# markweberdev/maskbit

Hardware: AMD Instinct MI355X
Metric: images/sec (256x256, 64-step MaskBit-12bit, CFG) (higher is better)
Workload: dtype f16

## Files before the change

include/maskbit_hip_diag.h:

```cpp
#ifndef MASKBIT_HIP_DIAG_H
#define MASKBIT_HIP_DIAG_H

#include "maskbit_hip.h"

#ifdef __cplusplus
extern "C" {
#endif

int mb_gemm(int epi, const void* A, const void* W, const float* bias, const float* residual, float* out_f32,
            void* out_h16, int M, int N, int K, int period, int variant, mb_stream stream);
int mb_gemm_ex(int epi, const void* A, const void* W, const float* bias, const float* residual, float* out_f32, void* out_h16,
               int M, int N, int K, const float* ln_stats, const float* ln_g, const float* ln_b, int period, int variant, mb_stream stream);
int mb_layernorm(const float* y, const float* gamma, const float* beta, float eps, float* x_f32, void* x_h16, void* x_lo, float* stats,
                 int M, int d, mb_stream stream);
int mb_gemm_act_split(int epi, const void* A_hi, const void* A_lo, const void* W, const float* bias, const float* residual,
                      float* out_f32, void* out_h16, int M, int N, int kw, int variant, mb_stream stream);
int mb_gemm_mini(int epi, const void* A, const void* W, const float* bias, const float* residual, float* out_f32, void* out_h16, void* out4,
                 void* out4_scale, int rows, int pair, int N, int K, int nlo, const void* const* lo, mb_stream stream);
int mb_gemm_mini_seq(int epi, const void* A, const void* W, const float* bias, const float* residual, float* out_f32, void* out_h16, void* out4,
                     void* out4_scale, void* out4l, void* out4l_scale, int rows, int pair, int seq_rows, int N, int K, int nlo, const void* const* lo, mb_stream stream);
int mb_w4_from_f32(const float* W, int N, int K, void* dst4, void* scale_out, mb_stream stream);
int mb_w4lo_from_f32(const float* W, int N, int K, void* dst4, void* scale_out, mb_stream stream);
int mb_gemm_head(int epi, const void* A_hi, const void* A_lo, const void* W_hi, const void* W_lo, const float* scale, const float* bias, int bias_per_pos,
                 float* out_f32, int M, int N, int kw, int period, mb_stream stream);
int mb_cast_f32_to_h16(const float* src, void* dst, int64_t n, mb_stream stream);
int mb_split_f32_planes(const float* src, void* hi, void* lo, int N, int K, float* scale_out, unsigned* tmp, mb_stream stream);
int mb_gemm_mini_split(int epi, const void* A_hi, const void* A_lo, const void* W, const float* bias, void* out_h16, void* out4, void* out4_scale,
                       int rows, int N, int kw, const void* const* lo, mb_stream stream);
int mb_gemm_mini_ln(const void* A, const void* W, const float* bias, float* y, const float* ln_stats, const float* ln_g, const float* ln_b, int rows, int pair,
                    int seq_rows, int N, int K, int nlo, const void* const* lo, mb_stream stream);
int mb_layernorm_f4(const float* y, const float* gamma, const float* beta, float eps, float* x_f32, void* x_h16, void* x4, void* x4_scale, void* xl4,
                    void* xl4_scale, int M, int d, mb_stream stream);
int mb_layernorm_f4_seq(const float* y, const float* gamma, const float* beta, float eps, float* x_f32, void* x_h16, void* x4, void* x4_scale, void* xl4,
                        void* xl4_scale, int M, int d, int seq_rows, mb_stream stream);

int mb_layernorm_pair(const float* y, const float* gamma, const float* beta, float eps, void* x_h16, float* stats, void* x4, void* x4_scale, void* xl4,
                      void* xl4_scale, int P, int d, int seq_rows, mb_stream stream);
int mb_pairify(const float* x_f32, void* x_h16, void* x4, void* x4_scale, void* xl4, void* xl4_scale, int P, int d, int seq_rows, mb_stream stream);
int mb_embed_ln(const int64_t* tokens, const int64_t* labels, const uint8_t* drop, const float* w_in, const float* b_in, const float* class_emb,
                const float* pos, const float* gamma, const float* beta, const float* tables, float* x_f32, void* x_h16, void* x_lo, void* x4,
                void* x4_scale, void* xl4, void* xl4_scale, int nb, int seq, int m, int gbits, int d, int nclass, mb_stream stream);
int mb_embed_pair(const int64_t* tokens, const int64_t* labels, const float* w_in, const float* b_in, const float* class_emb, const float* pos,
                  const float* gamma, const float* beta, const float* tables, float* x_f32, void* x_h16, void* x4, void* x4_scale, void* xl4,
                  void* xl4_scale, int nb, int seq, int m, int gbits, int d, int nclass, mb_stream stream);
int mb_attention_pair(const void* qkv, void* out_h16, int pairs, int N, int d, int heads, mb_stream stream);
int mb_attention_pair_f4(const void* qkv, void* out_h16, void* out4, void* out4_scale, void* out4l, void* out4l_scale, int pairs, int N, int d, int heads, mb_stream stream);
int mb_attention(const void* qkv, void* out_h16, void* out4, void* out4_scale, int nb, int N, int d, int heads, mb_stream stream);
int mb_attention_probs(const void* qkv, float* out_f32, int nb, int N, int d, int heads, mb_stream stream);
int mb_gen_set_alo(mb_gen* g, int gemm_mask);
int mb_set_cu_count(int n);
int mb_gen_set_walk(mb_gen* g, int mode);
int mb_diag_set_walk(int reverse);
int mb_walk_tile(int vb, int ntiles, int reverse);
int mb_walk_seq(int slot, int n, int grp, int reverse);
int mb_walk_row(int slot, int rows, int seq_rows, int pair, int reverse);
int mb_walk_group(int seq_rows, int pair);
int mb_gemm_ht_supported(int epi, int M, int N, int K);

int mb_seeded_noise(const int64_t* seeds, int step, float randomize_temperature, float conf_weight, float* exp_u, float* exp_noise, float* conf_u,
                    float* conf_noise, int B, int P, int C, mb_stream stream);

int mb_vq_argmin(const float* z, const float* codebook, int N, int C, int K, int l2, int splits, int64_t* idx, float* dist, mb_stream stream);

int mb_vq_encode_rows(const void* z_h16, int stride16, const float* z_f32, const float* codebook, int B, int HW, int C, int K, int l2, int splits,
                      int64_t* idx, float* zq_nchw, float* zraw_nchw, float* dist, mb_stream stream);
int mb_vq_gather(const int64_t* codes, const float* codebook, int64_t npix, int C, int K, int l2, int cin_pad, void* out_h16, unsigned* sat,
                 mb_stream stream);
int mb_vq_pack_latent(const float* z_nchw, int B, int K, int HW, int cin_pad, void* out_h16, unsigned* sat, mb_stream stream);
int mb_lfq_pack(const void* z_h16, int B, int HW, int K, int Kp, int64_t* idx, float* zq_nchw, float* zraw_nchw, mb_stream stream);
int mb_lfq_latent(const int64_t* tokens, int64_t npix, int K, void* out_h16, mb_stream stream);
int mb_pack_image(const float* img_nchw, int B, int C, int H, int W, void* out_h16, mb_stream stream);

int mb_conv_layer(const void* in_h16, const float* w_oihw, const float* bias, const float* gn_gamma, const float* gn_beta, const void* residual_h16,
                  void* out_h16, float* img_nchw, uint8_t* img_nhwc_u8, const float* out_gamma, const float* out_beta, float* out_scale_shift,
                  float* out_gn_part, int* part_tiles, unsigned* saturated, int B, int H, int W, int Cin, int Cout, int ks, int up, int final_layer,
                  mb_stream stream);
int mb_conv_layer_ex(const void* in_h16, const float* w_oihw, const float* bias, const float* gn_gamma, const float* gn_beta, const void* residual_h16,
                     void* out_h16, float* img_nchw, uint8_t* img_nhwc_u8, const float* out_gamma, const float* out_beta, float* out_scale_shift,
                     float* out_gn_part, int* part_tiles, unsigned* saturated, int B, int H, int W, int Cin, int Cout, int ks, int up, int final_layer,
                     int flags, mb_stream stream);
int mb_autoenc_block(const void* x_h16, const float* n1_g, const float* n1_b, const float* c1_w, const float* c1_b, const float* n2_g, const float* n2_b,
                     const float* c2_w, const float* c2_b, const float* sc_w, const float* sc_b, int form, int bias, void* out_h16, void* h1_h16,
                     void* mid_h16, const float* out_gamma, const float* out_beta, float* out_scale_shift, unsigned* saturated, int B, int H, int W,
                     int cin, int cout, mb_stream stream);
int mb_groupnorm_stats(const void* x_h16, const float* gamma, const float* beta, float* scale_shift, int B, int HW, int C, mb_stream stream);
int mb_avgpool2(const void* x_h16, void* y_h16, int B, int H, int W, int C, mb_stream stream);
int mb_s2d(const void* x_h16, void* y_h16, int B, int H, int W, int C, mb_stream stream);

int mb_conv_relu_layer(const void* in_h16, const float* w_oihw, const float* bias, void* out_h16, unsigned* saturated, int B, int H, int W, int Cin,
                       int Cout, int ks, mb_stream stream);
int mb_maxpool2(const void* x_h16, void* y_h16, int B, int H, int W, int C, mb_stream stream);
int mb_lpips_input(const float* real, const float* fake, const float* shift_scale, void* out_h16, int B, int H, int W, int clamp01, mb_stream stream);
int mb_lpips_distance(const void* feat_a, const void* feat_b, const float* w, int B, int HW, int C, double* per_image, mb_stream stream);
int mb_lpips_features(mb_lpips* h, const float* real, const float* fake, int B, int H, int W, int clamp01, void* tap0, void* tap1, void* tap2, void* tap3,
                      void* tap4, mb_stream stream);

int mb_convbn_layer(const void* in_h16, const float* w_oihw, const float* scale, const float* shift, void* out_h16, unsigned* saturated, int B, int H,
                    int W, int Cin, int Cout, int kh, int kw, int stride, int ph, int pw, int in_off, int in_cs, int out_off, int out_cs, int variant,
                    mb_stream stream);
int mb_pool3(const void* x_h16, void* y_h16, int B, int H, int W, int C, int mode, int in_off, int in_cs, int out_off, int out_cs, mb_stream stream);
int mb_inception_input(const uint8_t* u8, void* out_h16, int B, int H, int W, mb_stream stream);
int mb_inception_taps(mb_inception* h, const uint8_t* u8, int B, int H, int W, void* map0, void* map1, void* map2, void* map3, float* tap64,
                      float* tap192, float* tap768, float* pool, float* logits_unbiased, float* logits, mb_stream stream);

int mb_spatial_attention(const void* q, const void* k, const void* v, void* out_h16, unsigned* sat, int B, int N, int ld, int ldo, mb_stream stream);
int mb_taming_set_tap(mb_taming* h, int block, void* out_h16);
int mb_taming_attn_block(mb_taming* h, int block, const void* x_h16, void* qkv_out, void* attn_out, void* out_h16, const float* out_gamma,
                         const float* out_beta, float* out_scale_shift, int B, int H, int W, mb_stream stream);
int mb_taming_final(mb_taming* h, const void* x_h16, float* img_nchw, uint8_t* img_nhwc_u8, int B, int H, int W, mb_stream stream);
int mb_taming_pack_image(const float* img_nchw, void* out_h16, int B, int H, int W, mb_stream stream);

int mb_gemm_f32(int epi, const float* A, const float* W, const float* bias, const float* residual, float* out, int M, int N, int K, int period,
                int bias_per_pos, mb_stream stream);
int mb_attention_f32(const float* qkv, float* out, int nb, int N, int d, int heads, mb_stream stream);

typedef struct {
  int64_t* label; int64_t* seed;
  int32_t* num_regen; int32_t* slot; int32_t* local_step; int32_t* N;
  mb_request_step* pool;
  int max_active, max_steps;
} mb_session_rows;
int mb_session_row_table(const mb_session_rows* rows, mb_request_step* row_out, int A, mb_stream stream);
int mb_session_admit_rows(const mb_session_rows* rows, int64_t* tokens, int A, int K, const int64_t* labels, const int64_t* seeds, const int* num_steps,
                          const mb_request_step* schedule, const int64_t* init_tokens, int n, int m, int C, mb_stream stream);
int mb_session_retire(const mb_session_rows* rows, int64_t* tokens, const int64_t* pred, int64_t* codes_all, int64_t* codes_out, int32_t* plan,
                      int A, int n, int m, int C, mb_stream stream);

int mb_image_coeffs(int in_size, int out_size, int filter, int first, int count, int ksize, int32_t* xmin, int32_t* n, int32_t* taps, mb_stream stream);

#ifdef __cplusplus
}
#endif
#endif
```

maskbit_amd/_lib.py:

```python
from __future__ import annotations

import ctypes as C
import os
from typing import Optional

_HERE = os.path.dirname(os.path.abspath(__file__))
LIB_PATH = os.path.join(_HERE, "libmaskbit_hip.so")
ABI_VERSION = 8


class GenCfg(C.Structure):
    _fields_ = [(n, C.c_int) for n in ("bits", "splits", "hidden", "heads", "depth", "mlp", "seq", "nclass", "prenorm", "embed_tables", "precision")]


class DecCfg(C.Structure):
    _fields_ = [("token_size", C.c_int), ("hidden_channels", C.c_int), ("num_resolutions", C.c_int),
                ("num_res_blocks", C.c_int), ("num_channels", C.c_int), ("channel_mult", C.c_int * 8),
                ("latent_size", C.c_int), ("build_encoder", C.c_int), ("sample_with_conv", C.c_int),
                ("enc_res_blocks", C.c_int)]


class SamplePlan(C.Structure):
    _fields_ = [("num_steps", C.c_int), ("use_guidance", C.c_int), ("scale", C.POINTER(C.c_float)),
                ("temperature", C.POINTER(C.c_float)), ("mask_len", C.POINTER(C.c_int)), ("step_begin", C.c_int), ("step_end", C.c_int)]
# ... 25 lines not shown
SIGNATURES = {
    "mb_gen_saturation_count": (C.c_int, [C.c_void_p, C.POINTER(C.c_uint), C.c_int, C.c_void_p]),
    "mb_abi_version": (C.c_int, []),
    "mb_last_error": (C.c_char_p, []),
    "mb_gen_create": (C.c_int, [C.POINTER(GenCfg), C.c_int, C.POINTER(C.c_void_p)]),
    "mb_gen_destroy": (None, [C.c_void_p]),
    "mb_gen_load": (C.c_int, [C.c_void_p, C.c_char_p, C.c_void_p, C.POINTER(C.c_int64), C.c_int, C.c_void_p]),
    "mb_gen_set_alo": (C.c_int, [C.c_void_p, C.c_int]),
    "mb_gen_forward": (C.c_int, [C.c_void_p, C.c_void_p, C.c_void_p, C.c_void_p, C.c_void_p, C.c_int, C.c_void_p]),
    "mb_gen_forward_cfg": (C.c_int, [C.c_void_p, C.c_void_p, C.c_void_p, C.c_void_p, C.c_int, C.c_void_p]),
    "mb_gen_forward_attn": (C.c_int, [C.c_void_p, C.c_void_p, C.c_void_p, C.c_void_p, C.c_void_p, C.c_void_p, C.c_int, C.c_void_p]),
    "mb_sample_step": (C.c_int, [C.c_void_p, C.c_void_p, C.c_float, C.c_float, C.c_void_p, C.c_void_p, C.c_int,
                                 C.c_void_p, C.c_void_p, C.c_void_p, C.c_int, C.c_int, C.c_int, C.c_int, C.c_void_p]),
    "mb_dec_create": (C.c_int, [C.POINTER(DecCfg), C.c_int, C.POINTER(C.c_void_p)]),
    "mb_dec_destroy": (None, [C.c_void_p]),
    "mb_dec_load": (C.c_int, [C.c_void_p, C.c_char_p, C.c_void_p, C.POINTER(C.c_int64), C.c_int, C.c_void_p]),
    "mb_dec_decode": (C.c_int, [C.c_void_p, C.c_void_p, C.c_void_p, C.c_void_p, C.c_int, C.c_void_p]),
    "mb_dec_saturation_count": (C.c_int, [C.c_void_p, C.POINTER(C.c_uint), C.c_int, C.c_void_p]),
    "mb_enc_encode": (C.c_int, [C.c_void_p, C.c_void_p, C.c_void_p, C.c_void_p, C.c_void_p, C.c_int, C.c_void_p]),
    "mb_dec_create_vq": (C.c_int, [C.POINTER(DecCfg), C.c_int, C.c_int, C.c_int, C.POINTER(C.c_void_p)]),
    "mb_dec_decode_latent": (C.c_int, [C.c_void_p, C.c_void_p, C.c_void_p, C.c_void_p, C.c_int, C.c_void_p]),
    "mb_enc_encode_vq": (C.c_int, [C.c_void_p, C.c_void_p, C.c_void_p, C.c_void_p, C.c_void_p, C.c_void_p, C.c_int, C.c_void_p]),
    "mb_vq_argmin": (C.c_int, [C.c_void_p, C.c_void_p, C.c_int, C.c_int, C.c_int, C.c_int, C.c_int, C.c_void_p, C.c_void_p, C.c_void_p]),
    "mb_vq_encode_rows": (C.c_int, [C.c_void_p, C.c_int, C.c_void_p, C.c_void_p] + [C.c_int] * 6 + [C.c_void_p] * 5),
    "mb_vq_gather": (C.c_int, [C.c_void_p, C.c_void_p, C.c_int64, C.c_int, C.c_int, C.c_int, C.c_int, C.c_void_p, C.c_void_p, C.c_void_p]),
    "mb_vq_pack_latent": (C.c_int, [C.c_void_p, C.c_int, C.c_int, C.c_int, C.c_int, C.c_void_p, C.c_void_p, C.c_void_p]),
    "mb_lfq_pack": (C.c_int, [C.c_void_p, C.c_int, C.c_int, C.c_int, C.c_int, C.c_void_p, C.c_void_p, C.c_void_p, C.c_void_p]),
    "mb_lfq_latent": (C.c_int, [C.c_void_p, C.c_int64, C.c_int, C.c_void_p, C.c_void_p]),
    "mb_pack_image": (C.c_int, [C.c_void_p, C.c_int, C.c_int, C.c_int, C.c_int, C.c_void_p, C.c_void_p]),
    "mb_sample": (C.c_int, [C.c_void_p, C.c_void_p, C.POINTER(SamplePlan), C.c_void_p, C.c_int, C.c_void_p, C.c_void_p,
                            C.c_void_p, C.c_void_p, C.c_void_p, C.c_void_p, C.c_void_p]),
    "mb_sample_step_edit": (C.c_int, [C.c_void_p, C.c_void_p, C.c_float, C.c_float, C.c_void_p, C.c_void_p, C.c_float, C.c_void_p,
                                      C.c_void_p, C.c_void_p, C.c_void_p, C.c_int, C.c_int, C.c_int, C.c_int, C.c_void_p]),
    "mb_sample_edit": (C.c_int, [C.c_void_p, C.c_void_p, C.POINTER(EditPlan), C.c_void_p, C.c_int, C.c_void_p, C.c_void_p, C.c_void_p,
                                 C.c_void_p, C.c_void_p, C.c_void_p, C.c_void_p, C.c_void_p]),
    "mb_sample_step_seeded": (C.c_int, [C.c_void_p, C.c_void_p, C.c_float, C.c_float, C.c_void_p, C.c_int, C.c_float, C.c_float, C.c_float, C.c_void_p,
                                        C.c_void_p, C.c_void_p, C.c_void_p, C.c_int, C.c_int, C.c_int, C.c_int, C.c_void_p]),
    "mb_sample_seeded": (C.c_int, [C.c_void_p, C.c_void_p, C.POINTER(EditPlan), C.c_void_p, C.c_int, C.c_void_p, C.c_void_p, C.c_float,
                                   C.POINTER(C.c_float), C.c_void_p, C.c_void_p, C.c_void_p, C.c_void_p, C.c_void_p]),
    "mb_sample_step_requests": (C.c_int, [C.c_void_p, C.c_void_p, C.c_void_p, C.c_void_p, C.c_void_p, C.c_void_p, C.c_void_p, C.c_void_p,
                                          C.c_int, C.c_int, C.c_int, C.c_int, C.c_void_p]),
    "mb_sample_requests": (C.c_int, [C.c_void_p, C.c_void_p, C.POINTER(RequestPlan), C.c_void_p, C.c_int, C.c_void_p, C.c_void_p,
                                     C.c_void_p, C.c_void_p, C.c_void_p, C.c_void_p, C.c_void_p]),
    "mb_session_create": (C.c_int, [C.c_int, C.c_int, C.c_int, C.c_int, C.c_int, C.c_int, C.POINTER(C.c_void_p)]),
    "mb_session_destroy": (None, [C.c_void_p]),
    "mb_session_admit": (C.c_int, [C.c_void_p, C.c_int, C.c_void_p, C.c_void_p, C.POINTER(C.c_int), C.c_void_p, C.c_void_p, C.POINTER(C.c_uint64), C.c_void_p]),
    "mb_session_due": (C.c_int, [C.c_void_p]),
    "mb_session_active": (C.c_int, [C.c_void_p]),
    "mb_session_tick": (C.c_int, [C.c_void_p, C.c_void_p, C.c_void_p, C.c_void_p, C.c_void_p, C.c_void_p, C.c_void_p, C.POINTER(C.c_uint64),
                                  C.POINTER(C.c_uint64), C.POINTER(C.c_int), C.c_void_p]),
    "mb_session_row_table": (C.c_int, [C.POINTER(SessionRows), C.c_void_p, C.c_int, C.c_void_p]),
    "mb_session_admit_rows": (C.c_int, [C.POINTER(SessionRows), C.c_void_p, C.c_int, C.c_int, C.c_void_p, C.c_void_p, C.POINTER(C.c_int), C.c_void_p,
                                        C.c_void_p, C.c_int, C.c_int, C.c_int, C.c_void_p]),
    "mb_session_retire": (C.c_int, [C.POINTER(SessionRows), C.c_void_p, C.c_void_p, C.c_void_p, C.c_void_p, C.c_void_p, C.c_int, C.c_int, C.c_int,
                                    C.c_int, C.c_void_p]),
    "mb_seeded_noise": (C.c_int, [C.c_void_p, C.c_int, C.c_float, C.c_float, C.c_void_p, C.c_void_p, C.c_void_p, C.c_void_p, C.c_int, C.c_int, C.c_int,
                                  C.c_void_p]),
    "mb_edit_init": (C.c_int, [C.c_void_p, C.c_void_p, C.c_void_p, C.c_void_p, C.c_int, C.c_int, C.c_int, C.c_int, C.c_void_p]),
    "mb_edit_token_mask": (C.c_int, [C.c_void_p, C.c_void_p, C.c_int, C.c_int, C.c_int, C.c_int, C.c_void_p]),
    "mb_edit_composite": (C.c_int, [C.c_void_p, C.c_void_p, C.c_void_p, C.c_void_p, C.c_void_p, C.c_int, C.c_int, C.c_int, C.c_int, C.c_void_p]),
    "mb_gemm_ex": (C.c_int, [C.c_int, C.c_void_p, C.c_void_p, C.c_void_p, C.c_void_p, C.c_void_p, C.c_void_p, C.c_int, C.c_int, C.c_int,
                             C.c_void_p, C.c_void_p, C.c_void_p, C.c_int, C.c_int, C.c_void_p]),
    "mb_layernorm": (C.c_int, [C.c_void_p, C.c_void_p, C.c_void_p, C.c_float, C.c_void_p, C.c_void_p, C.c_void_p, C.c_void_p, C.c_int, C.c_int, C.c_void_p]),
    "mb_w4_from_f32": (C.c_int, [C.c_void_p, C.c_int, C.c_int, C.c_void_p, C.c_void_p, C.c_void_p]),
    "mb_w4lo_from_f32": (C.c_int, [C.c_void_p, C.c_int, C.c_int, C.c_void_p, C.c_void_p, C.c_void_p]),
    "mb_gemm_head": (C.c_int, [C.c_int, C.c_void_p, C.c_void_p, C.c_void_p, C.c_void_p, C.c_void_p, C.c_void_p, C.c_int, C.c_void_p, C.c_int, C.c_int,
                               C.c_int, C.c_int, C.c_void_p]),
    "mb_cast_f32_to_h16": (C.c_int, [C.c_void_p, C.c_void_p, C.c_int64, C.c_void_p]),
    "mb_split_f32_planes": (C.c_int, [C.c_void_p, C.c_void_p, C.c_void_p, C.c_int, C.c_int, C.c_void_p, C.c_void_p, C.c_void_p]),
    "mb_layernorm_f4": (C.c_int, [C.c_void_p, C.c_void_p, C.c_void_p, C.c_float, C.c_void_p, C.c_void_p, C.c_void_p, C.c_void_p, C.c_void_p, C.c_void_p,
                                  C.c_int, C.c_int, C.c_void_p]),
    "mb_layernorm_f4_seq": (C.c_int, [C.c_void_p, C.c_void_p, C.c_void_p, C.c_float] + [C.c_void_p] * 6 + [C.c_int] * 3 + [C.c_void_p]),
    "mb_layernorm_pair": (C.c_int, [C.c_void_p, C.c_void_p, C.c_void_p, C.c_float] + [C.c_void_p] * 6 + [C.c_int] * 3 + [C.c_void_p]),
    "mb_pairify": (C.c_int, [C.c_void_p] * 6 + [C.c_int] * 3 + [C.c_void_p]),
    "mb_embed_ln": (C.c_int, [C.c_void_p] * 17 + [C.c_int] * 6 + [C.c_void_p]),
    "mb_embed_pair": (C.c_int, [C.c_void_p] * 15 + [C.c_int] * 6 + [C.c_void_p]),
    "mb_attention": (C.c_int, [C.c_void_p, C.c_void_p, C.c_void_p, C.c_void_p, C.c_int, C.c_int, C.c_int, C.c_int, C.c_void_p]),
    "mb_attention_probs": (C.c_int, [C.c_void_p, C.c_void_p, C.c_int, C.c_int, C.c_int, C.c_int, C.c_void_p]),
    "mb_attention_pair": (C.c_int, [C.c_void_p, C.c_void_p, C.c_int, C.c_int, C.c_int, C.c_int, C.c_void_p]),
    "mb_attention_pair_f4": (C.c_int, [C.c_void_p, C.c_void_p, C.c_void_p, C.c_void_p, C.c_void_p, C.c_void_p, C.c_int, C.c_int, C.c_int, C.c_int, C.c_void_p]),
    "mb_gemm_mini": (C.c_int, [C.c_int, C.c_void_p, C.c_void_p, C.c_void_p, C.c_void_p, C.c_void_p, C.c_void_p, C.c_void_p, C.c_void_p, C.c_int, C.c_int,
                               C.c_int, C.c_int, C.c_int, C.POINTER(C.c_void_p), C.c_void_p]),
    "mb_gemm_mini_seq": (C.c_int, [C.c_int, C.c_void_p, C.c_void_p, C.c_void_p, C.c_void_p, C.c_void_p, C.c_void_p, C.c_void_p, C.c_void_p, C.c_void_p, C.c_void_p, C.c_int, C.c_int,
                                   C.c_int, C.c_int, C.c_int, C.c_int, C.POINTER(C.c_void_p), C.c_void_p]),
    "mb_gemm_mini_split": (C.c_int, [C.c_int, C.c_void_p, C.c_void_p, C.c_void_p, C.c_void_p, C.c_void_p, C.c_void_p, C.c_void_p, C.c_int, C.c_int, C.c_int,
                                     C.POINTER(C.c_void_p), C.c_void_p]),
    "mb_gemm_mini_ln": (C.c_int, [C.c_void_p] * 7 + [C.c_int] * 6 + [C.POINTER(C.c_void_p), C.c_void_p]),
    "mb_gemm_act_split": (C.c_int, [C.c_int, C.c_void_p, C.c_void_p, C.c_void_p, C.c_void_p, C.c_void_p, C.c_void_p, C.c_void_p, C.c_int, C.c_int, C.c_int,
                                    C.c_int, C.c_void_p]),
    "mb_gemm": (C.c_int, [C.c_int, C.c_void_p, C.c_void_p, C.c_void_p, C.c_void_p, C.c_void_p, C.c_void_p, C.c_int, C.c_int, C.c_int,
                          C.c_int, C.c_int, C.c_void_p]),
    "mb_conv_layer": (C.c_int, [C.c_void_p] * 13 + [C.POINTER(C.c_int), C.POINTER(C.c_uint)] + [C.c_int] * 8 + [C.c_void_p]),
    "mb_conv_layer_ex": (C.c_int, [C.c_void_p] * 13 + [C.POINTER(C.c_int), C.POINTER(C.c_uint)] + [C.c_int] * 9 + [C.c_void_p]),
    "mb_autoenc_block": (C.c_int, [C.c_void_p] * 11 + [C.c_int, C.c_int] + [C.c_void_p] * 6 + [C.POINTER(C.c_uint)] + [C.c_int] * 5 + [C.c_void_p]),
    "mb_groupnorm_stats": (C.c_int, [C.c_void_p, C.c_void_p, C.c_void_p, C.c_void_p, C.c_int, C.c_int, C.c_int, C.c_void_p]),
    "mb_avgpool2": (C.c_int, [C.c_void_p, C.c_void_p, C.c_int, C.c_int, C.c_int, C.c_int, C.c_void_p]),
    "mb_s2d": (C.c_int, [C.c_void_p, C.c_void_p, C.c_int, C.c_int, C.c_int, C.c_int, C.c_void_p]),
    "mb_eval_workspace_bytes": (C.c_size_t, [C.c_int, C.c_int, C.c_int, C.c_int]),
    "mb_eval_images": (C.c_int, [C.c_void_p, C.c_void_p, C.c_int, C.c_int, C.c_int, C.c_int, C.c_uint, C.c_int, C.c_void_p, C.c_void_p, C.c_void_p, C.c_void_p]),
    "mb_eval_codebook": (C.c_int, [C.c_void_p, C.c_int64, C.c_int, C.c_void_p, C.c_void_p, C.c_void_p]),
    "mb_mlm_workspace_bytes": (C.c_size_t, [C.c_int, C.c_int, C.c_int, C.c_int]),
    "mb_mlm_state_bytes": (C.c_size_t, []),
    "mb_mlm_mask": (C.c_int, [C.c_void_p, C.c_void_p, C.c_void_p, C.c_int64, C.c_void_p, C.c_void_p, C.c_int, C.c_int, C.c_int, C.c_void_p]),
    "mb_mlm_loss": (C.c_int, [C.c_void_p, C.c_void_p, C.c_void_p, C.c_float, C.c_int, C.c_int, C.c_int, C.c_int, C.c_void_p, C.c_void_p, C.c_void_p,
                              C.c_void_p, C.c_void_p]),
    "mb_lpips_create": (C.c_int, [C.c_int, C.c_int, C.c_int, C.POINTER(C.c_void_p)]),
    "mb_lpips_destroy": (None, [C.c_void_p]),
    "mb_lpips_load": (C.c_int, [C.c_void_p, C.c_char_p, C.c_void_p, C.POINTER(C.c_int64), C.c_int, C.c_void_p]),
    "mb_lpips_forward": (C.c_int, [C.c_void_p, C.c_void_p, C.c_void_p, C.c_int, C.c_int, C.c_int, C.c_int, C.c_void_p, C.c_void_p, C.c_void_p]),
    "mb_lpips_saturation_count": (C.c_int, [C.c_void_p, C.POINTER(C.c_uint), C.c_int, C.c_void_p]),
    "mb_conv_relu_layer": (C.c_int, [C.c_void_p] * 4 + [C.POINTER(C.c_uint)] + [C.c_int] * 6 + [C.c_void_p]),
    "mb_maxpool2": (C.c_int, [C.c_void_p, C.c_void_p, C.c_int, C.c_int, C.c_int, C.c_int, C.c_void_p]),
    "mb_lpips_input": (C.c_int, [C.c_void_p, C.c_void_p, C.c_void_p, C.c_void_p, C.c_int, C.c_int, C.c_int, C.c_int, C.c_void_p]),
    "mb_lpips_distance": (C.c_int, [C.c_void_p, C.c_void_p, C.c_void_p, C.c_int, C.c_int, C.c_int, C.c_void_p, C.c_void_p]),
    "mb_lpips_features": (C.c_int, [C.c_void_p, C.c_void_p, C.c_void_p, C.c_int, C.c_int, C.c_int, C.c_int] + [C.c_void_p] * 6),
    "mb_fid_accumulate": (C.c_int, [C.c_void_p, C.c_int, C.c_int, C.c_int, C.c_int64, C.c_void_p, C.c_void_p, C.c_void_p]),
    "mb_is_workspace_bytes": (C.c_size_t, [C.c_int, C.c_int]),
    "mb_is_accumulate": (C.c_int, [C.c_void_p, C.c_int, C.c_int, C.c_int, C.c_int64, C.c_void_p, C.c_void_p, C.c_void_p, C.c_void_p]),
    "mb_manifold_workspace_bytes": (C.c_size_t, [C.c_int, C.c_int]),
    "mb_knn_radii": (C.c_int, [C.c_void_p, C.c_int, C.c_int, C.c_int, C.c_int64, C.c_int, C.c_void_p, C.c_void_p, C.c_void_p]),
    "mb_manifold_cover": (C.c_int, [C.c_void_p, C.c_int, C.c_int, C.c_int64, C.c_void_p, C.c_int, C.c_int, C.c_int64, C.c_int, C.c_void_p, C.c_void_p,
                                    C.c_void_p, C.c_void_p]),
    "mb_image_workspace_bytes": (C.c_size_t, [C.POINTER(ImageJob), C.c_int, C.c_int]),
    "mb_image_resample": (C.c_int, [C.POINTER(ImageJob), C.c_void_p, C.c_int, C.c_int, C.c_void_p, C.c_size_t, C.c_void_p, C.c_void_p, C.c_int64,
                                    C.c_void_p, C.c_size_t, C.c_void_p]),
    "mb_image_coeffs": (C.c_int, [C.c_int] * 6 + [C.c_void_p] * 4),
    "mb_inception_create": (C.c_int, [C.c_int, C.POINTER(C.c_void_p)]),
    "mb_inception_destroy": (None, [C.c_void_p]),
    "mb_inception_load": (C.c_int, [C.c_void_p, C.c_char_p, C.c_void_p, C.POINTER(C.c_int64), C.c_int, C.c_void_p]),
    "mb_inception_forward": (C.c_int, [C.c_void_p, C.c_void_p, C.c_int, C.c_int, C.c_int, C.c_void_p, C.c_void_p, C.c_void_p, C.c_void_p]),
    "mb_inception_forward_spatial": (C.c_int, [C.c_void_p, C.c_void_p, C.c_int, C.c_int, C.c_int, C.c_void_p, C.c_void_p, C.c_void_p, C.c_void_p, C.c_void_p]),
    "mb_inception_saturation_count": (C.c_int, [C.c_void_p, C.POINTER(C.c_uint), C.c_int, C.c_void_p]),
    "mb_convbn_layer": (C.c_int, [C.c_void_p] * 5 + [C.POINTER(C.c_uint)] + [C.c_int] * 15 + [C.c_void_p]),
    "mb_pool3": (C.c_int, [C.c_void_p, C.c_void_p] + [C.c_int] * 9 + [C.c_void_p]),
    "mb_inception_input": (C.c_int, [C.c_void_p, C.c_void_p, C.c_int, C.c_int, C.c_int, C.c_void_p]),
    "mb_inception_taps": (C.c_int, [C.c_void_p, C.c_void_p, C.c_int, C.c_int, C.c_int] + [C.c_void_p] * 11),
    "mb_taming_create": (C.c_int, [C.c_int, C.c_int, C.POINTER(C.c_void_p)]),
    "mb_taming_destroy": (None, [C.c_void_p]),
    "mb_taming_load": (C.c_int, [C.c_void_p, C.c_char_p, C.c_void_p, C.POINTER(C.c_int64), C.c_int, C.c_void_p]),
    "mb_taming_encode": (C.c_int, [C.c_void_p, C.c_void_p, C.c_void_p, C.c_void_p, C.c_void_p, C.c_void_p, C.c_int, C.c_void_p]),
    "mb_taming_decode": (C.c_int, [C.c_void_p, C.c_void_p, C.c_void_p, C.c_void_p, C.c_int, C.c_void_p]),
    "mb_taming_decode_latent": (C.c_int, [C.c_void_p, C.c_void_p, C.c_void_p, C.c_void_p, C.c_int, C.c_void_p]),
    "mb_taming_saturation_count": (C.c_int, [C.c_void_p, C.POINTER(C.c_uint), C.c_int, C.c_void_p]),
    "mb_taming_set_tap": (C.c_int, [C.c_void_p, C.c_int, C.c_void_p]),
    "mb_taming_attn_block": (C.c_int, [C.c_void_p, C.c_int] + [C.c_void_p] * 7 + [C.c_int] * 3 + [C.c_void_p]),
    "mb_taming_final": (C.c_int, [C.c_void_p] * 4 + [C.c_int] * 3 + [C.c_void_p]),
    "mb_taming_pack_image": (C.c_int, [C.c_void_p, C.c_void_p, C.c_int, C.c_int, C.c_int, C.c_void_p]),
    "mb_spatial_attention": (C.c_int, [C.c_void_p] * 5 + [C.c_int] * 4 + [C.c_void_p]),
    "mb_gemm_f32": (C.c_int, [C.c_int] + [C.c_void_p] * 5 + [C.c_int] * 5 + [C.c_void_p]),
    "mb_attention_f32": (C.c_int, [C.c_void_p, C.c_void_p] + [C.c_int] * 4 + [C.c_void_p]),
    "mb_set_cu_count":(C.c_int, [C.c_int]),
    "mb_gen_set_walk": (C.c_int, [C.c_void_p, C.c_int]),
    "mb_diag_set_walk": (C.c_int, [C.c_int]),
    "mb_walk_tile": (C.c_int, [C.c_int] * 3),
    "mb_walk_seq": (C.c_int, [C.c_int] * 4),
    "mb_walk_row": (C.c_int, [C.c_int] * 5),
    "mb_walk_group": (C.c_int, [C.c_int] * 2),
    "mb_gemm_ht_supported": (C.c_int, [C.c_int, C.c_int, C.c_int, C.c_int]),
    "mb_prof_enable": (C.c_int, [C.c_int]),
    "mb_prof_read": (C.c_int, [C.c_char_p, C.c_int]),
}

_lib: Optional[C.CDLL] = None


def load() -> C.CDLL:
    global _lib
    if _lib is not None:
        return _lib
    import torch
    if not os.path.exists(LIB_PATH):
        raise RuntimeError(
            f"{LIB_PATH} is missing: the MaskBit HIP kernels are not built. Run `python -c 'import __graft_entry__ as g; "
            f"g.build()'` (needs hipcc, gfx950). There is no CPU fallback in maskbit_amd.")
    lib = C.CDLL(LIB_PATH)
    for name, (res, args) in SIGNATURES.items():
        fn = getattr(lib, name)
        fn.restype = res
        fn.argtypes = args
    v = lib.mb_abi_version()
    if v != ABI_VERSION:
        raise RuntimeError(f"libmaskbit_hip.so ABI {v} != binding ABI {ABI_VERSION}; rebuild")
    _lib = lib
    return lib


def check(rc: int, what: str = "") -> None:
    if rc != 0:
        msg = load().mb_last_error()
        raise RuntimeError(f"{what or 'libmaskbit_hip'} failed (code {rc}): {msg.decode() if msg else '?'}")


def prof_enable(on, every: int = 1) -> None:
    load().mb_prof_enable(max(1, int(every)) if on else 0)


def prof_read() -> dict:
    buf = C.create_string_buffer(1 << 16)
    n = load().mb_prof_read(buf, len(buf))
    if n < 0:
        check(n, "mb_prof_read")
    out = {}
    for line in buf.value.decode().splitlines():
        name, calls, ms = line.split()
        out[name] = (int(calls), float(ms))
    return out
```

maskbit_amd/csrc/diag.hip:

```cpp
#include <hip/hip_runtime.h>

#include <vector>

#include "../../include/maskbit_hip_diag.h"
#include "mb_abi.h"
#include "mb_autoenc.h"
#include "mb_conv.h"
#include "mb_image.h"
#include "mb_kernels.h"
#include "mb_spattn.h"
#include "mb_vq.h"

using mb::fail;
using mb::launched;
using mb::ProfScope;

namespace {

int g_walk_reverse = 0;

int run_gemm(mb_stream stream, int epi, const mb::GemmArgs& args, int variant, const char* mini = nullptr) {
  mb::GemmArgs a = args;
  a.reverse = g_walk_reverse;
  ProfScope p("gemm_diag", (hipStream_t)stream);
  if (mb::gemm_tn((hipStream_t)stream, (mb::GemmEpi)epi, a, variant))
    return mini ? fail(-3, "%s: shape refused", mini) : fail(-3, "GEMM shape M=%d N=%d K=%d is outside the kernels' shapes", a.M, a.N, a.K);
  return launched();
}

int w4_entry(const char* what, decltype(mb::w4_from_f32)* pack, const float* W, int N, int K, void* dst4, void* scale_out, mb_stream stream) {
  if (!W || !dst4 || !scale_out || N <= 0 || K <= 0 || N % 64 || K % 128) return fail(-1, "%s: bad arguments", what);
  pack((hipStream_t)stream, W, (uint8_t*)dst4, N, K, (uint8_t*)scale_out);
  return launched();
}

int pool_entry(const char* what, decltype(mb::launch_s2d)* launch, const void* x, void* y, int B, int H, int W, int C, mb_stream stream) {
  if (!x || !y) return fail(-1, "%s: null argument", what);
  if (B <= 0 || H <= 0 || W <= 0 || H % 2 || W % 2 || C <= 0 || C % 8) return fail(-1, "%s: H and W must be even, C a multiple of 8", what);
  launch((hipStream_t)stream, (const h16*)x, (h16*)y, B, H, W, C);
  return launched();
}

bool vq_shape_ok(int C, int K) { return C >= 2 && C <= 65536 && K >= 1 && K <= 256; }
mb::VqCodebook vq_shape(int C, int K, int l2) {
  mb::VqCodebook q;
  q.C = C; q.K = K; q.Kp = mb::vq_kp(K); q.Cpad = mb::vq_cpad(C); q.l2 = l2 ? 1 : 0;
  return q;
}
struct StreamTemps {
  explicit StreamTemps(hipStream_t stream) : s(stream) {}
  StreamTemps(const StreamTemps&) = delete;
  StreamTemps& operator=(const StreamTemps&) = delete;
  ~StreamTemps() { for (void* p : owned) (void)hipFreeAsync(p, s); }
  template <class T>
  void get(T** out, size_t n) {
    void* p = nullptr;
    *out = nullptr;
    if (ok && hipMallocAsync(&p, n * sizeof(T), s) == hipSuccess) { owned.push_back(p); *out = (T*)p; }
    else ok = false;
  }
  hipStream_t s;
  std::vector<void*> owned;
  bool ok = true;
};

int f4_rows(const char* who, mb::Fp4Rows& f4, void* x4, void* x4_scale, void* xl4, void* xl4_scale, int rows, int d, int seq_rows) {
  f4 = mb::Fp4Rows{};
  if ((x4 != nullptr) != (x4_scale != nullptr) || (xl4 != nullptr) != (xl4_scale != nullptr)) return fail(-1, "%s: an e2m1 copy and its scale array go together", who);
  if (!x4 && !xl4) return 0;
  if (d != 768 && d != 1024) return fail(-1, "%s: e2m1 copies are written at d = 768 / 1024 only, not %d", who, d);
  if (seq_rows < 65 || (seq_rows - 1) % 64 || rows % seq_rows)
    return fail(-1, "%s: e2m1 copies: sequences of 64 k tokens + the class token, whole sequences (%d rows of %d)", who, rows, seq_rows);
  f4 = mb::Fp4Rows{(uint8_t*)x4, (uint8_t*)x4_scale, (uint8_t*)xl4, (uint8_t*)xl4_scale, rows / seq_rows, seq_rows};
  return 0;
}

int embed_args(const char* who, mb::EmbedArgs& e, const int64_t* tokens, const int64_t* labels, const float* w_in, const float* b_in, const float* class_emb,
               const float* pos, const float* gamma, const float* beta, const float* tables, float* x_f32, void* x_h16, void* x4, void* x4_scale, void* xl4,
               void* xl4_scale, int nb, int seq, int m, int gbits, int d, int nclass) {
  if (!tokens || !labels || !class_emb || !pos || !gamma || !beta || !x_f32 || !x_h16 || (!tables && (!w_in || !b_in))) return fail(-1, "%s: null argument", who);
  if (nb <= 0 || seq <= 0 || m <= 0 || gbits <= 0 || d <= 0 || nclass < 0) return fail(-1, "%s: bad sizes", who);
  if (d > 2048) return fail(-1, "%s: d = %d is beyond the row kernels (2048)", who, d);
  if ((int64_t)m * gbits > 24) return fail(-1, "%s: %d groups of %d bits are beyond the embed kernels (24 bits)", who, m, gbits);
  if (tables && m > 8) return fail(-1, "%s: %d embedding tables are beyond the embed kernel (8)", who, m);
  mb::Fp4Rows f4;
  if (int rc = f4_rows(who, f4, x4, x4_scale, xl4, xl4_scale, nb * (seq + 1), d, seq + 1)) return rc;
  e = mb::EmbedArgs{tokens, labels, nullptr, nullptr, b_in, class_emb, pos, gamma, beta, x_f32, (h16*)x_h16, nb, seq, m, gbits, d, nclass, tables};
  e.f4 = f4;
  return 0;
}
int embed_weight(const char* who, mb::DevArena& arena, mb::EmbedArgs& e, const float* w_in, hipStream_t s) {
  if (e.tables) return 0;
  const int K = e.m * e.gbits;
  float* wt = nullptr;
  arena.get(&wt, (size_t)K * e.d);
  if (int rc = arena.failed(who)) return rc;
  mb::transpose_f32(s, w_in, wt, e.d, K);
  e.w_in = wt;
  return 0;
}

}

extern "C" {

int mb_set_cu_count(int n) { mb::set_cu_count(n); return 0; }
int mb_diag_set_walk(int reverse) {
  if (reverse != 0 && reverse != 1) return fail(-1, "mb_diag_set_walk: direction 0 or 1");
  g_walk_reverse = reverse;
  return 0;
}
int mb_walk_tile(int vb, int ntiles, int reverse) { return vb < 0 || vb >= ntiles ? -1 : mb::walk_tile(vb, ntiles, reverse ? 1 : 0); }
int mb_walk_seq(int slot, int n, int grp, int reverse) { return slot < 0 || slot >= n || grp < 1 ? -1 : mb::walk_seq(slot, n, grp, reverse ? 1 : 0); }
int mb_walk_row(int slot, int rows, int seq_rows, int pair, int reverse) {
  return slot < 0 || slot >= rows ? -1 : mb::walk_row(slot, rows, mb::walk_rows(rows, seq_rows, pair != 0, reverse));
}
int mb_walk_group(int seq_rows, int pair) { return seq_rows < 2 ? -1 : mb::walk_group(seq_rows, pair != 0); }
int mb_gemm_ht_supported(int epi, int M, int N, int K) {
  mb::GemmArgs a{nullptr, nullptr, nullptr, nullptr, nullptr, nullptr, M, N, K, 0};
  return mb::gemm_ht_supported((mb::GemmEpi)epi, a) ? 1 : 0;
}

int mb_gemm(int epi, const void* A, const void* W, const float* bias, const float* residual, float* out_f32, void* out_h16,
            int M, int N, int K, int period, int variant, mb_stream stream) {
  if (!A || !W || !bias || epi < 0 || epi > 4) return fail(-1, "mb_gemm: bad arguments");
  if (K % 64) return fail(-1, "mb_gemm: K must be a multiple of 64");
  mb::GemmArgs a{(const h16*)A, (const h16*)W, bias, residual, out_f32, (h16*)out_h16, M, N, K, period};
  return run_gemm(stream, epi, a, variant);
}
int mb_gemm_ex(int epi, const void* A, const void* W, const float* bias, const float* residual, float* out_f32, void* out_h16,
               int M, int N, int K, const float* ln_stats, const float* ln_g, const float* ln_b, int period, int variant, mb_stream stream) {
  if (!A || !W || !bias || epi < 0 || epi > 4) return fail(-1, "mb_gemm_ex: bad arguments");
  if (K % 64) return fail(-1, "mb_gemm_ex: K must be a multiple of 64");
  if (ln_stats && (!ln_g || !ln_b || epi != mb::EPI_RES_F32)) return fail(-1, "mb_gemm_ex: LayerNorm residual needs gamma, beta and the fp32+residual epilogue");
  mb::GemmArgs a{(const h16*)A, (const h16*)W, bias, residual, out_f32, (h16*)out_h16, M, N, K, period, nullptr, ln_stats, ln_g, ln_b};
  return run_gemm(stream, epi, a, variant);
}
int mb_gemm_act_split(int epi, const void* A_hi, const void* A_lo, const void* W, const float* bias, const float* residual, float* out_f32,
                      void* out_h16, int M, int N, int kw, int variant, mb_stream stream) {
  if (!A_hi || !A_lo || !W || !bias || epi < 0 || epi > 3 || kw <= 0 || kw % 64) return fail(-1, "mb_gemm_act_split: bad arguments");
  mb::GemmArgs a{(const h16*)A_hi, (const h16*)W, bias, residual, out_f32, (h16*)out_h16, M, N, 2 * kw, 0};
  a.A2 = (const h16*)A_lo; a.kw = kw;
  return run_gemm(stream, epi, a, variant);
}
int mb_gemm_mini(int epi, const void* A, const void* W, const float* bias, const float* residual, float* out_f32, void* out_h16, void* out4,
                 void* out4_scale, int rows, int pair, int N, int K, int nlo, const void* const* lo , mb_stream stream) {
  return mb_gemm_mini_seq(epi, A, W, bias, residual, out_f32, out_h16, out4, out4_scale, nullptr, nullptr, rows, pair, 0, N, K, nlo, lo, stream);
}
int mb_gemm_mini_seq(int epi, const void* A, const void* W, const float* bias, const float* residual, float* out_f32, void* out_h16, void* out4,
                     void* out4_scale, void* out4l, void* out4l_scale, int rows, int pair, int seq_rows, int N, int K, int nlo, const void* const* lo, mb_stream stream) {
  if ((out4l || out4l_scale) && (!out4l || !out4l_scale || !out4 || !out4_scale)) return fail(-1, "mb_gemm_mini_seq: the lo copy (out4l / out4l_scale) rides with the value copy (out4 / out4_scale)");
  if (!A || !W || !bias || epi < 0 || epi > 2 || rows <= 0 || K <= 0 || K % 64 || nlo < 0 || nlo > 2 || (nlo && !lo)) return fail(-1, "mb_gemm_mini: bad arguments");
  mb::GemmArgs a{(const h16*)A, (const h16*)W, bias, residual, out_f32, (h16*)out_h16, pair ? 2 * rows : rows, N, K, 0};
  if (pair) a.pair_rows = rows;
  a.seq_rows = seq_rows;
  a.nlo = nlo;
  for (int i = 0; i < nlo; ++i) a.lo[i] = {(const uint8_t*)lo[4 * i], (const uint8_t*)lo[4 * i + 1], (const uint8_t*)lo[4 * i + 2], (const uint8_t*)lo[4 * i + 3]};
  a.out4 = (uint8_t*)out4; a.out4_scale = (uint8_t*)out4_scale;
  a.out4l = (uint8_t*)out4l; a.out4l_scale = (uint8_t*)out4l_scale;
  if ((!seq_rows && a.M % 257) || !mb::gemm_ht_supported((mb::GemmEpi)epi, a)) return fail(-3, "mb_gemm_mini: shape not supported by the sequence-aligned tiles");
  return run_gemm(stream, epi, a, 257, "mb_gemm_mini");
}
int mb_gemm_mini_ln(const void* A, const void* W, const float* bias, float* y, const float* ln_stats, const float* ln_g, const float* ln_b, int rows, int pair,
                    int seq_rows, int N, int K, int nlo, const void* const* lo, mb_stream stream) {
  if (!A || !W || !bias || !y || !ln_stats || !ln_g || !ln_b || rows <= 0 || K <= 0 || K % 64 || nlo < 0 || nlo > 2 || (nlo && !lo))
    return fail(-1, "mb_gemm_mini_ln: bad arguments");
  mb::GemmArgs a{(const h16*)A, (const h16*)W, bias, y, y, nullptr, pair ? 2 * rows : rows, N, K, 0, nullptr, ln_stats, ln_g, ln_b};
  if (pair) a.pair_rows = rows;
  a.seq_rows = seq_rows;
  a.nlo = nlo;
  for (int i = 0; i < nlo; ++i) a.lo[i] = {(const uint8_t*)lo[4 * i], (const uint8_t*)lo[4 * i + 1], (const uint8_t*)lo[4 * i + 2], (const uint8_t*)lo[4 * i + 3]};
  if ((!seq_rows && a.M % 257) || !mb::gemm_ht_supported(mb::EPI_RES_F32, a)) return fail(-3, "mb_gemm_mini_ln: shape not supported by the sequence-aligned tiles");
  return run_gemm(stream, mb::EPI_RES_F32, a, 257, "mb_gemm_mini_ln");
}
int mb_gemm_mini_split(int epi, const void* A_hi, const void* A_lo, const void* W, const float* bias, void* out_h16, void* out4, void* out4_scale,
                       int rows, int N, int kw, const void* const* lo , mb_stream stream) {
  if (!A_hi || !A_lo || !W || !bias || !out_h16 || !lo || epi < 0 || epi > 1 || rows <= 0 || rows % 257 || kw <= 0 || kw % 128)
    return fail(-1, "mb_gemm_mini_split: bad arguments");
  mb::GemmArgs a{(const h16*)A_hi, (const h16*)W, bias, nullptr, nullptr, (h16*)out_h16, rows, N, 2 * kw, 0};
  a.A2 = (const h16*)A_lo; a.kw = kw;
  a.nlo = 1;
  a.lo[0] = {(const uint8_t*)lo[0], (const uint8_t*)lo[1], (const uint8_t*)lo[2], (const uint8_t*)lo[3]};
  a.out4 = (uint8_t*)out4; a.out4_scale = (uint8_t*)out4_scale;
  if (!mb::gemm_ht_supported((mb::GemmEpi)epi, a)) return fail(-3, "mb_gemm_mini_split: shape not supported by the sequence-aligned tiles");
  return run_gemm(stream, epi, a, 257, "mb_gemm_mini_split");
}

int mb_gemm_head(int epi, const void* A_hi, const void* A_lo, const void* W_hi, const void* W_lo, const float* scale, const float* bias, int bias_per_pos,
                 float* out_f32, int M, int N, int kw, int period, mb_stream stream) {
  if (!A_hi || !A_lo || !W_hi || !bias || !out_f32) return fail(-1, "mb_gemm_head: null argument");
  if ((W_lo != nullptr) != (scale != nullptr)) return fail(-1, "mb_gemm_head: the weights' lo plane and the scale go together");
  if (epi != mb::EPI_GELU_F32 && epi != mb::EPI_LOGITS_F32) return fail(-1, "mb_gemm_head: epilogue 3 or 4");
  if (M <= 0 || N <= 0 || N % 4 || kw <= 0 || kw % 64) return fail(-1, "mb_gemm_head: M > 0, N a multiple of 4, kw a multiple of 64");
  if (epi == mb::EPI_LOGITS_F32 && (period < 2 || M % period)) return fail(-1, "mb_gemm_head: epilogue 4: whole sequences of period >= 2 rows");
  if (bias_per_pos && epi != mb::EPI_LOGITS_F32) return fail(-1, "mb_gemm_head: a per-position bias goes with epilogue 4");
  mb::GemmArgs a{(const h16*)A_hi, (const h16*)W_hi, bias, nullptr, out_f32, nullptr, M, N, (W_lo ? 3 : 2) * kw, period, scale};
  a.A2 = (const h16*)A_lo; a.kw = kw; a.W2 = (const h16*)W_lo;
  a.bias_per_pos = bias_per_pos;
  return run_gemm(stream, epi, a, 0, "mb_gemm_head");
}
int mb_cast_f32_to_h16(const float* src, void* dst, int64_t n, mb_stream stream) {
  if (!src || !dst || n < 0) return fail(-1, "mb_cast_f32_to_h16: bad arguments");
  mb::cast_f32_to_h16((hipStream_t)stream, src, (h16*)dst, (size_t)n);
  return launched();
}
int mb_split_f32_planes(const float* src, void* hi, void* lo, int N, int K, float* scale_out, unsigned* tmp, mb_stream stream) {
  if (!src || !hi || !lo || !scale_out || !tmp || N <= 0 || K <= 0) return fail(-1, "mb_split_f32_planes: bad arguments");
  mb::split_f32_to_h16_planes((hipStream_t)stream, src, (h16*)hi, (h16*)lo, N, K, scale_out, tmp);
  return launched();
}

int mb_w4_from_f32(const float* W, int N, int K, void* dst4, void* scale_out, mb_stream stream) {
  return w4_entry("mb_w4_from_f32", mb::w4_from_f32, W, N, K, dst4, scale_out, stream);
}
int mb_w4lo_from_f32(const float* W, int N, int K, void* dst4, void* scale_out, mb_stream stream) {
  return w4_entry("mb_w4lo_from_f32", mb::w4lo_from_f32, W, N, K, dst4, scale_out, stream);
}

int mb_layernorm(const float* y, const float* gamma, const float* beta, float eps, float* x_f32, void* x_h16, void* x_lo, float* stats, int M,
                 int d, mb_stream stream) {
  if (!y || !gamma || !beta || M <= 0 || d <= 0 || d > 2048) return fail(-1, "mb_layernorm: bad arguments");
  mb::layernorm_rows((hipStream_t)stream, y, gamma, beta, eps, x_f32, (h16*)x_h16, stats, M, d, (h16*)x_lo, mb::Fp4Rows{}, g_walk_reverse, 0);
  return launched();
}
int mb_layernorm_f4_seq(const float* y, const float* gamma, const float* beta, float eps, float* x_f32, void* x_h16, void* x4, void* x4_scale, void* xl4,
                        void* xl4_scale, int M, int d, int seq_rows, mb_stream stream) {
  if (!y || !gamma || !beta || (!x4 && !xl4) || M <= 0) return fail(-1, "mb_layernorm_f4: bad arguments (an e2m1 output is required)");
  mb::Fp4Rows f4;
  if (int rc = f4_rows("mb_layernorm_f4", f4, x4, x4_scale, xl4, xl4_scale, M, d, seq_rows)) return rc;
  mb::layernorm_rows((hipStream_t)stream, y, gamma, beta, eps, x_f32, (h16*)x_h16, nullptr, M, d, nullptr, f4, g_walk_reverse, seq_rows);
  return launched();
}
int mb_layernorm_f4(const float* y, const float* gamma, const float* beta, float eps, float* x_f32, void* x_h16, void* x4, void* x4_scale, void* xl4,
                    void* xl4_scale, int M, int d, mb_stream stream) {
  return mb_layernorm_f4_seq(y, gamma, beta, eps, x_f32, x_h16, x4, x4_scale, xl4, xl4_scale, M, d, 257, stream);
}

int mb_layernorm_pair(const float* y, const float* gamma, const float* beta, float eps, void* x_h16, float* stats, void* x4, void* x4_scale, void* xl4,
                      void* xl4_scale, int P, int d, int seq_rows, mb_stream stream) {
  if (!y || !gamma || !beta || !x_h16 || P <= 0 || d <= 0 || d > 2048) return fail(-1, "mb_layernorm_pair: bad arguments");
  mb::Fp4Rows f4;
  if (int rc = f4_rows("mb_layernorm_pair", f4, x4, x4_scale, xl4, xl4_scale, P, d, seq_rows)) return rc;
  if (mb::layernorm_pair((hipStream_t)stream, y, gamma, beta, eps, (h16*)x_h16, stats, P, d, f4, g_walk_reverse, seq_rows))
    return fail(-3, "mb_layernorm_pair: width %d is outside the pair kernels (768 or 1024)", d);
  return launched();
}
int mb_pairify(const float* x_f32, void* x_h16, void* x4, void* x4_scale, void* xl4, void* xl4_scale, int P, int d, int seq_rows, mb_stream stream) {
  if (!x_f32 || !x_h16 || P <= 0 || d <= 0 || d > 2048) return fail(-1, "mb_pairify: bad arguments");
  mb::Fp4Rows f4;
  if (int rc = f4_rows("mb_pairify", f4, x4, x4_scale, xl4, xl4_scale, P, d, seq_rows)) return rc;
  if (mb::pairify_rows((hipStream_t)stream, x_f32, (h16*)x_h16, P, d, f4, g_walk_reverse, seq_rows))
    return fail(-3, "mb_pairify: width %d is outside the pair kernels (768 or 1024)", d);
  return launched();
}
int mb_embed_ln(const int64_t* tokens, const int64_t* labels, const uint8_t* drop, const float* w_in, const float* b_in, const float* class_emb,
                const float* pos, const float* gamma, const float* beta, const float* tables, float* x_f32, void* x_h16, void* x_lo, void* x4,
                void* x4_scale, void* xl4, void* xl4_scale, int nb, int seq, int m, int gbits, int d, int nclass, mb_stream stream) {
  mb::EmbedArgs e;
  if (int rc = embed_args("mb_embed_ln", e, tokens, labels, w_in, b_in, class_emb, pos, gamma, beta, tables, x_f32, x_h16, x4, x4_scale, xl4, xl4_scale,
                          nb, seq, m, gbits, d, nclass)) return rc;
  e.drop = drop; e.x_lo = (h16*)x_lo;
  mb::DevArena arena;
  if (int rc = embed_weight("mb_embed_ln", arena, e, w_in, (hipStream_t)stream)) return rc;
  mb::embed_ln((hipStream_t)stream, e);
  if (hipStreamSynchronize((hipStream_t)stream) != hipSuccess) return fail(-10, "mb_embed_ln: the launch failed");
  return launched();
}
int mb_embed_pair(const int64_t* tokens, const int64_t* labels, const float* w_in, const float* b_in, const float* class_emb, const float* pos,
                  const float* gamma, const float* beta, const float* tables, float* x_f32, void* x_h16, void* x4, void* x4_scale, void* xl4,
                  void* xl4_scale, int nb, int seq, int m, int gbits, int d, int nclass, mb_stream stream) {
  const bool f4 = x4 || x4_scale || xl4 || xl4_scale;
  if (tables || (m > 0 && gbits > 0 && (int64_t)m * gbits > 24) || (!f4 && d > 0 && d <= 2048 && d != 768 && d != 1024))
    return fail(-3, "mb_embed_pair: not served by the fused kernel (embedding tables, more than 24 bits, widths other than 768 / 1024): embed_ln + pairify");
  mb::EmbedArgs e;
  if (int rc = embed_args("mb_embed_pair", e, tokens, labels, w_in, b_in, class_emb, pos, gamma, beta, tables, x_f32, x_h16, x4, x4_scale, xl4, xl4_scale,
                          nb, seq, m, gbits, d, nclass)) return rc;
  mb::DevArena arena;
  if (int rc = embed_weight("mb_embed_pair", arena, e, w_in, (hipStream_t)stream)) return rc;
  const int refused = mb::embed_pair((hipStream_t)stream, e);
  if (hipStreamSynchronize((hipStream_t)stream) != hipSuccess) return fail(-10, "mb_embed_pair: the launch failed");
  if (refused) return fail(-3, "mb_embed_pair: not served by the fused kernel");
  return launched();
}

int mb_attention(const void* qkv, void* out_h16, void* out4, void* out4_scale, int nb, int N, int d, int heads, mb_stream stream) {
  if (!qkv || !out_h16 || (!out4) != (!out4_scale) || nb <= 0 || N <= 0 || d <= 0 || heads <= 0 || d % heads) return fail(-1, "mb_attention: bad arguments");
  if (d / heads != 32 && d / heads != 64) return fail(-3, "mb_attention: head width %d is outside the attention kernels (32 or 64)", d / heads);
  ProfScope p("attention", (hipStream_t)stream);
  mb::attention((hipStream_t)stream, (const h16*)qkv, (h16*)out_h16, nb, N, d, heads, (uint8_t*)out4, (uint8_t*)out4_scale, g_walk_reverse);
  return launched();
}
int mb_attention_probs(const void* qkv, float* out_f32, int nb, int N, int d, int heads, mb_stream stream) {
  if (!qkv || !out_f32 || nb <= 0 || N <= 0 || d <= 0 || heads <= 0 || d % heads) return fail(-1, "mb_attention_probs: bad arguments");
  if (mb::attention_probs((hipStream_t)stream, (const h16*)qkv, out_f32, nb, N, d, heads))
    return fail(-3, "mb_attention_probs: head width %d / N = %d tokens is outside the probabilities kernel (32 or 64; N <= 5120)", d / heads, N);
  return launched();
}
int mb_attention_pair(const void* qkv, void* out_h16, int pairs, int N, int d, int heads, mb_stream stream) {
  if (!qkv || !out_h16 || pairs <= 0 || N <= 0 || heads <= 0 || d % heads) return fail(-1, "mb_attention_pair: bad arguments");
  ProfScope p("attention", (hipStream_t)stream);
  if (mb::attention_pair((hipStream_t)stream, (const h16*)qkv, (h16*)out_h16, pairs, N, d, heads, nullptr, nullptr, nullptr, nullptr, g_walk_reverse))
    return fail(-3, "mb_attention_pair: head width %d (N = %d tokens) is outside the attention kernels", d / heads, N);
  return launched();
}
int mb_attention_pair_f4(const void* qkv, void* out_h16, void* out4, void* out4_scale, void* out4l, void* out4l_scale, int pairs, int N, int d, int heads, mb_stream stream) {
  if (!qkv || !out_h16 || !out4 || !out4_scale || (!out4l) != (!out4l_scale) || pairs <= 0 || N <= 0 || heads <= 0 || d % heads) return fail(-1, "mb_attention_pair_f4: bad arguments");
  ProfScope p("attention", (hipStream_t)stream);
  if (mb::attention_pair((hipStream_t)stream, (const h16*)qkv, (h16*)out_h16, pairs, N, d, heads, (uint8_t*)out4, (uint8_t*)out4_scale, (uint8_t*)out4l, (uint8_t*)out4l_scale, g_walk_reverse))
    return fail(-3, "mb_attention_pair_f4: head width %d / N = %d tokens: no e2m1 copy for this shape", d / heads, N);
  return launched();
}

int mb_seeded_noise(const int64_t* seeds, int step, float randomize_temperature, float conf_weight, float* exp_u, float* exp_noise, float* conf_u,
                    float* conf_noise, int B, int P, int C, mb_stream stream) {
  if (!seeds || !exp_noise || !conf_noise) return fail(-1, "mb_seeded_noise: null argument");
  if (B <= 0 || P <= 0 || C <= 0 || step < 0) return fail(-1, "mb_seeded_noise: bad sizes");
  if (exp_u == exp_noise || conf_u == conf_noise) return fail(-1, "mb_seeded_noise: the uniforms and the noise must not alias");
  if (mb::seeded_noise_dump((hipStream_t)stream, seeds, step, randomize_temperature, conf_weight, exp_u, exp_noise, conf_u, conf_noise, B, P, C))
    return fail(-1, "mb_seeded_noise: C=%d or P=%d too large", C, P);
  return launched();
}

int mb_vq_argmin(const float* z, const float* codebook, int N, int C, int K, int l2, int splits, int64_t* idx, float* dist, mb_stream stream) {
  if (!z || !codebook || !idx) return fail(-1, "mb_vq_argmin: null argument");
  if (int rc = mb::vq_argmin(z, codebook, N, C, K, l2, splits, idx, dist, (hipStream_t)stream)) return rc;
  return launched();
}

int mb_vq_encode_rows(const void* z_h16, int stride16, const float* z_f32, const float* codebook, int B, int HW, int C, int K, int l2, int splits,
                      int64_t* idx, float* zq_nchw, float* zraw_nchw, float* dist, mb_stream stream) {
  using namespace mb;
  hipStream_t s = (hipStream_t)stream;
  if (!codebook || (z_h16 != nullptr) == (z_f32 != nullptr)) return fail(-1, "mb_vq_encode_rows: a codebook and exactly one of z_h16 / z_f32 required");
  if (!vq_shape_ok(C, K)) return fail(-1, "mb_vq_encode_rows: C in [2, 65536], K in [1, 256] required");
  if (B < 1 || HW < 1 || (int64_t)B * HW > (1 << 24)) return fail(-1, "mb_vq_encode_rows: B >= 1, HW >= 1, B * HW <= 2^24 required");
  if (z_h16 && stride16 < K) return fail(-1, "mb_vq_encode_rows: stride16 = %d is below K = %d", stride16, K);
  const int N = B * HW, Npad = vq_npad(N);
  VqCodebook q = vq_shape(C, K, l2);
  splits = vq_splits(q, N, splits);
  StreamTemps t(s);
  float *zT = nullptr, *ps = nullptr;
  int* pi = nullptr;
  t.get(&q.cb, (size_t)C * K); t.get(&q.cbT, (size_t)q.Kp * q.Cpad); t.get(&q.cbn, (size_t)q.Cpad);
  t.get(&zT, (size_t)q.Kp * Npad); t.get(&ps, (size_t)splits * Npad); t.get(&pi, (size_t)splits * Npad);
  if (!t.ok) return fail(-10, "mb_vq_encode_rows: device allocation failed");
  vq_prep_codebook(q, codebook, s);
  vq_prep_rows(q, (const h16*)z_h16, stride16, z_f32, N, HW, zT, zraw_nchw, s);
  vq_search(q, zT, N, HW, splits, ps, pi, idx, zq_nchw, dist, s);
  return launched();
}
int mb_vq_gather(const int64_t* codes, const float* codebook, int64_t npix, int C, int K, int l2, int cin_pad, void* out_h16, unsigned* sat,
                 mb_stream stream) {
  using namespace mb;
  hipStream_t s = (hipStream_t)stream;
  if (!codes || !codebook || !out_h16 || !sat) return fail(-1, "mb_vq_gather: null argument");
  if (!vq_shape_ok(C, K)) return fail(-1, "mb_vq_gather: C in [2, 65536], K in [1, 256] required");
  if (npix < 1 || npix > (1 << 24)) return fail(-1, "mb_vq_gather: npix in [1, 2^24] required");
  if (cin_pad < K || cin_pad % CK) return fail(-1, "mb_vq_gather: cin_pad = %d must be a multiple of 64 and at least K = %d", cin_pad, K);
  VqCodebook q = vq_shape(C, K, l2);
  StreamTemps t(s);
  t.get(&q.cb, (size_t)C * K); t.get(&q.cbT, (size_t)q.Kp * q.Cpad); t.get(&q.cbn, (size_t)q.Cpad);
  if (!t.ok) return fail(-10, "mb_vq_gather: device allocation failed");
  vq_prep_codebook(q, codebook, s);
  vq_gather(q, codes, (size_t)npix, (h16*)out_h16, cin_pad, sat, s);
  return launched();
}
int mb_vq_pack_latent(const float* z_nchw, int B, int K, int HW, int cin_pad, void* out_h16, unsigned* sat, mb_stream stream) {
  if (!z_nchw || !out_h16 || !sat) return fail(-1, "mb_vq_pack_latent: null argument");
  if (B < 1 || HW < 1 || (int64_t)B * HW > (1 << 24) || K < 1 || K > 256) return fail(-1, "mb_vq_pack_latent: B >= 1, HW >= 1, B * HW <= 2^24, K in [1, 256] required");
  if (cin_pad < K || cin_pad % mb::CK) return fail(-1, "mb_vq_pack_latent: cin_pad = %d must be a multiple of 64 and at least K = %d", cin_pad, K);
  mb::vq_pack_latent(z_nchw, B, K, HW, (h16*)out_h16, cin_pad, sat, (hipStream_t)stream);
  return launched();
}
int mb_lfq_pack(const void* z_h16, int B, int HW, int K, int Kp, int64_t* idx, float* zq_nchw, float* zraw_nchw, mb_stream stream) {
  if (!z_h16 || !idx) return fail(-1, "mb_lfq_pack: null argument");
  if (B < 1 || HW < 1 || (int64_t)B * HW > (1 << 24)) return fail(-1, "mb_lfq_pack: B >= 1, HW >= 1, B * HW <= 2^24 required");
  if (K < 1 || K > mb::CK || Kp < K) return fail(-1, "mb_lfq_pack: K in [1, 64] and Kp >= K required");
  mb::launch_lfq((hipStream_t)stream, (const h16*)z_h16, idx, zq_nchw, zraw_nchw, B, HW, K, Kp);
  return launched();
}
int mb_lfq_latent(const int64_t* tokens, int64_t npix, int K, void* out_h16, mb_stream stream) {
  if (!tokens || !out_h16) return fail(-1, "mb_lfq_latent: null argument");
  if (npix < 1 || npix > (1 << 24) || K < 1 || K > mb::CK) return fail(-1, "mb_lfq_latent: npix in [1, 2^24] and K in [1, 64] required");
  mb::launch_latent((hipStream_t)stream, tokens, (h16*)out_h16, (size_t)npix, K);
  return launched();
}
int mb_pack_image(const float* img_nchw, int B, int C, int H, int W, void* out_h16, mb_stream stream) {
  if (!img_nchw || !out_h16) return fail(-1, "mb_pack_image: null argument");
  if (B < 1 || H < 1 || W < 1 || (int64_t)B * H * W > (1 << 24) || C < 1 || C > 4) return fail(-1, "mb_pack_image: B, H, W >= 1, B * H * W <= 2^24, C in [1, 4] required");
  mb::launch_pack_image((hipStream_t)stream, img_nchw, (h16*)out_h16, B, C, H, W);
  return launched();
}

int mb_conv_layer(const void* in_h16, const float* w_oihw, const float* bias, const float* gn_gamma, const float* gn_beta, const void* residual_h16,
                  void* out_h16, float* img_nchw, uint8_t* img_nhwc_u8, const float* out_gamma, const float* out_beta, float* out_scale_shift,
                  float* out_gn_part, int* part_tiles, unsigned* saturated, int B, int H, int W, int Cin, int Cout, int ks, int up_, int final_layer,
// ... 249 lines not shown
```

maskbit_amd/csrc/engine.hip:

```cpp
#include <hip/hip_runtime.h>

#include <algorithm>
#include <cstdio>
#include <cstring>
#include <string>
#include <vector>

#include "../../include/maskbit_hip_diag.h"
#include "mb_abi.h"
#include "mb_kernels.h"

using mb::fail;
using mb::g_prof;
using mb::launched;
using mb::ProfScope;

struct F4Buf { uint8_t *v = nullptr, *s = nullptr; };

struct mb_gen {
  mb_gen_cfg c{};
  int max_seqs = 0, chunk_seqs = 0, N = 0, C = 0, gbits = 0, device = 0;
  struct Layer {
    h16 *wqkv = nullptr, *wo = nullptr, *w1 = nullptr, *w2 = nullptr;
    float *bqkv = nullptr, *bo = nullptr, *b1 = nullptr, *b2 = nullptr;
    float *ln1g = nullptr, *ln1b = nullptr, *ln2g = nullptr, *ln2b = nullptr;
  };
  std::vector<Layer> layers;
  float *w_in = nullptr, *b_in = nullptr, *class_emb = nullptr, *pos = nullptr, *ln0g = nullptr, *ln0b = nullptr;
  h16 *wl = nullptr, *wp = nullptr;
  float *bl = nullptr, *lnhg = nullptr, *lnhb = nullptr, *bp = nullptr;
  float *lnag = nullptr, *lnab = nullptr;
  float *tables = nullptr, *bias_pos = nullptr;
  unsigned* split_tmp = nullptr;
  float *y_f32 = nullptr, *ln_stats = nullptr;
  h16 *x_h16 = nullptr, *x_lo = nullptr, *qkv = nullptr, *att = nullptr, *h = nullptr;
  bool pair_ok = false, mini_ok = false;
  F4Buf x4, xl4;
  std::vector<uint8_t*> w4, w4s;
  float* logits_tmp = nullptr;
  h16 *wl_lo = nullptr, *wp_lo = nullptr;
  float* head_scale = nullptr;
  unsigned* sat = nullptr;
  std::vector<uint8_t*> w4lo, w4los;
  F4Buf att4, h4;
  F4Buf attl4, hl4;
  struct Run {
    struct Id {
      int B = 0, steps = 0, guided = 0, kind = 0;
      bool operator==(const Id& o) const { return B == o.B && steps == o.steps && guided == o.guided && kind == o.kind; }
    } id;
    int next = -1;
    const int64_t* cfg_labels = nullptr;
    int cfg_B = 0;
  } run;
  int* num_regen = nullptr;
  int alo_mask = 0, alo_mask_built = 0;
  int walk = 1;
  bool f32 = false;
  struct Layer32 { float *wqkv = nullptr, *wo = nullptr, *w1 = nullptr, *w2 = nullptr; };
  std::vector<Layer32> layers32;
  float *wl32 = nullptr, *wp32 = nullptr;
  float *x_f32 = nullptr, *qkv32 = nullptr, *att32 = nullptr, *h32 = nullptr;
  int64_t *tok_a = nullptr, *tok_b = nullptr, *tok_cfg = nullptr, *lab_cfg = nullptr, *pred = nullptr, *codes = nullptr;
  uint8_t* drop_cfg = nullptr;
  float* logits = nullptr;
  mb::DevArena mem;
  int loaded = 0;
};

namespace {

void alloc_f4(mb::DevArena& m, F4Buf* b, size_t rows, size_t width, size_t ntok) {
  m.zeroed(&b->v, rows * 2 * width);
  m.zeroed(&b->s, (width / 64) * ntok + 256);
}

int head_gemms(mb_gen* g, float* logits, int M, hipStream_t s) {
  using namespace mb;
  const mb_gen_cfg& c = g->c;
  const int d = c.hidden;
  int rc = 0;
  { ProfScope p("gemm_head", s, true);
    GemmArgs ga{g->x_h16, g->wl, g->bl, nullptr, g->y_f32, nullptr, M, d, 3 * d, 0, g->head_scale};
    ga.A2 = g->x_lo; ga.kw = d; ga.W2 = g->wl_lo;
    rc |= gemm_tn(s, EPI_GELU_F32, ga); }
  { ProfScope p("layernorm", s, true);
    layernorm_rows(s, g->y_f32, g->lnhg, g->lnhb, 1e-12f, nullptr, g->x_h16, nullptr, M, d, g->x_lo); }
  { ProfScope p("gemm_head", s, true);
    GemmArgs ga{g->x_h16, g->wp, c.embed_tables ? g->bias_pos : g->bp, nullptr, logits, nullptr, M, c.splits * g->C, (g->wp_lo ? 3 : 2) * d, g->N,
                g->wp_lo ? g->head_scale + 1 : nullptr};
    ga.A2 = g->x_lo; ga.kw = d; ga.W2 = g->wp_lo;
    ga.bias_per_pos = c.embed_tables;
    rc |= gemm_tn(s, EPI_LOGITS_F32, ga); }
  return rc;
}

int gen_forward_impl(mb_gen* g, const int64_t* tokens, const int64_t* labels, const uint8_t* drop, float* logits,
                     int nb, hipStream_t s, float* attn = nullptr) {
  using namespace mb;
  const mb_gen_cfg& c = g->c;
  const int d = c.hidden, f = c.mlp, N = g->N, M = nb * N;
  auto attn_maps = [&](int l) {
    return attn ? attention_probs(s, g->qkv, attn + (size_t)l * nb * N * N, nb, N, d, c.heads) : 0;
  };
  int attn_rc = 0, gemm_rc = 0;
  int wdir = 0;
  auto walk_next = [&] { wdir ^= g->walk; return wdir; };
  const bool xlo = c.precision >= 1;
  const bool wm = g->mini_ok && c.precision >= 2;
  const bool xlo_all = xlo && !wm;
  auto xlo_layer = [&](int l) { return xlo && (xlo_all || 2 * l + 1 >= c.depth); };
  h16* const xlo_ffn = xlo ? g->x_lo : nullptr;
  h16* const xlo_qkv = xlo_all ? g->x_lo : nullptr;
  Fp4Rows f4x;
  if (wm) { f4x.x4 = g->x4.v; f4x.x4s = g->x4.s; f4x.nseq = nb; f4x.seq_rows = N; }
  auto lo_set = [&](GemmArgs& ga, const uint8_t* a4, const uint8_t* a4s, int widx) {
    if (!wm) return;
    ga.nlo = 1; ga.lo[0] = {a4, a4s, g->w4lo[widx], g->w4los[widx]};
  };
  auto xgemm = [&](GemmEpi epi, const h16* W, const float* bias, h16* out, int Nout, int widx) {
    GemmArgs ga{g->x_h16, W, bias, nullptr, nullptr, out, M, Nout, d, 0};
    if (wm) ga.seq_rows = N;
    lo_set(ga, g->x4.v, g->x4.s, widx);
    if (wm && epi == EPI_GELU_H16) { ga.out4 = g->h4.v; ga.out4_scale = g->h4.s; }
    if (((widx & 3) == 2 || xlo_all) && xlo_layer(widx >> 2)) { ga.K = 2 * d; ga.A2 = g->x_lo; ga.kw = d; }
    ga.sat = g->sat;
    ga.reverse = walk_next();
    gemm_rc |= gemm_tn(s, epi, ga, wm ? 257 : 0);
  };
  auto rgemm = [&](const h16* A, const h16* W, const float* bias, int K, int widx, const uint8_t* a4, const uint8_t* a4s, const float* ln_g, const float* ln_b) {
    GemmArgs ga{A, W, bias, g->y_f32, g->y_f32, nullptr, M, d, K, 0};
    if (ln_g) { ga.ln_stats = g->ln_stats; ga.ln_g = ln_g; ga.ln_b = ln_b; }
    if (wm) ga.seq_rows = N;
    lo_set(ga, a4, a4s, widx);
    ga.reverse = walk_next();
    gemm_rc |= gemm_tn(s, EPI_RES_F32, ga, wm ? 257 : 0);
  };
  {
    ProfScope p("embed_ln", s, true);
    EmbedArgs e{tokens, labels, drop, g->w_in, g->b_in, g->class_emb, g->pos, g->ln0g, g->ln0b,
                g->y_f32, g->x_h16, nb, c.seq, c.splits, g->gbits, d, c.nclass, g->tables};
    e.x_lo = c.depth ? (c.prenorm ? nullptr : xlo_qkv) : g->x_lo;
    e.f4 = f4x;
    embed_ln(s, e);
  }
  for (int l = 0; l < c.depth; ++l) {
    const mb_gen::Layer& L = g->layers[l];
    if (c.prenorm) { ProfScope p("layernorm", s, true); layernorm_rows(s, g->y_f32, L.ln1g, L.ln1b, 1e-12f, nullptr, g->x_h16, nullptr, M, d, xlo_qkv, f4x, walk_next(), N); }
    { ProfScope p("gemm_qkv", s, true); xgemm(EPI_H16, L.wqkv, L.bqkv, g->qkv, 3 * d, 4 * l); }
    { ProfScope p("attention", s, true); attention(s, g->qkv, g->att, nb, N, d, c.heads, wm ? g->att4.v : nullptr, wm ? g->att4.s : nullptr, walk_next()); }
    attn_rc |= attn_maps(l);
    { ProfScope p("gemm_attn_out", s, true);
      const bool re = !c.prenorm && l > 0;
      rgemm(g->att, L.wo, L.bo, d, 4 * l + 1, g->att4.v, g->att4.s, re ? g->layers[l - 1].ln2g : nullptr, re ? g->layers[l - 1].ln2b : nullptr); }
    { ProfScope p("layernorm", s, true);
      layernorm_rows(s, g->y_f32, c.prenorm ? L.ln2g : L.ln1g, c.prenorm ? L.ln2b : L.ln1b, 1e-12f, nullptr, g->x_h16, c.prenorm ? nullptr : g->ln_stats, M, d, xlo_layer(l) ? xlo_ffn : nullptr, f4x, walk_next(), N); }
    { ProfScope p("gemm_ffn_up", s, true); xgemm(EPI_GELU_H16, L.w1, L.b1, g->h, f, 4 * l + 2); }
    { ProfScope p("gemm_ffn_down", s, true);
      rgemm(g->h, L.w2, L.b2, f, 4 * l + 3, g->h4.v, g->h4.s, c.prenorm ? nullptr : L.ln1g, c.prenorm ? nullptr : L.ln1b); }
    if (!c.prenorm) { ProfScope p("layernorm", s, true);
      const bool last = l + 1 == c.depth;
      layernorm_rows(s, g->y_f32, L.ln2g, L.ln2b, 1e-12f, nullptr, g->x_h16, g->ln_stats, M, d, last ? g->x_lo : xlo_qkv, last ? Fp4Rows{} : f4x, walk_next(), N); }
  }
  if (c.prenorm) { ProfScope p("layernorm", s, true); layernorm_rows(s, g->y_f32, g->lnag, g->lnab, 1e-12f, nullptr, g->x_h16, nullptr, M, d, g->x_lo, Fp4Rows{}, walk_next(), N); }
  gemm_rc |= head_gemms(g, logits, M, s);
  if (int rc = launched()) return rc;
  if (attn_rc) return fail(-3, "attention maps: head dim %d / %d tokens not supported", d / c.heads, N);
  if (gemm_rc) return fail(-3, "a trunk GEMM of this forward (%d sequences x %d tokens, hidden %d, mlp %d; precision %d%s) is outside the half-tile "
                               "kernel's shapes: its correction mini-tiles cannot run", nb, N, d, f, c.precision, wm ? ", weight-correction mini-tiles" : "");
  return 0;
}

int gen_forward_pair_impl(mb_gen* g, const int64_t* tokens, const int64_t* labels, const uint8_t* drop, float* logits, int B, bool wmode, hipStream_t s) {
  using namespace mb;
  const mb_gen_cfg& c = g->c;
  const int d = c.hidden, f = c.mlp, N = g->N, nb = 2 * B, M = nb * N, P = B * N;
  int rc = 0;
  int wdir = 0;
  auto walk_next = [&] { wdir ^= g->walk; return wdir; };
  auto alo_on = [&](int gemm) { return wmode && c.precision >= 3 && ((g->alo_mask >> gemm) & 1); };
  auto f4_for = [&](bool feeds_ffn = false) {
    Fp4Rows f;
    if (wmode) {
      f.x4 = g->x4.v; f.x4s = g->x4.s; f.nseq = B; f.seq_rows = N;
      if (alo_on(feeds_ffn ? 2 : 0)) { f.xl4 = g->xl4.v; f.xl4s = g->xl4.s; }
    }
    return f;
  };
  auto pgemm = [&](GemmEpi epi, const h16* A, const h16* W, const float* bias, h16* out16, float* res, int Nout, int K, int widx, int lo,
                   const uint8_t* a4 = nullptr, const uint8_t* a4s = nullptr, const uint8_t* al4 = nullptr, const uint8_t* al4s = nullptr) {
    GemmArgs ga{A, W, bias, res, res, out16, M, Nout, K, 0};
    ga.pair_rows = P;
    ga.seq_rows = N;
    if (epi != EPI_RES_F32) ga.sat = g->sat;
    if (lo) {
      ga.nlo = lo; ga.lo[0] = {a4, a4s, g->w4lo[widx], g->w4los[widx]};
      if (lo == 2) ga.lo[1] = {al4, al4s, g->w4[widx], g->w4s[widx]};
    }
    ga.reverse = walk_next();
    return ga;
  };
  {
    ProfScope p("embed_ln", s, true);
    EmbedArgs e{tokens, labels, nullptr, g->w_in, g->b_in, g->class_emb, g->pos, g->ln0g, g->ln0b,
                g->y_f32, g->x_h16, B, c.seq, c.splits, g->gbits, d, c.nclass, g->tables};
    e.f4 = f4_for();
    if (embed_pair(s, e)) {
      e.drop = drop; e.nb = nb; e.f4 = Fp4Rows{};
      embed_ln(s, e);
      rc |= pairify_rows(s, g->y_f32, g->x_h16, P, d, f4_for(), walk_next(), N);
    }
  }
  if (c.prenorm && c.depth > 0) {
    ProfScope p("layernorm", s, true);
    rc |= layernorm_pair(s, g->y_f32, g->layers[0].ln1g, g->layers[0].ln1b, 1e-12f, g->x_h16, nullptr, P, d, f4_for(), walk_next(), N);
  }
  for (int l = 0; l < c.depth; ++l) {
    const mb_gen::Layer& L = g->layers[l];
    const int xlo_mode = wmode ? (alo_on(2) ? 2 : 1) : 0;
    { ProfScope p("gemm_qkv", s, true);
      GemmArgs ga = pgemm(EPI_H16, g->x_h16, L.wqkv, L.bqkv, g->qkv, nullptr, 3 * d, d, 4 * l, wmode ? (alo_on(0) ? 2 : 1) : 0, g->x4.v, g->x4.s, g->xl4.v, g->xl4.s);
      rc |= gemm_tn(s, EPI_H16, ga, 257); }
    const bool lo_o = alo_on(1), lo_h = alo_on(3);
    { ProfScope p("attention", s, true); rc |= attention_pair(s, g->qkv, g->att, B, N, d, c.heads, wmode ? g->att4.v : nullptr, wmode ? g->att4.s : nullptr,
                                                              lo_o ? g->attl4.v : nullptr, lo_o ? g->attl4.s : nullptr, walk_next()); }
    { ProfScope p("gemm_attn_out", s, true);
      GemmArgs ga = pgemm(EPI_RES_F32, g->att, L.wo, L.bo, nullptr, g->y_f32, d, d, 4 * l + 1, wmode ? (alo_on(1) ? 2 : 1) : 0, g->att4.v, g->att4.s, g->attl4.v, g->attl4.s);
      if (l > 0 && !c.prenorm) { ga.ln_stats = g->ln_stats; ga.ln_g = g->layers[l - 1].ln2g; ga.ln_b = g->layers[l - 1].ln2b; }
      rc |= gemm_tn(s, EPI_RES_F32, ga, 257); }
    { ProfScope p("layernorm", s, true);
      rc |= layernorm_pair(s, g->y_f32, c.prenorm ? L.ln2g : L.ln1g, c.prenorm ? L.ln2b : L.ln1b, 1e-12f, g->x_h16, c.prenorm ? nullptr : g->ln_stats, P, d, f4_for(true), walk_next(), N); }
    { ProfScope p("gemm_ffn_up", s, true);
      GemmArgs ga = pgemm(EPI_GELU_H16, g->x_h16, L.w1, L.b1, g->h, nullptr, f, d, 4 * l + 2, xlo_mode, g->x4.v, g->x4.s, g->xl4.v, g->xl4.s);
      if (wmode) { ga.out4 = g->h4.v; ga.out4_scale = g->h4.s; }
      if (lo_h) { ga.out4l = g->hl4.v; ga.out4l_scale = g->hl4.s; }
      rc |= gemm_tn(s, EPI_GELU_H16, ga, 257); }
    { ProfScope p("gemm_ffn_down", s, true);
      GemmArgs ga = pgemm(EPI_RES_F32, g->h, L.w2, L.b2, nullptr, g->y_f32, d, f, 4 * l + 3, wmode ? (alo_on(3) ? 2 : 1) : 0, g->h4.v, g->h4.s, g->hl4.v, g->hl4.s);
      if (!c.prenorm) { ga.ln_stats = g->ln_stats; ga.ln_g = L.ln1g; ga.ln_b = L.ln1b; }
      rc |= gemm_tn(s, EPI_RES_F32, ga, 257); }
    { ProfScope p("layernorm", s, true);
      if (c.prenorm) {
        if (l + 1 == c.depth) layernorm_rows(s, g->y_f32, g->lnag, g->lnab, 1e-12f, nullptr, g->x_h16, nullptr, M, d, g->x_lo, Fp4Rows{}, walk_next(), N);
        else rc |= layernorm_pair(s, g->y_f32, g->layers[l + 1].ln1g, g->layers[l + 1].ln1b, 1e-12f, g->x_h16, nullptr, P, d, f4_for(), walk_next(), N);
      }
      else if (l + 1 == c.depth) layernorm_rows(s, g->y_f32, L.ln2g, L.ln2b, 1e-12f, nullptr, g->x_h16, g->ln_stats, M, d, g->x_lo, Fp4Rows{}, walk_next(), N);
      else rc |= layernorm_pair(s, g->y_f32, L.ln2g, L.ln2b, 1e-12f, g->x_h16, g->ln_stats, P, d, f4_for(), walk_next(), N); }
  }
  rc |= head_gemms(g, logits, M, s);
  if (int lrc = launched()) return lrc;
  if (rc) return fail(-3, "differential CFG forward: a kernel refused the shape (%d pairs x %d tokens, hidden %d, mlp %d)", B, N, d, f);
  return 0;
}

int gen_forward_f32_impl(mb_gen* g, const int64_t* tokens, const int64_t* labels, const uint8_t* drop, float* logits, int nb, hipStream_t s) {
  using namespace mb;
  const mb_gen_cfg& c = g->c;
  const int d = c.hidden, f = c.mlp, N = g->N, M = nb * N;
  int rc = 0;
  auto gemm = [&](int epi, const float* A, const float* W, const float* bias, const float* res, float* out, int Nout, int K) {
    GemmF32Args ga{epi, A, W, bias, res, out, M, Nout, K};
    rc |= gemm_f32(s, ga);
  };
  auto ln = [&](const float* gamma, const float* beta) {
    ProfScope p("layernorm", s, true);
    layernorm_rows(s, g->y_f32, gamma, beta, 1e-12f, g->x_f32, nullptr, nullptr, M, d);
  };
  float* const stream = c.prenorm ? g->y_f32 : g->x_f32;
  {
    ProfScope p("embed_ln", s, true);
    EmbedArgs e{tokens, labels, drop, g->w_in, g->b_in, g->class_emb, g->pos, g->ln0g, g->ln0b,
                stream, nullptr, nb, c.seq, c.splits, g->gbits, d, c.nclass, g->tables};
    embed_ln(s, e);
  }
  for (int l = 0; l < c.depth; ++l) {
    const mb_gen::Layer& L = g->layers[l];
    const mb_gen::Layer32& W = g->layers32[l];
    if (c.prenorm) ln(L.ln1g, L.ln1b);
    { ProfScope p("gemm_qkv", s, true); gemm(F32_EPI_PLAIN, g->x_f32, W.wqkv, L.bqkv, nullptr, g->qkv32, 3 * d, d); }
    { ProfScope p("attention", s, true); rc |= attention_f32(s, g->qkv32, g->att32, nb, N, d, c.heads); }
    { ProfScope p("gemm_attn_out", s, true); gemm(F32_EPI_RES, g->att32, W.wo, L.bo, stream, g->y_f32, d, d); }
    ln(c.prenorm ? L.ln2g : L.ln1g, c.prenorm ? L.ln2b : L.ln1b);
    { ProfScope p("gemm_ffn_up", s, true); gemm(F32_EPI_GELU, g->x_f32, W.w1, L.b1, nullptr, g->h32, f, d); }
    { ProfScope p("gemm_ffn_down", s, true); gemm(F32_EPI_RES, g->h32, W.w2, L.b2, stream, g->y_f32, d, f); }
    if (!c.prenorm) ln(L.ln2g, L.ln2b);
  }
  if (c.prenorm) ln(g->lnag, g->lnab);
  { ProfScope p("gemm_head", s, true); gemm(F32_EPI_GELU, g->x_f32, g->wl32, g->bl, nullptr, g->y_f32, d, d); }
  ln(g->lnhg, g->lnhb);
  { ProfScope p("gemm_head", s, true);
    GemmF32Args ga{F32_EPI_LOGITS, g->x_f32, g->wp32, c.embed_tables ? g->bias_pos : g->bp, nullptr, logits, M, c.splits * g->C, d, N, c.embed_tables};
    rc |= gemm_f32(s, ga); }
  if (int lrc = launched()) return lrc;
  if (rc) return fail(-3, "fp32 reference forward: a kernel refused the shape (%d sequences x %d tokens, hidden %d, heads %d, mlp %d)", nb, N, d, c.heads, f);
  return 0;
}

int gen_forward_pass(mb_gen* g, const int64_t* tokens, const int64_t* labels, const uint8_t* drop, float* logits, int nb, hipStream_t s, float* attn = nullptr) {
  if (g->f32) return gen_forward_f32_impl(g, tokens, labels, drop, logits, nb, s);
  return gen_forward_impl(g, tokens, labels, drop, logits, nb, s, attn);
}

int gen_forward(mb_gen* g, const int64_t* tokens, const int64_t* labels, const uint8_t* drop, float* logits, int nb, hipStream_t s,
                float* attn = nullptr) {
  const int chunk = g->chunk_seqs;
  g_prof.begin_forward(true);
  if (nb <= chunk) return gen_forward_pass(g, tokens, labels, drop, logits, nb, s, attn);
  if (attn) return fail(-3, "attention maps are limited to %d sequences per call", chunk);
  const size_t P = (size_t)g->c.seq * g->c.splits;
  for (int b0 = 0; b0 < nb; b0 += chunk) {
    const int nc = nb - b0 < chunk ? nb - b0 : chunk;
    int rc = gen_forward_pass(g, tokens + (size_t)b0 * P, labels + b0, drop ? drop + b0 : nullptr, logits + (size_t)b0 * P * g->C, nc, s);
    if (rc) return rc;
  }
  return 0;
}

int gen_forward_cfg(mb_gen* g, const int64_t* tokens, const int64_t* labels, float* logits, int B, hipStream_t s) {
  const size_t P = (size_t)g->c.seq * g->c.splits;
  const bool pair = !g->f32 && g->pair_ok && g->c.precision >= 1;
  const bool wmode = pair && g->c.precision >= 2;
  const int chunk = g->chunk_seqs / 2;
  if (chunk < 1) return fail(-1, "engine holds %d sequences: too few for a guided forward", g->chunk_seqs);
  for (int b0 = 0; b0 < B; b0 += chunk) {
    const int nc = B - b0 < chunk ? B - b0 : chunk;
    HIP_TRY(hipMemcpyAsync(g->tok_cfg, tokens + (size_t)b0 * P, nc * P * sizeof(int64_t), hipMemcpyDeviceToDevice, s));
    if (!(pair && !g->c.embed_tables && g->c.bits <= 24))
      HIP_TRY(hipMemcpyAsync(g->tok_cfg + nc * P, tokens + (size_t)b0 * P, nc * P * sizeof(int64_t), hipMemcpyDeviceToDevice, s));
    if (!(nc == B && g->run.cfg_labels == labels && g->run.cfg_B == B)) {
      g->run.cfg_labels = nullptr;
      HIP_TRY(hipMemcpyAsync(g->lab_cfg, labels + b0, nc * sizeof(int64_t), hipMemcpyDeviceToDevice, s));
      HIP_TRY(hipMemcpyAsync(g->lab_cfg + nc, labels + b0, nc * sizeof(int64_t), hipMemcpyDeviceToDevice, s));
      HIP_TRY(hipMemsetAsync(g->drop_cfg, 0, nc, s));
      HIP_TRY(hipMemsetAsync(g->drop_cfg + nc, 1, nc, s));
    }
    float* out = (nc == B) ? logits : g->logits_tmp;
    if (b0 == 0) g_prof.begin_forward(false);
    int rc = pair ? gen_forward_pair_impl(g, g->tok_cfg, g->lab_cfg, g->drop_cfg, out, nc, wmode, s)
                  : gen_forward_pass(g, g->tok_cfg, g->lab_cfg, g->drop_cfg, out, 2 * nc, s);
    if (rc) return rc;
    if (nc != B) {
      HIP_TRY(hipMemcpyAsync(logits + (size_t)b0 * P * g->C, out, nc * P * g->C * sizeof(float), hipMemcpyDeviceToDevice, s));
      HIP_TRY(hipMemcpyAsync(logits + (size_t)(B + b0) * P * g->C, out + (size_t)nc * P * g->C, nc * P * g->C * sizeof(float), hipMemcpyDeviceToDevice, s));
    }
  }
  return 0;
}

}

extern "C" {

int mb_abi_version(void) { return MB_ABI_VERSION; }
const char* mb_last_error(void) { return mb::g_err.c_str(); }

int mb_prof_enable(int on) {
  if (!on) g_prof.drain();
  g_prof.on = on != 0;
  if (on) { g_prof.acc.clear(); g_prof.stride = on; g_prof.tick[0] = g_prof.tick[1] = 0; }
  return 0;
}
int mb_prof_read(char* buf, int buflen) {
  g_prof.drain();
  std::string out;
  char line[256];
  for (auto& kv : g_prof.acc) {
    snprintf(line, sizeof line, "%s %ld %.6f\n", g_prof.names[kv.first].c_str(), kv.second.first, kv.second.second);
    out += line;
  }
  if ((int)out.size() + 1 > buflen) return fail(-3, "mb_prof_read: buffer too small (%zu needed)", out.size() + 1);
  memcpy(buf, out.c_str(), out.size() + 1);
  return (int)out.size();
}

int mb_gen_create(const mb_gen_cfg* cfg, int max_seqs, mb_gen** out) {
  if (!cfg || !out || max_seqs <= 0) return fail(-1, "mb_gen_create: bad arguments");
  const mb_gen_cfg& c = *cfg;
  if (c.splits <= 0 || c.bits % c.splits) return fail(-1, "bits (%d) must be divisible by splits (%d)", c.bits, c.splits);
  if (c.bits > 24) return fail(-1, "bits > 24 is not supported");
  if (c.hidden % 64 || c.mlp % 64) return fail(-1, "hidden (%d) and mlp (%d) must be multiples of 64", c.hidden, c.mlp);
  if (c.hidden > 2048) return fail(-1, "hidden > 2048 is not supported");
  const int dh = c.heads > 0 ? c.hidden / c.heads : 0;
  if (c.heads <= 0 || c.hidden % c.heads || (dh != 32 && dh != 64)) return fail(-1, "hidden/heads must be 32 or 64 (got %d)", dh);
  if (c.seq < 1 || c.seq > 4096) return fail(-1, "seq = %d outside [1, 4096]", c.seq);
  if ((size_t)c.seq * c.splits > 8192) return fail(-1, "seq * splits = %zu exceeds the step kernel's 8192 positions", (size_t)c.seq * c.splits);
  const int C = 1 << (c.bits / c.splits);
  if (C > 4096 || (c.splits * C) % 4) return fail(-1, "unsupported group codebook size %d (the fused step kernel holds up to 4096 codes per group)", C);
  if ((c.prenorm != 0 && c.prenorm != 1) || (c.embed_tables != 0 && c.embed_tables != 1)) return fail(-1, "prenorm / embed_tables must be 0 or 1");
  if (c.embed_tables && c.splits > 8) return fail(-1, "embed_tables supports up to 8 token groups");
  if (c.precision < 0 || c.precision > MB_PREC_F32) return fail(-1, "precision must be 0 .. 5 (MB_PREC_FP16 / _DIFF / _WCORR / _ALO / _ALO_ALL / _F32)");
  const bool f32 = c.precision == MB_PREC_F32;
  mb_gen* g = new mb_gen();
  g->f32 = f32;
  g->c = c; g->max_seqs = max_seqs; g->N = c.seq + 1; g->gbits = c.bits / c.splits; g->C = C;
  (void)hipGetDevice(&g->device);
  const size_t widest = (size_t)(c.mlp > 3 * c.hidden ? c.mlp : 3 * c.hidden);
  const size_t max_rows = ((1ull << 32) - 1) / (4 * widest);
  g->chunk_seqs = (int)std::min<size_t>((size_t)max_seqs, std::max<size_t>(1, max_rows / g->N));
  const size_t d = c.hidden, f = c.mlp, M = (size_t)g->chunk_seqs * g->N;
  mb::DevArena& m = g->mem;
  g->layers.resize(c.depth);
  if (f32) g->layers32.resize(c.depth);
  else m.get(&g->split_tmp, 1);
  m.zeroed(&g->sat, 1);
  for (int l = 0; l < c.depth; ++l) {
    mb_gen::Layer& L = g->layers[l];
    if (f32) { mb_gen::Layer32& W = g->layers32[l]; m.get(&W.wqkv, 3 * d * d); m.get(&W.wo, d * d); m.get(&W.w1, f * d); m.get(&W.w2, d * f); }
    else { m.get(&L.wqkv, 3 * d * d); m.get(&L.wo, d * d); m.get(&L.w1, f * d); m.get(&L.w2, d * f); }
    m.get(&L.bqkv, 3 * d); m.get(&L.bo, d); m.get(&L.b1, f); m.get(&L.b2, d);
    m.get(&L.ln1g, d); m.get(&L.ln1b, d); m.get(&L.ln2g, d); m.get(&L.ln2b, d);
  }
  m.get(&g->w_in, d * c.bits); m.get(&g->b_in, d);
  if (c.prenorm) { m.get(&g->lnag, d); m.get(&g->lnab, d); }
  if (c.embed_tables) { m.get(&g->tables, (size_t)c.splits * (C + 1) * d); m.get(&g->bias_pos, (size_t)c.seq * c.splits * C); }
  m.get(&g->class_emb, (size_t)(c.nclass + 1) * d); m.get(&g->pos, (size_t)g->N * d);
  m.get(&g->ln0g, d); m.get(&g->ln0b, d);
  m.get(&g->bl, d); m.get(&g->lnhg, d); m.get(&g->lnhb, d); m.get(&g->bp, (size_t)c.splits * C);
  m.get(&g->y_f32, M * d);
  if (f32) {
    m.get(&g->wl32, d * d); m.get(&g->wp32, (size_t)c.splits * C * d);
    m.get(&g->x_f32, M * d); m.get(&g->qkv32, M * 3 * d); m.get(&g->att32, M * d); m.get(&g->h32, M * f);
  } else {
    m.get(&g->wl, d * d); m.get(&g->wl_lo, d * d);
    m.get(&g->wp, (size_t)c.splits * C * d); m.get(&g->head_scale, 2);
    if (!c.embed_tables) m.get(&g->wp_lo, (size_t)c.splits * C * d);
    m.get(&g->ln_stats, M * 2); m.get(&g->x_h16, M * d);
    m.get(&g->x_lo, M * d);
    m.get(&g->qkv, M * 3 * d); m.get(&g->att, M * d); m.get(&g->h, M * f);
  }
  g->mini_ok = !f32 && c.precision >= 2 && (c.seq == 256 || c.seq == 1024) && (c.hidden == 768 || c.hidden == 1024) && c.mlp % 256 == 0 && c.hidden / c.heads == 64;
  if (c.precision == 3) g->alo_mask = g->alo_mask_built = 6;
  if (c.precision == 4) g->alo_mask = g->alo_mask_built = 14;
  g->pair_ok = !f32 && c.precision >= 1 && (c.seq == 256 || c.seq == 1024) && (c.hidden == 768 || c.hidden == 1024) && c.mlp % 256 == 0 && g->chunk_seqs >= 2 &&
               (c.precision == 1 || g->mini_ok);
  if (g->mini_ok) {
    const size_t ntok = (size_t)g->chunk_seqs * c.seq;
    alloc_f4(m, &g->x4, M, d, ntok);
    alloc_f4(m, &g->att4, M, d, ntok);
    alloc_f4(m, &g->h4, M, f, ntok);
    if (g->alo_mask_built & 5) alloc_f4(m, &g->xl4, M, d, ntok);
    if (g->alo_mask_built & 2) alloc_f4(m, &g->attl4, M, d, ntok);
    if (g->alo_mask_built & 8) alloc_f4(m, &g->hl4, M, f, ntok);
    g->w4lo.assign((size_t)4 * c.depth, nullptr); g->w4los.assign((size_t)4 * c.depth, nullptr);
    g->w4.assign((size_t)4 * c.depth, nullptr); g->w4s.assign((size_t)4 * c.depth, nullptr);
    const size_t wn[4] = {3 * d * d, d * d, f * d, d * f};
    for (int i = 0; i < 4 * c.depth; ++i) {
      const size_t n = wn[i & 3];
      m.get(&g->w4lo[i], n / 2); m.get(&g->w4los[i], n / 128);
      if ((g->alo_mask_built >> (i & 3)) & 1) { m.get(&g->w4[i], n / 2); m.get(&g->w4s[i], n / 128); }
    }
  }
  const size_t P = (size_t)c.seq * c.splits, B = max_seqs;
  m.get(&g->tok_a, B * P); m.get(&g->tok_b, B * P); m.get(&g->tok_cfg, B * P);
  m.get(&g->pred, B * P); m.get(&g->codes, B * c.seq);
  m.get(&g->lab_cfg, B); m.get(&g->drop_cfg, B); m.get(&g->logits, B * P * C);
  m.get(&g->num_regen, B);
  if (g->chunk_seqs < max_seqs) m.get(&g->logits_tmp, (size_t)g->chunk_seqs * P * C);
  if (int rc = m.failed("mb_gen_create")) { delete g; return rc; }
  *out = g;
  return 0;
}

void mb_gen_destroy(mb_gen* g) { delete g; }

int mb_gen_load(mb_gen* g, const char* name, const float* data, const int64_t* shape, int ndim, mb_stream stream) {
  if (!g || !name || !data) return fail(-1, "mb_gen_load: bad arguments");
  hipStream_t s = (hipStream_t)stream;
  const mb_gen_cfg& c = g->c;
  const size_t d = c.hidden, f = c.mlp;
  size_t numel = 1;
  for (int i = 0; i < ndim; ++i) numel *= (size_t)shape[i];
  float* dst_f = nullptr; h16* dst_h = nullptr; size_t want = 0;
  int wrows = 0, wcols = 0, sidx = -1;
  int l = -1, sub = -1; char rest[96] = {0};
  std::string n(name);
  if (c.embed_tables && (n.rfind("prediction_layer.", 0) == 0 || n.rfind("input_proj.", 0) == 0))
    return fail(-2, "mb_gen_load: unknown checkpoint entry '%s' (embed_tables engine: tok_emb_list.* / bias.* instead)", name);
  if (sscanf(name, "transformer.layers.%d.%d.%95s", &l, &sub, rest) == 3) {
    if (l < 0 || l >= c.depth) return fail(-2, "layer index out of range in '%s'", name);
    mb_gen::Layer& L = g->layers[l];
    std::string r(rest);
    if (sub == 0) {
      if (r == "mha.in_proj_weight") { dst_h = L.wqkv; want = 3 * d * d; wrows = 3 * d; wcols = d; sidx = 4 * l; }
      else if (r == "mha.in_proj_bias") { dst_f = L.bqkv; want = 3 * d; }
      else if (r == "mha.out_proj.weight") { dst_h = L.wo; want = d * d; wrows = d; wcols = d; sidx = 4 * l + 1; }
      else if (r == "mha.out_proj.bias") { dst_f = L.bo; want = d; }
      else if (r == "norm.weight") { dst_f = L.ln1g; want = d; }
      else if (r == "norm.bias") { dst_f = L.ln1b; want = d; }
    } else if (sub == 1) {
      if (r == "net.0.weight") { dst_h = L.w1; want = f * d; wrows = f; wcols = d; sidx = 4 * l + 2; }
      else if (r == "net.0.bias") { dst_f = L.b1; want = f; }
      else if (r == "net.2.weight") { dst_h = L.w2; want = d * f; wrows = d; wcols = f; sidx = 4 * l + 3; }
      else if (r == "net.2.bias") { dst_f = L.b2; want = d; }
      else if (r == "norm.weight") { dst_f = L.ln2g; want = d; }
      else if (r == "norm.bias") { dst_f = L.ln2b; want = d; }
    }
  } else if (n == "pos_emb") { dst_f = g->pos; want = (size_t)g->N * d; }
  else if (n == "class_emb.weight") { dst_f = g->class_emb; want = (size_t)(c.nclass + 1) * d; }
  else if (n == "input_proj.weight") { dst_f = g->w_in; want = d * c.bits; }
  else if (n == "input_proj.bias") { dst_f = g->b_in; want = d; }
  else if (n == "first_layer.0.weight") { dst_f = g->ln0g; want = d; }
  else if (n == "first_layer.0.bias") { dst_f = g->ln0b; want = d; }
  else if (n == "last_layer.0.weight") { dst_h = g->wl; want = d * d; wrows = d; wcols = d; sidx = 4 * c.depth; }
  else if (n == "last_layer.0.bias") { dst_f = g->bl; want = d; }
  else if (n == "last_layer.2.weight") { dst_f = g->lnhg; want = d; }
  else if (n == "last_layer.2.bias") { dst_f = g->lnhb; want = d; }
  else if (n == "prediction_layer.weight") { dst_h = g->wp; want = (size_t)c.splits * g->C * d; wrows = c.splits * g->C; wcols = d; sidx = 4 * c.depth + 1; }
  else if (n == "prediction_layer.bias") { dst_f = g->bp; want = (size_t)c.splits * g->C; }
  else if (n == "bits_to_indices") return 0;
  else if (c.prenorm && n == "norm_after_transformer.weight") { dst_f = g->lnag; want = d; }
  else if (c.prenorm && n == "norm_after_transformer.bias") { dst_f = g->lnab; want = d; }
  else if (c.embed_tables) {
    int q = -1;
    if (sscanf(name, "tok_emb_list.%d.weight", &q) == 1 && n == "tok_emb_list." + std::to_string(q) + ".weight") {
      if (q < 0 || q >= c.splits) return fail(-2, "group index out of range in '%s'", name);
      const size_t rows = (size_t)g->C + 1;
      if (numel != rows * d) return fail(-4, "mb_gen_load: '%s' has %zu elements, expected %zu", name, numel, rows * d);
      HIP_TRY(hipMemcpyAsync(g->tables + (size_t)q * rows * d, data, numel * sizeof(float), hipMemcpyDeviceToDevice, s));
      if (g->f32) HIP_TRY(hipMemcpyAsync(g->wp32 + (size_t)q * g->C * d, data, (size_t)g->C * d * sizeof(float), hipMemcpyDeviceToDevice, s));
      else mb::cast_f32_to_h16(s, data, g->wp + (size_t)q * g->C * d, (size_t)g->C * d);
      g->loaded++;
      return 0;
    }
    if (sscanf(name, "bias.%d", &q) == 1 && n == "bias." + std::to_string(q)) {
      if (q < 0 || q >= c.splits) return fail(-2, "group index out of range in '%s'", name);
      if (numel != (size_t)c.seq * g->C) return fail(-4, "mb_gen_load: '%s' has %zu elements, expected %zu", name, numel, (size_t)c.seq * g->C);
      HIP_TRY(hipMemcpy2DAsync(g->bias_pos + (size_t)q * g->C, (size_t)c.splits * g->C * sizeof(float), data, (size_t)g->C * sizeof(float),
                               (size_t)g->C * sizeof(float), (size_t)c.seq, hipMemcpyDeviceToDevice, s));
      g->loaded++;
      return 0;
    }
  }
  if (g->f32 && sidx >= 0) {
    if (sidx < 4 * c.depth) { mb_gen::Layer32& W = g->layers32[sidx >> 2]; float* const w4[4] = {W.wqkv, W.wo, W.w1, W.w2}; dst_f = w4[sidx & 3]; }
    else dst_f = sidx == 4 * c.depth ? g->wl32 : g->wp32;
    dst_h = nullptr;
  }
  if (!dst_f && !dst_h) return fail(-2, "mb_gen_load: unknown checkpoint entry '%s'", name);
  if (numel != want) return fail(-4, "mb_gen_load: '%s' has %zu elements, expected %zu", name, numel, want);
  if (dst_f == g->w_in) mb::transpose_f32(s, data, g->w_in, (int)d, c.bits);
  else if (dst_h && dst_h == g->wl) mb::split_f32_to_h16_planes(s, data, g->wl, g->wl_lo, wrows, wcols, g->head_scale, g->split_tmp);
  else if (dst_h && dst_h == g->wp) mb::split_f32_to_h16_planes(s, data, g->wp, g->wp_lo, wrows, wcols, g->head_scale + 1, g->split_tmp);
  else if (dst_h) {
    mb::cast_f32_to_h16(s, data, dst_h, numel);
    if (g->mini_ok && sidx >= 0 && sidx < 4 * c.depth) {
      mb::w4lo_from_f32(s, data, g->w4lo[sidx], wrows, wcols, g->w4los[sidx]);
      if (g->w4[sidx]) mb::w4_from_f32(s, data, g->w4[sidx], wrows, wcols, g->w4s[sidx]);
    }
  }
  else HIP_TRY(hipMemcpyAsync(dst_f, data, numel * sizeof(float), hipMemcpyDeviceToDevice, s));
  g->loaded++;
  return 0;
}

int mb_gen_set_alo(mb_gen* g, int gemm_mask) {
  if (!g || gemm_mask < 0 || gemm_mask > 15) return fail(-1, "mb_gen_set_alo: mask outside [0, 15]");
  if (gemm_mask & ~g->alo_mask_built)
    return fail(-1, "mb_gen_set_alo: the handle was created (precision %d) with the activation-lo operands of GEMM mask %d only", g->c.precision, g->alo_mask_built);
  g->alo_mask = gemm_mask;
  return 0;
}

int mb_gen_set_walk(mb_gen* g, int mode) {
  if (!g || (mode != 0 && mode != 1)) return fail(-1, "mb_gen_set_walk: mode 0 (every launch front to back) or 1 (alternating)");
  g->walk = mode;
  return 0;
}

int mb_gen_saturation_count(mb_gen* g, unsigned* count, int reset, mb_stream stream) {
  if (!g || !count) return fail(-1, "mb_gen_saturation_count: null argument");
  return mb::read_counter("mb_gen_saturation_count", g->sat, count, reset, (hipStream_t)stream);
}

int mb_gen_forward(mb_gen* g, const int64_t* tokens, const int64_t* labels, const uint8_t* drop, float* logits,
                   int nb, mb_stream stream) {
  if (!g || !tokens || !labels || !logits) return fail(-1, "mb_gen_forward: null argument");
  if (nb <= 0 || nb > g->max_seqs) return fail(-1, "mb_gen_forward: nb=%d outside [1, %d]", nb, g->max_seqs);
  return gen_forward(g, tokens, labels, drop, logits, nb, (hipStream_t)stream);
}

int mb_gen_forward_cfg(mb_gen* g, const int64_t* tokens, const int64_t* labels, float* logits, int B, mb_stream stream) {
  if (!g || !tokens || !labels || !logits) return fail(-1, "mb_gen_forward_cfg: null argument");
  if (B <= 0 || 2 * B > g->max_seqs) return fail(-1, "mb_gen_forward_cfg: B=%d needs %d sequences, engine holds %d", B, 2 * B, g->max_seqs);
  return gen_forward_cfg(g, tokens, labels, logits, B, (hipStream_t)stream);
}

int mb_gen_forward_attn(mb_gen* g, const int64_t* tokens, const int64_t* labels, const uint8_t* drop, float* logits, float* attn,
                        int nb, mb_stream stream) {
  if (!g || !tokens || !labels || !logits || !attn) return fail(-1, "mb_gen_forward_attn: null argument");
  if (nb <= 0 || nb > g->max_seqs) return fail(-1, "mb_gen_forward_attn: nb=%d outside [1, %d]", nb, g->max_seqs);
  if (g->f32) return fail(-3, "mb_gen_forward_attn: attention maps are not available in the fp32 reference mode (precision %d)", (int)MB_PREC_F32);
  return gen_forward(g, tokens, labels, drop, logits, nb, (hipStream_t)stream, attn);
}

static int sample_step_checked(const char* who, const mb::StepArgs& a, const int64_t* tokens_in, const int32_t* num_regen, float mask_ratio, hipStream_t s) {
  if (!a.logits_c || (!a.seeds && (!a.exp_noise || !a.conf_noise)) || !tokens_in || !a.tokens) return fail(-1, "%s: null argument", who);
  if (tokens_in == a.tokens) return fail(-1, "%s: tokens_in and tokens_out must not alias", who);
  if (a.B <= 0 || a.P <= 0 || a.C <= 0) return fail(-1, "%s: bad sizes", who);
  ProfScope p(a.req ? "sample_step_requests" : a.seeds ? "sample_step_seeded" : num_regen ? "sample_step_edit" : "sample_step", s);
  if (mb::sample_step(s, a, tokens_in, num_regen, mask_ratio)) return fail(-1, "%s: C=%d or n*m=%d too large", who, a.C, a.P);
  return launched();
}

static int step_slots(int n, int m) { return n > 0 && m > 0 ? n * m : 0; }

int mb_sample_step(const float* logits_c, const float* logits_u, float scale, float temperature,
                   const float* exp_noise, const float* conf_noise, int k_mask_len, const int64_t* tokens_in,
                   int64_t* tokens_out, int64_t* pred_out, int B, int n, int m, int C, mb_stream stream) {
  mb::StepArgs a{};
  a.logits_c = logits_c; a.logits_u = logits_u; a.scale = scale; a.temperature = temperature;
  a.exp_noise = exp_noise; a.conf_noise = conf_noise; a.k_mask_len = k_mask_len;
  a.tokens = tokens_out; a.pred = pred_out; a.B = B; a.P = step_slots(n, m); a.C = C;
  return sample_step_checked("mb_sample_step", a, tokens_in, nullptr, 0.f, (hipStream_t)stream);
}

int mb_sample_step_edit(const float* logits_c, const float* logits_u, float scale, float temperature, const float* exp_noise, const float* conf_noise,
                        float mask_ratio, const int32_t* num_regen, const int64_t* tokens_in, int64_t* tokens_out, int64_t* pred_out, int B, int n, int m,
                        int C, mb_stream stream) {
  if (!num_regen) return fail(-1, "mb_sample_step_edit: null argument");
  mb::StepArgs a{};
  a.logits_c = logits_c; a.logits_u = logits_u; a.scale = scale; a.temperature = temperature;
  a.exp_noise = exp_noise; a.conf_noise = conf_noise;
  a.tokens = tokens_out; a.pred = pred_out; a.B = B; a.P = step_slots(n, m); a.C = C;
  return sample_step_checked("mb_sample_step_edit", a, tokens_in, num_regen, mask_ratio, (hipStream_t)stream);
}

int mb_sample_step_seeded(const float* logits_c, const float* logits_u, float scale, float temperature, const int64_t* seeds, int step,
                          float randomize_temperature, float conf_weight, float mask_ratio, const int32_t* num_regen, const int64_t* tokens_in,
                          int64_t* tokens_out, int64_t* pred_out, int B, int n, int m, int C, mb_stream stream) {
  if (!seeds || !num_regen) return fail(-1, "mb_sample_step_seeded: null argument");
  if (step < 0) return fail(-1, "mb_sample_step_seeded: step = %d is negative", step);
  if (pred_out && (pred_out == tokens_out || pred_out == tokens_in)) return fail(-1, "mb_sample_step_seeded: pred_out must not alias tokens_in or tokens_out");
  mb::StepArgs a{};
  a.logits_c = logits_c; a.logits_u = logits_u; a.scale = scale; a.temperature = temperature;
  a.seeds = seeds; a.step = step; a.rand_temp = randomize_temperature; a.conf_w = conf_weight;
  a.tokens = tokens_out; a.pred = pred_out; a.B = B; a.P = step_slots(n, m); a.C = C;
  return sample_step_checked("mb_sample_step_seeded", a, tokens_in, num_regen, mask_ratio, (hipStream_t)stream);
}

static_assert(sizeof(mb::RequestStep) == sizeof(mb_request_step) && sizeof(mb_request_step) == 24, "mb_request_step is the kernels' RequestStep");

int mb_sample_step_requests(const float* logits_c, const float* logits_u, const mb_request_step* table_row, const int64_t* seeds, const int32_t* num_regen,
                            const int64_t* tokens_in, int64_t* tokens_out, int64_t* pred_out, int B, int n, int m, int C, mb_stream stream) {
  if (!table_row || !seeds || !num_regen) return fail(-1, "mb_sample_step_requests: null argument");
  if (pred_out && (pred_out == tokens_out || pred_out == tokens_in)) return fail(-1, "mb_sample_step_requests: pred_out must not alias tokens_in or tokens_out");
  mb::StepArgs a{};
  a.logits_c = logits_c; a.logits_u = logits_u;
  a.seeds = seeds; a.req = (const mb::RequestStep*)table_row;
  a.tokens = tokens_out; a.pred = pred_out; a.B = B; a.P = step_slots(n, m); a.C = C;
  return sample_step_checked("mb_sample_step_requests", a, tokens_in, num_regen, 0.f, (hipStream_t)stream);
}

}

namespace {

struct RunNoise {
  const float* exp_noise = nullptr; const float* conf_noise = nullptr;
  const int64_t* seeds = nullptr; float rand_temp = 0.f; const float* conf_weight = nullptr;
};
struct RunSpec {
  const char* who = nullptr;
  int num_steps = 0, use_guidance = 0, step_begin = 0, step_end = 0;
  const float* scale = nullptr; const float* temperature = nullptr;
  const int* mask_len = nullptr; const float* mask_ratio = nullptr;
  const int64_t* init_tokens = nullptr;
  RunNoise noise;
};
struct RunOut { int64_t* step_tokens; int64_t* codes; float* img_nchw; uint8_t* img_nhwc_u8; };

const char* const kRunKind[3] = {"plain", "edit", "seeded"};
const char* const kStepEntry[3] = {"mb_sample_step", "mb_sample_step_edit", "mb_sample_step_seeded"};

template <class Plan>
RunSpec run_spec(const char* who, const Plan& p) {
  RunSpec r;
  r.who = who; r.num_steps = p.num_steps; r.use_guidance = p.use_guidance; r.step_begin = p.step_begin; r.step_end = p.step_end;
  r.scale = p.scale; r.temperature = p.temperature;
  return r;
}

int sample_run(mb_gen* g, mb_dec* d, const RunSpec& r, const int64_t* labels, int B, const RunOut& out, hipStream_t s) {
  const char* who = r.who;
  const RunNoise& nz = r.noise;
  const bool edit = r.mask_ratio != nullptr, seeded = nz.seeds != nullptr;
  const int num_steps = r.num_steps;
  if (!r.scale || !r.temperature || !(edit ? (const void*)r.mask_ratio : (const void*)r.mask_len) || num_steps <= 0) return fail(-1, "%s: incomplete plan", who);
  const mb_gen::Run::Id id{B, num_steps, r.use_guidance != 0, seeded ? 2 : edit ? 1 : 0};
  const int nbf = id.guided ? 2 * B : B;
  if (B <= 0 || nbf > g->max_seqs) return fail(-1, "%s: B=%d needs %d sequences, engine holds %d", who, B, nbf, g->max_seqs);
  if (!d && (out.img_nchw || out.img_nhwc_u8)) return fail(-1, "%s: image requested without a decoder", who);
  const mb_gen_cfg& c = g->c;
  const int n = c.seq, m = c.splits, C = g->C;
  const size_t P = (size_t)n * m;
  const int s0 = r.step_end > 0 ? r.step_begin : 0, s1 = r.step_end > 0 ? r.step_end : num_steps;
  if (s0 < 0 || s1 > num_steps || s0 >= s1) return fail(-1, "%s: step chunk [%d, %d) outside [0, %d)", who, s0, s1, num_steps);
  mb_gen::Run& run = g->run;
  if (s0 == 0) {
    if (r.init_tokens) mb::edit_load_tokens(s, r.init_tokens, g->tok_a, g->num_regen, B, (int)P, C);
    else {
      mb::fill_i64(s, g->tok_a, (int64_t)C, (size_t)B * P);
      if (seeded) mb::edit_load_tokens(s, g->tok_a, nullptr, g->num_regen, B, (int)P, C);
    }
    run.id = id;
  }
  else if (!(run.id == id && run.next == s0))
    return fail(-1, "%s: step chunk [%d, %d) of a %d-step %s run with B = %d does not continue the run in progress (next step %d of %d, B = %d, %s %s run)",
                who, s0, s1, num_steps, kRunKind[id.kind], B, run.next, run.id.steps, run.id.B, run.id.kind == 1 ? "an" : "a", kRunKind[run.id.kind]);
  run.next = -1;
  int64_t* cur = (s0 & 1) ? g->tok_b : g->tok_a;
  int64_t* nxt = (s0 & 1) ? g->tok_a : g->tok_b;
  int64_t* last_pred = g->pred;
  struct CfgReady { mb_gen::Run& run; ~CfgReady() { run.cfg_labels = nullptr; } } cfg_ready{run};
  run.cfg_labels = nullptr;
  mb::StepArgs a{};
  a.logits_c = g->logits; a.B = B; a.P = (int)P; a.C = C;
  a.seeds = nz.seeds; a.rand_temp = nz.rand_temp;
  for (int i = s0; i < s1; ++i) {
    int rc;
    if (id.guided && (r.scale[i] != 0.0f || (!g->f32 && g->pair_ok && c.precision >= 4))) {
      rc = gen_forward_cfg(g, cur, labels, g->logits, B, s);
      a.logits_u = g->logits + (size_t)B * P * C;
      if (B <= g->chunk_seqs / 2) { run.cfg_labels = labels; run.cfg_B = B; }
    } else {
      rc = gen_forward(g, cur, labels, nullptr, g->logits, B, s);
      a.logits_u = nullptr;
    }
    if (rc) return rc;
    const size_t k = (size_t)(i - s0);
    a.scale = r.scale[i]; a.temperature = r.temperature[i];
    a.tokens = nxt; a.pred = out.step_tokens ? out.step_tokens + k * B * P : g->pred;
    if (seeded) { a.step = i; a.conf_w = nz.conf_weight[i]; }
    else { a.exp_noise = nz.exp_noise + k * B * P * C; a.conf_noise = nz.conf_noise + k * B * P; }
    if (!edit) a.k_mask_len = r.mask_len[i];
    rc = sample_step_checked(kStepEntry[id.kind], a, cur, edit ? g->num_regen : nullptr, edit ? r.mask_ratio[i] : 0.f, s);
    if (rc) return rc;
    last_pred = a.pred;
    int64_t* t = cur; cur = nxt; nxt = t;
  }
  if (s1 < num_steps) {
    if (int rc = launched()) return rc;
    run.next = s1;
    return 0;
  }
  int64_t* codes = out.codes ? out.codes : g->codes;
  mb::combine_groups(s, last_pred, codes, (size_t)B * n, m, g->gbits);
  if (d) {
    int rc = mb_dec_decode(d, codes, out.img_nchw, out.img_nhwc_u8, B, (mb_stream)s);
    if (rc) return rc;
  }
  return launched();
}

int sample_requests_run(mb_gen* g, mb_dec* d, const mb_request_plan& plan, const int64_t* labels, int B, const int64_t* init_tokens, const int64_t* seeds,
                        const RunOut& out, hipStream_t s) {
  const char* who = "mb_sample_requests";
  const int S = plan.num_steps;
  if (!plan.active || !plan.table || !labels || !seeds) return fail(-1, "%s: null argument", who);
  if (S <= 0 || B <= 0) return fail(-1, "%s: bad sizes (num_steps = %d, B = %d)", who, S, B);
  for (int t = 0; t < S; ++t) {
    if (plan.active[t] < 1 || plan.active[t] > B) return fail(-1, "%s: active[%d] = %d outside [1, %d]", who, t, plan.active[t], B);
    if (t && plan.active[t] < plan.active[t - 1])
      return fail(-1, "%s: active[] is not non-decreasing (active[%d] = %d after %d): order the requests by num_steps descending", who, t, plan.active[t], plan.active[t - 1]);
  }
  if (plan.active[S - 1] != B) return fail(-1, "%s: active[%d] = %d, but all %d requests run the last step", who, S - 1, plan.active[S - 1], B);
  if (!d && (out.img_nchw || out.img_nhwc_u8)) return fail(-1, "%s: image requested without a decoder", who);
  if (!g) return fail(-1, "%s: null argument (no generator handle)", who);
  const bool guided = plan.use_guidance != 0;
  const int nbf = guided ? 2 * B : B;
  if (nbf > g->max_seqs) return fail(-1, "%s: B=%d needs %d sequences, engine holds %d", who, B, nbf, g->max_seqs);
  const mb_gen_cfg& c = g->c;
  const int n = c.seq, m = c.splits, C = g->C;
  const size_t P = (size_t)n * m;
  mb_gen::Run& run = g->run;
  run.next = -1;
  if (init_tokens) mb::edit_load_tokens(s, init_tokens, g->tok_a, g->num_regen, B, (int)P, C);
  else {
    mb::fill_i64(s, g->tok_a, (int64_t)C, (size_t)B * P);
    mb::edit_load_tokens(s, g->tok_a, nullptr, g->num_regen, B, (int)P, C);
  }
  HIP_TRY(hipMemcpyAsync(g->tok_b, g->tok_a, (size_t)B * P * sizeof(int64_t), hipMemcpyDeviceToDevice, s));
  int64_t* cur = g->tok_a;
  int64_t* nxt = g->tok_b;
  int64_t* last_pred = g->pred;
  struct CfgReady { mb_gen::Run& run; ~CfgReady() { run.cfg_labels = nullptr; } } cfg_ready{run};
  run.cfg_labels = nullptr;
  mb::StepArgs a{};
  a.logits_c = g->logits; a.P = (int)P; a.C = C;
  a.seeds = seeds;
  for (int t = 0; t < S; ++t) {
    const int Bt = plan.active[t];
    int rc;
    if (guided) {
      rc = gen_forward_cfg(g, cur, labels, g->logits, Bt, s);
      a.logits_u = g->logits + (size_t)Bt * P * C;
      if (Bt <= g->chunk_seqs / 2) { run.cfg_labels = labels; run.cfg_B = Bt; }
      else run.cfg_labels = nullptr;
    } else {
      rc = gen_forward(g, cur, labels, nullptr, g->logits, Bt, s);
      a.logits_u = nullptr;
    }
    if (rc) return rc;
    a.B = Bt;
    a.req = (const mb::RequestStep*)plan.table + (size_t)t * B;
    a.tokens = nxt; a.pred = out.step_tokens ? out.step_tokens + (size_t)t * B * P : g->pred;
    rc = sample_step_checked(who, a, cur, g->num_regen, 0.f, s);
    if (rc) return rc;
    last_pred = a.pred;
    int64_t* tmp = cur; cur = nxt; nxt = tmp;
  }
  int64_t* codes = out.codes ? out.codes : g->codes;
  mb::combine_groups(s, last_pred, codes, (size_t)B * n, m, g->gbits);
  if (d) {
    int rc = mb_dec_decode(d, codes, out.img_nchw, out.img_nhwc_u8, B, (mb_stream)s);
    if (rc) return rc;
  }
  return launched();
}

}

extern "C" {

int mb_sample_requests(mb_gen* g, mb_dec* d, const mb_request_plan* plan, const int64_t* labels, int B, const int64_t* init_tokens, const int64_t* seeds,
                       int64_t* step_tokens, int64_t* tokens_out, float* img_nchw, uint8_t* img_nhwc_u8, mb_stream stream) {
  if (!plan) return fail(-1, "mb_sample_requests: null argument");
  return sample_requests_run(g, d, *plan, labels, B, init_tokens, seeds, RunOut{step_tokens, tokens_out, img_nchw, img_nhwc_u8}, (hipStream_t)stream);
}

int mb_sample(mb_gen* g, mb_dec* d, const mb_sample_plan* plan, const int64_t* labels, int B, const float* exp_noise,
              const float* conf_noise, int64_t* step_tokens, int64_t* tokens_out, float* img_nchw,
              uint8_t* img_nhwc_u8, mb_stream stream) {
  if (!plan || !g || !labels || !exp_noise || !conf_noise) return fail(-1, "mb_sample: null argument");
  RunSpec r = run_spec("mb_sample", *plan);
  r.mask_len = plan->mask_len;
  r.noise.exp_noise = exp_noise; r.noise.conf_noise = conf_noise;
  return sample_run(g, d, r, labels, B, RunOut{step_tokens, tokens_out, img_nchw, img_nhwc_u8}, (hipStream_t)stream);
}

int mb_sample_edit(mb_gen* g, mb_dec* d, const mb_edit_plan* plan, const int64_t* labels, int B, const int64_t* init_tokens, const float* exp_noise,
                   const float* conf_noise, int64_t* step_tokens, int64_t* tokens_out, float* img_nchw, uint8_t* img_nhwc_u8, mb_stream stream) {
  if (!plan || !plan->mask_ratio) return fail(-1, "mb_sample_edit: %s", plan ? "incomplete plan" : "null argument");
  if (!g || !labels || !exp_noise || !conf_noise || !init_tokens) return fail(-1, "mb_sample_edit: null argument");
  RunSpec r = run_spec("mb_sample_edit", *plan);
  r.mask_ratio = plan->mask_ratio;
  r.init_tokens = init_tokens;
  r.noise.exp_noise = exp_noise; r.noise.conf_noise = conf_noise;
  return sample_run(g, d, r, labels, B, RunOut{step_tokens, tokens_out, img_nchw, img_nhwc_u8}, (hipStream_t)stream);
}

int mb_sample_seeded(mb_gen* g, mb_dec* d, const mb_edit_plan* plan, const int64_t* labels, int B, const int64_t* init_tokens, const int64_t* seeds,
                     float randomize_temperature, const float* conf_weight, int64_t* step_tokens, int64_t* tokens_out, float* img_nchw,
                     uint8_t* img_nhwc_u8, mb_stream stream) {
  if (!plan || !plan->mask_ratio) return fail(-1, "mb_sample_seeded: %s", plan ? "incomplete plan" : "null argument");
  if (!seeds || !conf_weight || !g || !labels) return fail(-1, "mb_sample_seeded: null argument");
  RunSpec r = run_spec("mb_sample_seeded", *plan);
  r.mask_ratio = plan->mask_ratio;
  r.init_tokens = init_tokens;
  r.noise.seeds = seeds; r.noise.rand_temp = randomize_temperature; r.noise.conf_weight = conf_weight;
  return sample_run(g, d, r, labels, B, RunOut{step_tokens, tokens_out, img_nchw, img_nhwc_u8}, (hipStream_t)stream);
}

}

struct mb_session {
  int n = 0, m = 0, C = 0, gbits = 0, cap = 0, max_steps = 0;
  bool guided = false, allocated = false;
  size_t P = 0;
  struct Row { uint64_t ticket; int local_step, N; };
  std::vector<Row> rows;
  uint64_t next_ticket = 0;
  int64_t* tok[2] = {nullptr, nullptr};
  int cur = 0;
  int64_t *pred = nullptr, *codes_all = nullptr, *codes = nullptr;
  mb::SessionRows st{};
  mb::RequestStep* row = nullptr;
  int* plan = nullptr;
  bool cfg_dirty = true;
  mb::DevArena mem;
};

namespace {

int session_allocate(mb_session* s) {
  if (s->allocated) return 0;
  mb::DevArena& m = s->mem;
  const size_t cap = (size_t)s->cap;
  m.get(&s->tok[0], cap * s->P); m.get(&s->tok[1], cap * s->P); m.get(&s->pred, cap * s->P);
  m.get(&s->codes_all, cap * s->n); m.get(&s->codes, cap * s->n);
  m.get(&s->st.label, cap); m.get(&s->st.seed, cap);
  m.get(&s->st.num_regen, cap); m.get(&s->st.slot, cap); m.zeroed(&s->st.local_step, cap); m.zeroed(&s->st.N, cap);
  m.get(&s->st.pool, cap * s->max_steps);
  m.get(&s->row, cap); m.get(&s->plan, mb::session_plan_ints(s->cap));
  if (int rc = m.failed("mb_session_admit")) return rc;
  std::vector<int> iota(cap);
  for (size_t r = 0; r < cap; ++r) iota[r] = (int)r;
  HIP_TRY(hipMemcpy(s->st.slot, iota.data(), cap * sizeof(int), hipMemcpyHostToDevice));
  s->st.cap = s->cap; s->st.max_steps = s->max_steps;
  s->allocated = true;
  return 0;
}

}

extern "C" {

int mb_session_create(int seq, int splits, int bits, int max_active, int max_steps, int use_guidance, mb_session** out) {
  if (!out) return fail(-1, "mb_session_create: null argument");
  if (max_active < 1 || max_steps < 1) return fail(-1, "mb_session_create: bad sizes (max_active = %d, max_steps = %d: both at least 1)", max_active, max_steps);
  if (seq < 1 || splits < 1 || bits < 1 || bits > 24 || bits % splits || (size_t)seq * splits > 8192 || (1 << (bits / splits)) > 4096)
    return fail(-1, "mb_session_create: seq = %d, splits = %d, bits = %d is no generator configuration (mb_gen_create)", seq, splits, bits);
  if ((size_t)max_active * max_steps > ((size_t)1 << 27)) return fail(-1, "mb_session_create: max_active * max_steps = %zu schedule records exceed 2^27", (size_t)max_active * max_steps);
  mb_session* s = new mb_session();
  s->n = seq; s->m = splits; s->gbits = bits / splits; s->C = 1 << s->gbits; s->P = (size_t)seq * splits;
  s->cap = max_active; s->max_steps = max_steps; s->guided = use_guidance != 0;
  s->rows.reserve(max_active);
  *out = s;
  return 0;
}

void mb_session_destroy(mb_session* s) { delete s; }

int mb_session_active(const mb_session* s) { return s ? (int)s->rows.size() : -1; }

int mb_session_due(const mb_session* s) {
  if (!s) return -1;
  int due = 0;
  for (const mb_session::Row& r : s->rows) due += r.local_step + 1 == r.N;
  return due;
}

int mb_session_admit(mb_session* s, int K, const int64_t* labels, const int64_t* seeds, const int* num_steps, const mb_request_step* schedule,
                     const int64_t* init_tokens, uint64_t* tickets, mb_stream stream) {
  const char* who = "mb_session_admit";
  if (K < 1) return fail(-1, "%s: bad sizes (K = %d)", who, K);
  if (!s || !labels || !seeds || !num_steps || !schedule || !tickets) return fail(-1, "%s: null argument", who);
  for (int k = 0; k < K; ++k)
    if (num_steps[k] < 1 || num_steps[k] > s->max_steps) return fail(-1, "%s: num_steps[%d] = %d outside [1, %d]", who, k, num_steps[k], s->max_steps);
  const int A = (int)s->rows.size();
  if (K > s->cap - A) return fail(-1, "%s: %d active + %d new requests exceed max_active = %d", who, A, K, s->cap);
  if (int rc = session_allocate(s)) return rc;
  hipStream_t st = (hipStream_t)stream;
  mb::session_admit(st, s->st, s->tok[s->cur], init_tokens, num_steps, labels, seeds, (const mb::RequestStep*)schedule, A, K, (int)s->P, s->C);
  for (int k = 0; k < K; ++k) {
    tickets[k] = s->next_ticket;
    s->rows.push_back({s->next_ticket++, 0, num_steps[k]});
  }
  s->cfg_dirty = true;
  return launched();
}

int mb_session_tick(mb_session* s, mb_gen* g, mb_dec* d, int64_t* pred_out, int64_t* codes_out, float* img_nchw, uint8_t* img_nhwc_u8, uint64_t* finished,
                    uint64_t* ran, int* num_finished, mb_stream stream) {
  const char* who = "mb_session_tick";
  if (!s || !num_finished) return fail(-1, "%s: null argument", who);
// ... 68 lines not shown
```

maskbit_amd/csrc/mb_kernels.h:

```cpp
#pragma once
#include "mb_common.h"

namespace mb {

enum GemmEpi {
  EPI_H16 = 0,
  EPI_GELU_H16 = 1,
  EPI_RES_F32 = 2,
  EPI_GELU_F32 = 3,
  EPI_LOGITS_F32 = 4,
};
struct GemmArgs {
  const h16* A;
  const h16* W;
  const float* bias;
  const float* residual;
  float* out_f32;
  h16* out_h16;
  int M, N, K;
  int period;
  const float* scale = nullptr;
  const float* ln_stats = nullptr;
  const float* ln_g = nullptr;
  const float* ln_b = nullptr;
  int bias_per_pos = 0;
  const h16* A2 = nullptr;
  int kw = 0;
  const h16* W2 = nullptr;
  int pair_rows = 0;
  int seq_rows = 0;
  uint8_t* out4 = nullptr;
  uint8_t* out4_scale = nullptr;
  uint8_t* out4l = nullptr;
  uint8_t* out4l_scale = nullptr;
  struct LoSet { const uint8_t* A4; const uint8_t* a_scale; const uint8_t* W4; const uint8_t* w_scale; };
  LoSet lo[2] = {};
  int nlo = 0;
  unsigned* sat = nullptr;
  int reverse = 0;
};
__host__ __device__ inline size_t w4_packed_offset(int n, int k, int K) {
  const int r = n & 15, c = (k & 127) >> 5;
  return ((size_t)(n >> 4) * (K >> 7) + (k >> 7)) * 1024 + r * 64 + ((c ^ ((r >> 1) & 3)) << 4) + ((k & 31) >> 1);
}
__host__ __device__ inline size_t w4_scale_index(int n, int j, int K) {
  return (((size_t)(n >> 6) * (K >> 7) + j) * 16 + (n & 15)) * 4 + ((n >> 4) & 3);
}
__host__ __device__ inline size_t fp4_scale_index(int blk, int nseq, int seq, int r, int groups = 4) {
  return (((size_t)blk * nseq + seq) * groups + (r >> 6)) * 64 + (r & 15) * 4 + ((r >> 4) & 3);
}
__host__ __device__ inline int walk_tile(int vb, int ntiles, int reverse) { return xcd_remap(reverse ? ntiles - 1 - vb : vb, ntiles); }
__host__ __device__ inline int xcd_chunk_start(int x, int n) { return xcd_remap(x, n); }
__host__ __device__ inline int walk_seq(int slot, int n, int grp, int reverse) {
  if (reverse) slot = n - 1 - slot;
  const int q = n >> 3, r = n & 7;
  for (int lo = 0, before = 0;; lo += grp) {
    const int a = q + 1 - lo < grp ? (q + 1 - lo > 0 ? q + 1 - lo : 0) : grp;
    const int b = q - lo < grp ? (q - lo > 0 ? q - lo : 0) : grp;
    const int step = r * a + (8 - r) * b;
    if (slot < before + step) {
      int s = slot - before, x;
      if (s < r * a) { x = s / a; s -= x * a; }
      else { s -= r * a; x = s / b; s -= x * b; x += r; }
      return xcd_chunk_start(x, n) + lo + s;
    }
    before += step;
  }
}
inline int walk_group(int seq_rows, bool pair) { const int tps = (seq_rows - 1) / (pair ? 128 : 256); return tps >= 8 ? 1 : tps >= 1 ? 8 / tps : 8; }
struct WalkRows { int seq_rows, grp, reverse; };
__host__ __device__ inline int walk_row(int slot, int rows, const WalkRows& w) {
  if (w.reverse) slot = rows - 1 - slot;
  const int ss = slot / w.seq_rows;
  return walk_seq(ss, rows / w.seq_rows, w.grp, 0) * w.seq_rows + (slot - ss * w.seq_rows);
}
inline WalkRows walk_rows(int rows, int seq_rows, bool pair, int reverse) {
  if (seq_rows <= 0 || rows % seq_rows) return WalkRows{rows, 8, reverse ? 1 : 0};
  return WalkRows{seq_rows, walk_group(seq_rows, pair), reverse ? 1 : 0};
}

int gemm_tn(hipStream_t s, GemmEpi epi, const GemmArgs& a, int variant = 0);
bool gemm_ht_supported(GemmEpi epi, const GemmArgs& a);
void gemm_ht(hipStream_t s, GemmEpi epi, const GemmArgs& a, int mt);
void set_cu_count(int n);

enum GemmF32Epi {
  F32_EPI_PLAIN = 0,
  F32_EPI_GELU = 1,
  F32_EPI_RES = 2,
  F32_EPI_LOGITS = 3,
};
struct GemmF32Args {
  int epi;
  const float* A; const float* W; const float* bias; const float* residual; float* out;
  int M, N, K;
  int period = 0, bias_per_pos = 0;
};
int gemm_f32(hipStream_t s, const GemmF32Args& a);
int attention_f32(hipStream_t s, const float* qkv, float* out, int nb, int N, int d, int heads);

void w4_from_f32(hipStream_t s, const float* src, uint8_t* dst4, int N, int K, uint8_t* scale_out);
void w4lo_from_f32(hipStream_t s, const float* src, uint8_t* dst4, int N, int K, uint8_t* scale_out);

struct Fp4Rows { uint8_t* x4 = nullptr; uint8_t* x4s = nullptr; uint8_t* xl4 = nullptr; uint8_t* xl4s = nullptr; int nseq = 0; int seq_rows = 257; };

void layernorm_rows(hipStream_t s, const float* y, const float* gamma, const float* beta, float eps,
                    float* x_f32, h16* x_h16, float* stats, int M, int d, h16* x_lo = nullptr,
                    const Fp4Rows& f4 = Fp4Rows{}, int reverse = 0, int seq_rows = 0);

int layernorm_pair(hipStream_t s, const float* y, const float* gamma, const float* beta, float eps, h16* x_h16, float* stats, int P, int d,
                   const Fp4Rows& f4 = Fp4Rows{}, int reverse = 0, int seq_rows = 0);
int pairify_rows(hipStream_t s, const float* x32, h16* x_h16, int P, int d, const Fp4Rows& f4 = Fp4Rows{}, int reverse = 0, int seq_rows = 0);

struct EmbedArgs {
  const int64_t* tokens;
  const int64_t* labels;
  const uint8_t* drop;
  const float* w_in;
  const float* b_in;
  const float* class_emb;
  const float* pos;
  const float* gamma; const float* beta;
  float* x_f32; h16* x_h16;
  int nb, seq, m, gbits, d, nclass;
  const float* tables = nullptr;
  h16* x_lo = nullptr;
  Fp4Rows f4;
};
void embed_ln(hipStream_t s, const EmbedArgs& a);
int embed_pair(hipStream_t s, const EmbedArgs& a);
void transpose_f32(hipStream_t s, const float* src , float* dst , int rows, int cols);

void attention(hipStream_t s, const h16* qkv, h16* out, int nb, int N, int d, int heads,
               uint8_t* out4 = nullptr, uint8_t* out4s = nullptr, int reverse = 0);
int attention_pair(hipStream_t s, const h16* qkv, h16* out, int P, int N, int d, int heads, uint8_t* out4 = nullptr, uint8_t* out4s = nullptr,
                   uint8_t* out4l = nullptr, uint8_t* out4ls = nullptr, int reverse = 0);
int attention_probs(hipStream_t s, const h16* qkv, float* out, int nb, int N, int d, int heads);

struct RequestStep { float scale, temperature, mask_ratio, rand_temp, conf_w; int32_t step; };
struct StepArgs {
  const float* logits_c; const float* logits_u;
  float scale, temperature;
  const float* exp_noise;
  const float* conf_noise;
  int k_mask_len;
  int64_t* tokens;
  int64_t* pred;
  int B, P , C;
  const int64_t* seeds = nullptr;
  int step = 0;
  float rand_temp = 0.f, conf_w = 0.f;
  const RequestStep* req = nullptr;
};
int sample_step(hipStream_t s, const StepArgs& a, const int64_t* tokens_in, const int* num_regen = nullptr, float mask_ratio = 0.f);
int seeded_noise_dump(hipStream_t s, const int64_t* seeds, int step, float rand_temp, float conf_w, float* exp_u, float* exp_noise, float* conf_u,
                      float* conf_noise, int B, int P, int C);

void fill_i64(hipStream_t s, int64_t* dst, int64_t value, size_t n);

void edit_load_tokens(hipStream_t s, const int64_t* src, int64_t* dst, int* num_regen, int B, int P, int C);
void edit_init(hipStream_t s, const int64_t* codes, const uint8_t* regen, int64_t* tokens, int* num_regen, int B, int n, int m, int gbits);
void edit_token_mask(hipStream_t s, const uint8_t* pixel_mask, uint8_t* token_mask, int B, int H, int W, int st);
int edit_composite(hipStream_t s, const float* gen, const float* orig, const uint8_t* pixel_mask, float* out_nchw, uint8_t* out_u8, int B, int C, int H, int W);
void combine_groups(hipStream_t s, const int64_t* tokens , int64_t* codes , size_t rows, int m, int gbits);

struct SessionRows {
  int64_t* label; int64_t* seed;
  int* num_regen; int* slot; int* local_step; int* N;
  RequestStep* pool;
  int cap, max_steps;
};
struct AdmitBatch { enum { MAX = 64 }; int n[MAX]; int off[MAX]; };
inline size_t session_plan_ints(int cap) { return 2 + 3 * (size_t)cap; }
void session_row_table(hipStream_t s, const SessionRows& st, RequestStep* row, int A);
void session_admit(hipStream_t s, const SessionRows& st, int64_t* tokens, const int64_t* init_tokens, const int* num_steps, const int64_t* labels,
                   const int64_t* seeds, const RequestStep* sched, int A, int K, int P, int C);
void session_retire(hipStream_t s, const SessionRows& st, int* plan, int64_t* tokens, const int64_t* pred, int64_t* codes_all, int64_t* codes_out,
                    int A, int n, int m, int gbits, int k, int moves);

void cast_f32_to_h16(hipStream_t s, const float* src, h16* dst, size_t n);
void split_f32_to_h16_planes(hipStream_t s, const float* src, h16* hi, h16* lo, int N, int K, float* scale_out, unsigned* tmp);

}
```

maskbit_amd/csrc/norm_embed.hip:

```cpp
#include "mb_kernels.h"

namespace mb {

constexpr int MAXS = 32;

template <int NV>
__device__ __forceinline__ void fp4_row_store(const float4* v, int lane, uint8_t* x4row, uint8_t* scales, int nseq, int seq, int tok, int groups) {
#pragma unroll
  for (int q = 0; q < NV; ++q) {
    float am = fmaxf(fmaxf(fabsf(v[q].x), fabsf(v[q].y)), fmaxf(fabsf(v[q].z), fabsf(v[q].w)));
    am = row16_max(am);
    if ((lane & 15) == 0) scales[fp4_scale_index(q * 4 + (lane >> 4), nseq, seq, tok, groups)] = (uint8_t)fp4_scale_byte_nosat(am);
    *(uint16_t*)(x4row + q * 128 + lane * 2) = (uint16_t)fp4_pack4(v[q].x, v[q].y, v[q].z, v[q].w, fp4_scale_mul_nosat(am));
  }
}
template <int NV>
__device__ __forceinline__ void fp4_rows_out(const Fp4Rows& f4, float4* v, int lane, int row, int d) {
  const int seq = row / f4.seq_rows, tok = row - seq * f4.seq_rows, groups = (f4.seq_rows - 1) >> 6;
  if (tok == f4.seq_rows - 1) return;
  if (f4.x4) fp4_row_store<NV>(v, lane, f4.x4 + (size_t)row * 2 * d, f4.x4s, f4.nseq, seq, tok, groups);
  if (f4.xl4) {
#pragma unroll
    for (int q = 0; q < NV; ++q)
      v[q] = make_float4(v[q].x - (float)to_h(v[q].x), v[q].y - (float)to_h(v[q].y), v[q].z - (float)to_h(v[q].z), v[q].w - (float)to_h(v[q].w));
    fp4_row_store<NV>(v, lane, f4.xl4 + (size_t)row * 2 * d, f4.xl4s, f4.nseq, seq, tok, groups);
  }
}

template <int NV>
__device__ __forceinline__ void ln_finish(float4* v, const float* sc, int ns, int d, int lane,
                                          const float* __restrict__ gamma, const float* __restrict__ beta,
                                          float eps, float* xo, h16* xb, float* st = nullptr, h16* xl = nullptr,
                                          const Fp4Rows* f4 = nullptr, int row = 0) {
  constexpr bool VEC = NV > 0;
  constexpr int nv = NV;
  float s = 0.f;
  if (VEC) {
#pragma unroll
    for (int q = 0; q < nv; ++q) s += (v[q].x + v[q].y) + (v[q].z + v[q].w);
  }
  else     { for (int q = 0; q < ns; ++q) s += sc[q]; }
  const float mean = wave_sum(s) / (float)d;
  float ss = 0.f;
  if (VEC) {
#pragma unroll
    for (int q = 0; q < nv; ++q) {
      const float a = v[q].x - mean, b = v[q].y - mean, c = v[q].z - mean, e = v[q].w - mean;
      ss += (a * a + b * b) + (c * c + e * e);
    }
  } else {
    for (int q = 0; q < ns; ++q) { const int c = lane + q * 64; if (c < d) { const float a = sc[q] - mean; ss += a * a; } }
  }
  const float rstd = rsqrtf(wave_sum(ss) / (float)d + eps);
  if (st && lane == 0) *(float2*)st = make_float2(mean, rstd);
  if (VEC) {
#pragma unroll
    for (int q = 0; q < nv; ++q) {
      const int c = q * 256 + lane * 4;
      const float4 g = *(const float4*)(gamma + c), b = *(const float4*)(beta + c);
      float4 o;
      o.x = ln_affine(v[q].x, mean, rstd, g.x, b.x); o.y = ln_affine(v[q].y, mean, rstd, g.y, b.y);
      o.z = ln_affine(v[q].z, mean, rstd, g.z, b.z); o.w = ln_affine(v[q].w, mean, rstd, g.w, b.w);
      if (xo) *(float4*)(xo + c) = o;
      const h16x4 hi = {to_h(o.x), to_h(o.y), to_h(o.z), to_h(o.w)};
      if (xb) *(h16x4*)(xb + c) = hi;
      if (xl) *(h16x4*)(xl + c) = h16x4{to_h(o.x - (float)hi[0]), to_h(o.y - (float)hi[1]), to_h(o.z - (float)hi[2]), to_h(o.w - (float)hi[3])};
      if (f4) v[q] = o;
    }
    if constexpr (VEC) { if (f4) fp4_rows_out<NV>(*f4, v, lane, row, d); }
  } else {
    for (int q = 0; q < ns; ++q) {
      const int c = lane + q * 64;
      if (c < d) {
        const float o = ln_affine(sc[q], mean, rstd, gamma[c], beta[c]);
        if (xo) xo[c] = o;
        if (xb) xb[c] = to_h(o);
        if (xl) xl[c] = to_h(o - (float)to_h(o));
      }
    }
  }
}

template <int NV>
__global__ __launch_bounds__(256) void ln_rows_kernel(const float* __restrict__ y, const float* __restrict__ gamma,
                                                      const float* __restrict__ beta, float eps, float* x_f32,
                                                      h16* x_h16, float* stats, int M, int d, h16* x_lo, Fp4Rows f4, WalkRows wk) {
  const int lane = threadIdx.x & 63;
  const int slot = blockIdx.x * 4 + __builtin_amdgcn_readfirstlane(threadIdx.x >> 6);
  if (slot >= M) return;
  const int row = walk_row(slot, M, wk);
  const float* yr = y + (size_t)row * d;
  constexpr bool VEC = NV > 0;
  float4 v[VEC ? NV : 1]; float sc[VEC ? 1 : MAXS];
  const int ns = (d + 63) / 64;
  if (VEC) {
#pragma unroll
    for (int q = 0; q < NV; ++q) v[q] = *(const float4*)(yr + q * 256 + lane * 4);
  }
  else     { for (int q = 0; q < ns; ++q) { const int c = lane + q * 64; sc[q] = c < d ? yr[c] : 0.f; } }
  ln_finish<NV>(v, sc, ns, d, lane, gamma, beta, eps, x_f32 ? x_f32 + (size_t)row * d : nullptr,
                 x_h16 ? x_h16 + (size_t)row * d : nullptr, stats ? stats + (size_t)row * 2 : nullptr,
                 x_lo ? x_lo + (size_t)row * d : nullptr,
                 (f4.x4 || f4.xl4) ? &f4 : nullptr, row);
}

template <int NV>
__device__ __forceinline__ float2 ln_normalize(float4* v, int d, const float* __restrict__ gamma, const float* __restrict__ beta, float eps, int lane) {
  float s = 0.f;
#pragma unroll
  for (int q = 0; q < NV; ++q) s += (v[q].x + v[q].y) + (v[q].z + v[q].w);
  const float mean = wave_sum(s) / (float)d;
  float ss = 0.f;
#pragma unroll
  for (int q = 0; q < NV; ++q) {
    const float a = v[q].x - mean, b = v[q].y - mean, c = v[q].z - mean, e = v[q].w - mean;
    ss += (a * a + b * b) + (c * c + e * e);
  }
  const float rstd = rsqrtf(wave_sum(ss) / (float)d + eps);
#pragma unroll
  for (int q = 0; q < NV; ++q) {
    const int c = q * 256 + lane * 4;
    const float4 g = *(const float4*)(gamma + c), b = *(const float4*)(beta + c);
    v[q] = make_float4(ln_affine(v[q].x, mean, rstd, g.x, b.x), ln_affine(v[q].y, mean, rstd, g.y, b.y),
                       ln_affine(v[q].z, mean, rstd, g.z, b.z), ln_affine(v[q].w, mean, rstd, g.w, b.w));
  }
  return make_float2(mean, rstd);
}

template <int NV>
__device__ __forceinline__ void pair_store(float4* xc, const float4* xu, int lane, h16* oc, h16* ou, const Fp4Rows& f4, int row, int d) {
#pragma unroll
  for (int q = 0; q < NV; ++q) {
    const int c = q * 256 + lane * 4;
    *(h16x4*)(oc + c) = h16x4{to_h(xc[q].x), to_h(xc[q].y), to_h(xc[q].z), to_h(xc[q].w)};
    *(h16x4*)(ou + c) = h16x4{to_h(xu[q].x - xc[q].x), to_h(xu[q].y - xc[q].y), to_h(xu[q].z - xc[q].z), to_h(xu[q].w - xc[q].w)};
  }
  if (f4.x4 || f4.xl4) fp4_rows_out<NV>(f4, xc, lane, row, d);
}

template <int NV>
__global__ __launch_bounds__(256) void ln_pair_kernel(const float* __restrict__ y, const float* __restrict__ gamma, const float* __restrict__ beta, float eps,
                                                      h16* __restrict__ x_h16, float* __restrict__ stats, int P, int d, Fp4Rows f4, WalkRows wk) {
  const int lane = threadIdx.x & 63;
  const int slot = blockIdx.x * 4 + __builtin_amdgcn_readfirstlane(threadIdx.x >> 6);
  if (slot >= P) return;
  const int row = walk_row(slot, P, wk);
  float4 vc[NV], vu[NV];
#pragma unroll
  for (int q = 0; q < NV; ++q) { vc[q] = *(const float4*)(y + (size_t)row * d + q * 256 + lane * 4); vu[q] = *(const float4*)(y + (size_t)(row + P) * d + q * 256 + lane * 4); }
  const float2 sc = ln_normalize<NV>(vc, d, gamma, beta, eps, lane), su = ln_normalize<NV>(vu, d, gamma, beta, eps, lane);
  if (stats && lane == 0) { *(float2*)(stats + 2 * (size_t)row) = sc; *(float2*)(stats + 2 * (size_t)(row + P)) = su; }
  pair_store<NV>(vc, vu, lane, x_h16 + (size_t)row * d, x_h16 + (size_t)(row + P) * d, f4, row, d);
}

template <int NV>
__global__ __launch_bounds__(256) void pairify_kernel(const float* __restrict__ x32, h16* __restrict__ x_h16, int P, int d, Fp4Rows f4, WalkRows wk) {
  const int lane = threadIdx.x & 63;
  const int slot = blockIdx.x * 4 + __builtin_amdgcn_readfirstlane(threadIdx.x >> 6);
  if (slot >= P) return;
  const int row = walk_row(slot, P, wk);
  float4 vc[NV], vu[NV];
#pragma unroll
  for (int q = 0; q < NV; ++q) { vc[q] = *(const float4*)(x32 + (size_t)row * d + q * 256 + lane * 4); vu[q] = *(const float4*)(x32 + (size_t)(row + P) * d + q * 256 + lane * 4); }
  pair_store<NV>(vc, vu, lane, x_h16 + (size_t)row * d, x_h16 + (size_t)(row + P) * d, f4, row, d);
}

int layernorm_pair(hipStream_t s, const float* y, const float* gamma, const float* beta, float eps, h16* x_h16, float* stats, int P, int d,
                   const Fp4Rows& f4, int reverse, int seq_rows) {
  dim3 grid((P + 3) / 4), block(256);
  const WalkRows wk = walk_rows(P, seq_rows, true, reverse);
  if (d == 1024) hipLaunchKernelGGL(ln_pair_kernel<4>, grid, block, 0, s, y, gamma, beta, eps, x_h16, stats, P, d, f4, wk);
  else if (d == 768) hipLaunchKernelGGL(ln_pair_kernel<3>, grid, block, 0, s, y, gamma, beta, eps, x_h16, stats, P, d, f4, wk);
  else return -1;
  return 0;
}
int pairify_rows(hipStream_t s, const float* x32, h16* x_h16, int P, int d, const Fp4Rows& f4, int reverse, int seq_rows) {
  dim3 grid((P + 3) / 4), block(256);
  const WalkRows wk = walk_rows(P, seq_rows, true, reverse);
  if (d == 1024) hipLaunchKernelGGL(pairify_kernel<4>, grid, block, 0, s, x32, x_h16, P, d, f4, wk);
  else if (d == 768) hipLaunchKernelGGL(pairify_kernel<3>, grid, block, 0, s, x32, x_h16, P, d, f4, wk);
  else return -1;
  return 0;
}

void layernorm_rows(hipStream_t s, const float* y, const float* gamma, const float* beta, float eps,
                    float* x_f32, h16* x_h16, float* stats, int M, int d, h16* x_lo, const Fp4Rows& f4, int reverse, int seq_rows) {
  dim3 grid((M + 3) / 4), block(256);
  const WalkRows wk = walk_rows(M, seq_rows, false, reverse);
  if (d == 1024) hipLaunchKernelGGL(ln_rows_kernel<4>, grid, block, 0, s, y, gamma, beta, eps, x_f32, x_h16, stats, M, d, x_lo, f4, wk);
  else if (d == 768) hipLaunchKernelGGL(ln_rows_kernel<3>, grid, block, 0, s, y, gamma, beta, eps, x_f32, x_h16, stats, M, d, x_lo, f4, wk);
  else hipLaunchKernelGGL(ln_rows_kernel<0>, grid, block, 0, s, y, gamma, beta, eps, x_f32, x_h16, stats, M, d, x_lo, Fp4Rows{}, wk);
}

constexpr int MAXBITS = 24;

template <int NV>
__global__ __launch_bounds__(256) void embed_ln_kernel(EmbedArgs a) {
  const int lane = threadIdx.x & 63;
  const int row = blockIdx.x * 4 + (threadIdx.x >> 6);
  const int N = a.seq + 1;
  if (row >= a.nb * N) return;
  const int sq = row / N, t = row - sq * N;
  const int d = a.d, K = a.m * a.gbits;
  uint32_t plus = 0, live = 0;
  const float* cls = nullptr;
  const float* trow[8] = {};
  if (t < a.seq) {
    for (int g = 0; g < a.m; ++g) {
      const int64_t idx = a.tokens[((size_t)sq * a.seq + t) * a.m + g];
      if (a.tables && g < 8) {
        const int64_t nrow = ((int64_t)1 << a.gbits) + 1;
        const int64_t ix = idx < 0 ? 0 : (idx >= nrow ? nrow - 1 : idx);
        trow[g] = a.tables + ((size_t)g * nrow + (size_t)ix) * d;
      }
      const uint32_t gm = (1u << a.gbits) - 1u;
      if (idx != ((int64_t)1 << a.gbits)) { live |= gm << (g * a.gbits); plus |= ((uint32_t)idx & gm) << (g * a.gbits); }
    }
  } else {
    int64_t lab = a.labels[sq];
    if (a.drop && a.drop[sq]) lab = a.nclass;
    lab = lab < 0 ? 0 : (lab > a.nclass ? a.nclass : lab);
    cls = a.class_emb + (size_t)lab * d;
  }
  const float* pos = a.pos + (size_t)t * d;
  constexpr bool VEC = NV > 0;
  float4 v[VEC ? NV : 1]; float sc[VEC ? 1 : MAXS];
  const int ns = (d + 63) / 64;
  if (VEC) {
#pragma unroll
    for (int q = 0; q < NV; ++q) {
      const int c = q * 256 + lane * 4;
      float4 e = cls ? *(const float4*)(cls + c) : (a.tables ? make_float4(0.f, 0.f, 0.f, 0.f) : *(const float4*)(a.b_in + c));
      if (!cls && a.tables) {
#pragma unroll
        for (int g = 0; g < 8; ++g)
          if (g < a.m) { const float4 w = *(const float4*)(trow[g] + c); e.x += w.x; e.y += w.y; e.z += w.z; e.w += w.w; }
      } else if (!cls) {
#pragma unroll
        for (int j = 0; j < MAXBITS; ++j) {
          if (j < K) {
            const float4 w = *(const float4*)(a.w_in + (size_t)j * d + c);
            const float sj = ((live >> j) & 1u) ? (((plus >> j) & 1u) ? 1.f : -1.f) : 0.f;
            e.x = fmaf(sj, w.x, e.x); e.y = fmaf(sj, w.y, e.y); e.z = fmaf(sj, w.z, e.z); e.w = fmaf(sj, w.w, e.w);
          }
        }
      }
      const float4 p = *(const float4*)(pos + c);
      v[q] = make_float4(e.x + p.x, e.y + p.y, e.z + p.z, e.w + p.w);
    }
  } else {
    for (int q = 0; q < ns; ++q) {
      const int c = lane + q * 64;
      float e = 0.f;
      if (c < d) {
        if (cls) e = cls[c];
        else if (a.tables) {
          for (int g = 0; g < a.m && g < 8; ++g) e += trow[g][c];
        } else {
          e = a.b_in[c];
          for (int j = 0; j < K; ++j) {
            const float sj = ((live >> j) & 1u) ? (((plus >> j) & 1u) ? 1.f : -1.f) : 0.f;
            e = fmaf(sj, a.w_in[(size_t)j * d + c], e);
          }
        }
        e += pos[c];
      }
      sc[q] = e;
    }
  }
  ln_finish<NV>(v, sc, ns, d, lane, a.gamma, a.beta, 1e-12f, a.x_f32 + (size_t)row * d, a.x_h16 ? a.x_h16 + (size_t)row * d : nullptr, nullptr,
                 a.x_lo ? a.x_lo + (size_t)row * d : nullptr,
                 (a.f4.x4 || a.f4.xl4) ? &a.f4 : nullptr, row);
}

template <int NV>
__global__ __launch_bounds__(256) void embed_pair_kernel(EmbedArgs a) {
  const int lane = threadIdx.x & 63;
  const int row = blockIdx.x * 4 + (threadIdx.x >> 6);
  const int N = a.seq + 1, P = a.nb * N;
  if (row >= P) return;
  const int sq = row / N, t = row - sq * N;
  const int d = a.d, K = a.m * a.gbits;
  uint32_t plus = 0, live = 0;
  const float* cls = nullptr;
  if (t < a.seq) {
    for (int g = 0; g < a.m; ++g) {
      const int64_t idx = a.tokens[((size_t)sq * a.seq + t) * a.m + g];
      const uint32_t gm = (1u << a.gbits) - 1u;
      if (idx != ((int64_t)1 << a.gbits)) { live |= gm << (g * a.gbits); plus |= ((uint32_t)idx & gm) << (g * a.gbits); }
    }
  } else {
    int64_t lab = a.labels[sq];
    lab = lab < 0 ? 0 : (lab > a.nclass ? a.nclass : lab);
    cls = a.class_emb + (size_t)lab * d;
  }
  const float* pos = a.pos + (size_t)t * d;
  float4 vc[NV], vu[NV];
#pragma unroll
  for (int q = 0; q < NV; ++q) {
    const int c = q * 256 + lane * 4;
    float4 e = cls ? *(const float4*)(cls + c) : *(const float4*)(a.b_in + c);
    if (!cls) {
#pragma unroll
      for (int j = 0; j < MAXBITS; ++j) {
        if (j < K) {
          const float4 w = *(const float4*)(a.w_in + (size_t)j * d + c);
          const float sj = ((live >> j) & 1u) ? (((plus >> j) & 1u) ? 1.f : -1.f) : 0.f;
          e.x = fmaf(sj, w.x, e.x); e.y = fmaf(sj, w.y, e.y); e.z = fmaf(sj, w.z, e.z); e.w = fmaf(sj, w.w, e.w);
        }
      }
    }
    const float4 p = *(const float4*)(pos + c);
    vc[q] = make_float4(e.x + p.x, e.y + p.y, e.z + p.z, e.w + p.w);
    if (cls) {
      const float4 eu = *(const float4*)(a.class_emb + (size_t)a.nclass * d + c);
      vu[q] = make_float4(eu.x + p.x, eu.y + p.y, eu.z + p.z, eu.w + p.w);
    }
  }
  ln_normalize<NV>(vc, d, a.gamma, a.beta, 1e-12f, lane);
  if (cls) ln_normalize<NV>(vu, d, a.gamma, a.beta, 1e-12f, lane);
  else {
#pragma unroll
    for (int q = 0; q < NV; ++q) vu[q] = vc[q];
  }
#pragma unroll
  for (int q = 0; q < NV; ++q) {
    const int c = q * 256 + lane * 4;
    *(float4*)(a.x_f32 + (size_t)row * d + c) = vc[q];
    *(float4*)(a.x_f32 + (size_t)(row + P) * d + c) = vu[q];
  }
  pair_store<NV>(vc, vu, lane, a.x_h16 + (size_t)row * d, a.x_h16 + (size_t)(row + P) * d, a.f4, row, d);
}

int embed_pair(hipStream_t s, const EmbedArgs& a) {
  if (a.tables || a.m * a.gbits > MAXBITS) return -1;
  const int rows = a.nb * (a.seq + 1);
  dim3 grid((rows + 3) / 4), block(256);
  if (a.d == 1024) hipLaunchKernelGGL(embed_pair_kernel<4>, grid, block, 0, s, a);
  else if (a.d == 768) hipLaunchKernelGGL(embed_pair_kernel<3>, grid, block, 0, s, a);
  else return -1;
  return 0;
}

void embed_ln(hipStream_t s, const EmbedArgs& a) {
// ... 17 lines not shown
```

maskbit_amd/csrc/sampling.hip:

```cpp
#include "mb_kernels.h"

namespace mb {

__device__ __forceinline__ float cfg_combine(float c, float u, float scale) {
#pragma clang fp contract(off)
  const float d = c - u;
  const float m = scale * d;
  return c + m;
}

struct Philox4 { uint32_t w[4]; };
__device__ __forceinline__ Philox4 philox4x32_10(uint32_t c0, uint32_t c1, uint32_t c2, uint32_t c3, uint32_t k0, uint32_t k1) {
#pragma unroll
  for (int r = 0; r < 10; ++r) {
    const uint32_t hi0 = __umulhi(0xD2511F53u, c0), lo0 = 0xD2511F53u * c0;
    const uint32_t hi1 = __umulhi(0xCD9E8D57u, c2), lo1 = 0xCD9E8D57u * c2;
    c0 = hi1 ^ c1 ^ k0; c1 = lo1; c2 = hi0 ^ c3 ^ k1; c3 = lo0;
    k0 += 0x9E3779B9u; k1 += 0xBB67AE85u;
  }
  return Philox4{{c0, c1, c2, c3}};
}
__device__ __forceinline__ float seeded_noise(uint64_t seed, int step, int slot, int c, bool conf, float rand_temp, float conf_w, float* u_out) {
#pragma clang fp contract(off)
  const Philox4 r = philox4x32_10(conf ? 0u : (uint32_t)c >> 2, (uint32_t)slot, (uint32_t)step, conf ? 1u : 0u, (uint32_t)seed, (uint32_t)(seed >> 32));
  const int k = conf ? 0 : c & 3;
  const uint32_t x = k == 0 ? r.w[0] : k == 1 ? r.w[1] : k == 2 ? r.w[2] : r.w[3];
  const float u = (float)((x >> 8) | 1u) * 0x1p-24f;
  if (u_out) *u_out = u;
  const float q = -logf(u);
  if (!conf) return q;
  const float g = -logf(q);
  const float t = g * rand_temp;
  return t * conf_w;
}

template <int CPL, bool SEEDED, bool REQ = false>
__global__ __launch_bounds__(256) void sample_rows_kernel(StepArgs a, const int64_t* __restrict__ tokens_in) {
  static_assert(SEEDED || !REQ, "the per-sample records go with the seeded noise");
  const int C = a.C;
  const int lane = threadIdx.x & 63, wave = threadIdx.x >> 6;
  const int64_t mask_tok = (int64_t)C;
  const size_t nrows = (size_t)a.B * a.P;
#pragma unroll 1
  for (int it = 0; it < 4; ++it) {
    const size_t row = (size_t)blockIdx.x * 16 + wave * 4 + it;
    if (row >= nrows) return;
    const float* lc = a.logits_c + row * C;
    const float* lu = a.logits_u ? a.logits_u + row * C : nullptr;
    const float* qn = SEEDED ? nullptr : a.exp_noise + row * C;
    uint64_t seed = 0; int slot = 0;
    float scale = a.scale, temperature = a.temperature, rand_temp = a.rand_temp, conf_w = a.conf_w;
    int step = a.step;
    if constexpr (SEEDED) {
      const size_t b = row / (size_t)a.P;
      seed = (uint64_t)a.seeds[b];
      slot = (int)(row - b * (size_t)a.P);
      if constexpr (REQ) {
        const RequestStep rs = a.req[__builtin_amdgcn_readfirstlane((int)b)];
        scale = rs.scale; temperature = rs.temperature; step = rs.step; rand_temp = rs.rand_temp; conf_w = rs.conf_w;
      }
    }
    float l[CPL];
    float mx = -INFINITY;
#pragma unroll
    for (int i = 0; i < CPL; ++i) {
      const int c = lane + 64 * i;
      float v = -INFINITY;
      if (c < C) {
        v = lc[c];
        if (lu) v = cfg_combine(v, lu[c], scale);
        v = v / temperature;
      }
      l[i] = v;
      mx = fmaxf(mx, v);
    }
    mx = wave_max(mx);
    float sum = 0.f;
#pragma unroll
    for (int i = 0; i < CPL; ++i) { l[i] = (lane + 64 * i < C) ? expf(l[i] - mx) : 0.f; sum += l[i]; }
    sum = wave_sum(sum);
    float psum = 0.f;
#pragma unroll
    for (int i = 0; i < CPL; ++i) { l[i] = l[i] / sum; psum += l[i]; }
    psum = wave_sum(psum);
    float best = -INFINITY; int bi = 0x7fffffff;
#pragma clang loop unroll(full)
    for (int i = 0; i < CPL; ++i) {
      const int c = lane + 64 * i;
      if (c < C) {
        float q;
        if constexpr (SEEDED) {
          int cc = c;
          if constexpr (CPL >= 32) asm volatile("" : "+v"(cc));
          q = seeded_noise(seed, step, slot, cc, false, 0.f, 0.f, nullptr);
        }
        else q = qn[c];
        const float ratio = (l[i] / psum) / q;
        if (ratio > best) { best = ratio; bi = c; }
      }
    }
#pragma unroll
    for (int o = 32; o > 0; o >>= 1) {
      const float ob = __shfl_xor(best, o); const int oi = __shfl_xor(bi, o);
      if (ob > best || (ob == best && oi < bi)) { best = ob; bi = oi; }
    }
    const int64_t tin = tokens_in[row];
    const bool masked = tin == mask_tok;
    const int pred = masked ? bi : (int)tin;
    float pv = 0.f;
#pragma unroll
    for (int i = 0; i < CPL; ++i) if (pred == lane + 64 * i) pv = l[i];
    pv = __shfl(pv, pred & 63);
    if (lane == 0) {
      float cn;
      if constexpr (SEEDED) cn = seeded_noise(seed, step, slot, 0, true, rand_temp, conf_w, nullptr);
      else cn = a.conf_noise[row];
      const float conf = (masked ? logf(pv) : INFINITY) + cn;
      a.tokens[row] = (int64_t)(((uint64_t)(uint32_t)pred << 32) | (uint64_t)__float_as_uint(conf));
    }
  }
}

template <bool EDIT, bool REQ = false>
__global__ __launch_bounds__(1024) void sample_thresh_kernel(StepArgs a, const int64_t* __restrict__ tokens_in, float ratio, const int* __restrict__ num_regen) {
  extern __shared__ float sm[];
  const int P = a.P;
  float* conf_s = sm;
  int* pred_s = (int*)(sm + P);
  int* cnt_s = pred_s + P;
  float* thr_s = (float*)(cnt_s + 16);
  const int tid = threadIdx.x, lane = tid & 63, wave = tid >> 6, nw = blockDim.x >> 6;
  const int b = blockIdx.x;
  const int64_t mask_tok = (int64_t)a.C;
  if constexpr (REQ) ratio = a.req[b].mask_ratio;
  const int64_t* tin = EDIT ? tokens_in + (size_t)b * P : tokens_in;
  int mycnt = 0;
  for (int p = tid; p < P; p += blockDim.x) mycnt += tin[p] == mask_tok;
  mycnt = (int)wave_sum((float)mycnt);
  if (lane == 0) cnt_s[wave] = mycnt;
  if (tid == 0) *thr_s = -INFINITY;
  for (int p = tid; p < P; p += blockDim.x) {
    const uint64_t v = (uint64_t)a.tokens[(size_t)b * P + p];
    conf_s[p] = __uint_as_float((uint32_t)v);
    pred_s[p] = (int)(uint32_t)(v >> 32);
  }
  __syncthreads();
  int nm = 0;
  for (int w = 0; w < nw; ++w) nm += cnt_s[w];
  const int mask_len = EDIT ? (int)floorf(__fmul_rn(ratio, (float)num_regen[b])) : a.k_mask_len;
  const bool remask = !EDIT || nm >= 2;
  int k = min(max(mask_len, 1), nm - 1);
  int idx = k - 1;
  if (idx < 0) idx += P;
  if (remask) {
    for (int p = tid; p < P; p += blockDim.x) {
      const float x = conf_s[p];
      int lt = 0, le = 0;
      for (int j = 0; j < P; ++j) { const float y = conf_s[j]; lt += y < x; le += y <= x; }
      if (lt <= idx && idx < le) *thr_s = x;
    }
  }
  __syncthreads();
  const float thr = *thr_s;
  for (int p = tid; p < P; p += blockDim.x) {
    const size_t row = (size_t)b * P + p;
    const int pr = pred_s[p];
    a.tokens[row] = remask && conf_s[p] <= thr ? mask_tok : (int64_t)pr;
    if (a.pred) a.pred[row] = (int64_t)pr;
  }
}

template <bool SEEDED, bool REQ = false>
static void launch_rows(hipStream_t s, const StepArgs& a, const int64_t* tokens_in) {
  const size_t nrows = (size_t)a.B * a.P;
  dim3 grid((unsigned)((nrows + 15) / 16)), block(256);
  if (a.C <= 64) hipLaunchKernelGGL((sample_rows_kernel<1, SEEDED, REQ>), grid, block, 0, s, a, tokens_in);
  else if (a.C <= 128) hipLaunchKernelGGL((sample_rows_kernel<2, SEEDED, REQ>), grid, block, 0, s, a, tokens_in);
  else if (a.C <= 256) hipLaunchKernelGGL((sample_rows_kernel<4, SEEDED, REQ>), grid, block, 0, s, a, tokens_in);
  else if (a.C <= 512) hipLaunchKernelGGL((sample_rows_kernel<8, SEEDED, REQ>), grid, block, 0, s, a, tokens_in);
  else if (a.C <= 1024) hipLaunchKernelGGL((sample_rows_kernel<16, SEEDED, REQ>), grid, block, 0, s, a, tokens_in);
  else if (a.C <= 2048) hipLaunchKernelGGL((sample_rows_kernel<32, SEEDED, REQ>), grid, block, 0, s, a, tokens_in);
  else hipLaunchKernelGGL((sample_rows_kernel<64, SEEDED, REQ>), grid, block, 0, s, a, tokens_in);
}

int sample_step(hipStream_t s, const StepArgs& a, const int64_t* tokens_in, const int* num_regen, float mask_ratio) {
  if (a.C > 4096 || a.P > 8192) return -1;
  if (a.seeds && !num_regen) return -1;
  if (a.req && !a.seeds) return -1;
  if (a.req) launch_rows<true, true>(s, a, tokens_in);
  else if (a.seeds) launch_rows<true>(s, a, tokens_in);
  else launch_rows<false>(s, a, tokens_in);
  const size_t shm = (size_t)a.P * 8 + 16 * 4 + 16;
  const dim3 tblock(a.P >= 1024 ? 1024 : 512);
  if (a.req) hipLaunchKernelGGL((sample_thresh_kernel<true, true>), dim3(a.B), tblock, shm, s, a, tokens_in, 0.f, num_regen);
  else if (num_regen) hipLaunchKernelGGL(sample_thresh_kernel<true>, dim3(a.B), tblock, shm, s, a, tokens_in, mask_ratio, num_regen);
  else hipLaunchKernelGGL(sample_thresh_kernel<false>, dim3(a.B), tblock, shm, s, a, tokens_in, 0.f, (const int*)nullptr);
  return 0;
}

__global__ __launch_bounds__(256) void seeded_noise_kernel(const int64_t* __restrict__ seeds, int step, float rand_temp, float conf_w, float* __restrict__ exp_u,
                                                            float* __restrict__ exp_noise, float* __restrict__ conf_u, float* __restrict__ conf_noise, size_t total, int P, int C) {
  const size_t i = (size_t)blockIdx.x * 256 + threadIdx.x;
  if (i >= total) return;
  const size_t row = i / (size_t)C;
  const int c = (int)(i - row * (size_t)C);
  const size_t b = row / (size_t)P;
  const int slot = (int)(row - b * (size_t)P);
  const uint64_t seed = (uint64_t)seeds[b];
  float u;
  const float q = seeded_noise(seed, step, slot, c, false, 0.f, 0.f, &u);
  if (exp_noise) exp_noise[i] = q;
  if (exp_u) exp_u[i] = u;
  if (c == 0) {
    const float cn = seeded_noise(seed, step, slot, 0, true, rand_temp, conf_w, &u);
    if (conf_noise) conf_noise[row] = cn;
    if (conf_u) conf_u[row] = u;
  }
}
int seeded_noise_dump(hipStream_t s, const int64_t* seeds, int step, float rand_temp, float conf_w, float* exp_u, float* exp_noise, float* conf_u,
                      float* conf_noise, int B, int P, int C) {
  if (C > 4096 || P > 8192) return -1;
  const size_t total = (size_t)B * P * C;
  if ((total + 255) / 256 > 0x7fffffffull) return -1;
  hipLaunchKernelGGL(seeded_noise_kernel, dim3((unsigned)((total + 255) / 256)), dim3(256), 0, s, seeds, step, rand_temp, conf_w, exp_u, exp_noise, conf_u,
                     conf_noise, total, P, C);
  return 0;
}

__global__ void fill_i64_kernel(int64_t* dst, int64_t v, size_t n) {
  for (size_t i = (size_t)blockIdx.x * blockDim.x + threadIdx.x; i < n; i += (size_t)gridDim.x * blockDim.x) dst[i] = v;
}
void fill_i64(hipStream_t s, int64_t* dst, int64_t value, size_t n) {
  hipLaunchKernelGGL(fill_i64_kernel, dim3((unsigned)min((size_t)1024, (n + 255) / 256)), dim3(256), 0, s, dst, value, n);
}

__global__ void combine_groups_kernel(const int64_t* __restrict__ tok, int64_t* __restrict__ codes, size_t rows, int m, int gbits) {
  for (size_t i = (size_t)blockIdx.x * blockDim.x + threadIdx.x; i < rows; i += (size_t)gridDim.x * blockDim.x) {
    int64_t v = 0;
    for (int g = 0; g < m; ++g) v += tok[i * m + g] << (g * gbits);
    codes[i] = v;
  }
}
void combine_groups(hipStream_t s, const int64_t* tokens, int64_t* codes, size_t rows, int m, int gbits) {
  hipLaunchKernelGGL(combine_groups_kernel, dim3((unsigned)min((size_t)1024, (rows + 255) / 256)), dim3(256), 0, s,
                     tokens, codes, rows, m, gbits);
}

}
```

Measured before the change: 35.44.

## Pack only still-masked positions through the last transformer layer's FFN and head

```diff
diff --git a/include/maskbit_hip_diag.h b/include/maskbit_hip_diag.h
--- a/include/maskbit_hip_diag.h
+++ b/include/maskbit_hip_diag.h
@@ -55,6 +55,11 @@
 int mb_walk_seq(int slot, int n, int grp, int reverse);
 int mb_walk_row(int slot, int rows, int seq_rows, int pair, int reverse);
 int mb_walk_group(int seq_rows, int pair);
+int mb_masked_row_map(const int64_t* tokens, int* map, int* inv, int* count, int B, int n, int m, int C, mb_stream stream);
+int mb_diag_set_row_map(const int* src_rows, int src_pair_rows, float* y_out);
+int mb_gen_set_tail(mb_gen* g, int mode);
+int mb_gen_tail_counts(mb_gen* g, int* served, long long* packed_forwards, long long* full_forwards);
+int mb_gen_forward_tail(mb_gen* g, const int64_t* tokens, const int64_t* labels, int guided, float* logits, int* inv, int* packed, int B, mb_stream stream);
 int mb_gemm_ht_supported(int epi, int M, int N, int K);
 
 int mb_seeded_noise(const int64_t* seeds, int step, float randomize_temperature, float conf_weight, float* exp_u, float* exp_noise, float* conf_u,
diff --git a/maskbit_amd/_lib.py b/maskbit_amd/_lib.py
--- a/maskbit_amd/_lib.py
+++ b/maskbit_amd/_lib.py
@@ -201,6 +201,11 @@
     "mb_set_cu_count":(C.c_int, [C.c_int]),
     "mb_gen_set_walk": (C.c_int, [C.c_void_p, C.c_int]),
     "mb_diag_set_walk": (C.c_int, [C.c_int]),
+    "mb_masked_row_map": (C.c_int, [C.c_void_p] * 4 + [C.c_int] * 4 + [C.c_void_p]),
+    "mb_diag_set_row_map": (C.c_int, [C.c_void_p, C.c_int, C.c_void_p]),
+    "mb_gen_set_tail": (C.c_int, [C.c_void_p, C.c_int]),
+    "mb_gen_tail_counts": (C.c_int, [C.c_void_p, C.POINTER(C.c_int), C.POINTER(C.c_longlong), C.POINTER(C.c_longlong)]),
+    "mb_gen_forward_tail": (C.c_int, [C.c_void_p, C.c_void_p, C.c_void_p, C.c_int, C.c_void_p, C.c_void_p, C.POINTER(C.c_int), C.c_int, C.c_void_p]),
     "mb_walk_tile": (C.c_int, [C.c_int] * 3),
     "mb_walk_seq": (C.c_int, [C.c_int] * 4),
     "mb_walk_row": (C.c_int, [C.c_int] * 5),
diff --git a/maskbit_amd/csrc/diag.hip b/maskbit_amd/csrc/diag.hip
--- a/maskbit_amd/csrc/diag.hip
+++ b/maskbit_amd/csrc/diag.hip
@@ -18,6 +18,7 @@
 namespace {
 
 int g_walk_reverse = 0;
+mb::RowMap g_row_map;
 
 int run_gemm(mb_stream stream, int epi, const mb::GemmArgs& args, int variant, const char* mini = nullptr) {
   mb::GemmArgs a = args;
@@ -105,6 +106,16 @@
 extern "C" {
 
 int mb_set_cu_count(int n) { mb::set_cu_count(n); return 0; }
+int mb_diag_set_row_map(const int* src_rows, int src_pair_rows, float* y_out) {
+  if (src_pair_rows < 0 || (!src_rows && (src_pair_rows || y_out))) return fail(-1, "mb_diag_set_row_map: a pair distance or a copy without a map");
+  g_row_map = mb::RowMap{src_rows, src_pair_rows, y_out};
+  return 0;
+}
+int mb_masked_row_map(const int64_t* tokens, int* map, int* inv, int* count, int B, int n, int m, int C, mb_stream stream) {
+  if (!tokens || !map || !inv || !count) return fail(-1, "mb_masked_row_map: null argument");
+  if (mb::masked_row_map((hipStream_t)stream, tokens, map, inv, count, B, n, m, C)) return fail(-1, "mb_masked_row_map: bad sizes (B = %d in [1, 8192], n = %d, m = %d)", B, n, m);
+  return launched();
+}
 int mb_diag_set_walk(int reverse) {
   if (reverse != 0 && reverse != 1) return fail(-1, "mb_diag_set_walk: direction 0 or 1");
   g_walk_reverse = reverse;
@@ -220,7 +231,7 @@
 int mb_layernorm(const float* y, const float* gamma, const float* beta, float eps, float* x_f32, void* x_h16, void* x_lo, float* stats, int M,
                  int d, mb_stream stream) {
   if (!y || !gamma || !beta || M <= 0 || d <= 0 || d > 2048) return fail(-1, "mb_layernorm: bad arguments");
-  mb::layernorm_rows((hipStream_t)stream, y, gamma, beta, eps, x_f32, (h16*)x_h16, stats, M, d, (h16*)x_lo, mb::Fp4Rows{}, g_walk_reverse, 0);
+  mb::layernorm_rows((hipStream_t)stream, y, gamma, beta, eps, x_f32, (h16*)x_h16, stats, M, d, (h16*)x_lo, mb::Fp4Rows{}, g_walk_reverse, 0, g_row_map);
   return launched();
 }
 int mb_layernorm_f4_seq(const float* y, const float* gamma, const float* beta, float eps, float* x_f32, void* x_h16, void* x4, void* x4_scale, void* xl4,
@@ -228,7 +239,7 @@
   if (!y || !gamma || !beta || (!x4 && !xl4) || M <= 0) return fail(-1, "mb_layernorm_f4: bad arguments (an e2m1 output is required)");
   mb::Fp4Rows f4;
   if (int rc = f4_rows("mb_layernorm_f4", f4, x4, x4_scale, xl4, xl4_scale, M, d, seq_rows)) return rc;
-  mb::layernorm_rows((hipStream_t)stream, y, gamma, beta, eps, x_f32, (h16*)x_h16, nullptr, M, d, nullptr, f4, g_walk_reverse, seq_rows);
+  mb::layernorm_rows((hipStream_t)stream, y, gamma, beta, eps, x_f32, (h16*)x_h16, nullptr, M, d, nullptr, f4, g_walk_reverse, seq_rows, g_row_map);
   return launched();
 }
 int mb_layernorm_f4(const float* y, const float* gamma, const float* beta, float eps, float* x_f32, void* x_h16, void* x4, void* x4_scale, void* xl4,
@@ -241,7 +252,7 @@
   if (!y || !gamma || !beta || !x_h16 || P <= 0 || d <= 0 || d > 2048) return fail(-1, "mb_layernorm_pair: bad arguments");
   mb::Fp4Rows f4;
   if (int rc = f4_rows("mb_layernorm_pair", f4, x4, x4_scale, xl4, xl4_scale, P, d, seq_rows)) return rc;
-  if (mb::layernorm_pair((hipStream_t)stream, y, gamma, beta, eps, (h16*)x_h16, stats, P, d, f4, g_walk_reverse, seq_rows))
+  if (mb::layernorm_pair((hipStream_t)stream, y, gamma, beta, eps, (h16*)x_h16, stats, P, d, f4, g_walk_reverse, seq_rows, g_row_map))
     return fail(-3, "mb_layernorm_pair: width %d is outside the pair kernels (768 or 1024)", d);
   return launched();
 }
diff --git a/maskbit_amd/csrc/engine.hip b/maskbit_amd/csrc/engine.hip
--- a/maskbit_amd/csrc/engine.hip
+++ b/maskbit_amd/csrc/engine.hip
@@ -64,11 +64,57 @@
   int64_t *tok_a = nullptr, *tok_b = nullptr, *tok_cfg = nullptr, *lab_cfg = nullptr, *pred = nullptr, *codes = nullptr;
   uint8_t* drop_cfg = nullptr;
   float* logits = nullptr;
+  struct Tail {
+    bool ok = false, armed = false;
+    int mode = 1, B = 0, packed = 0;
+    int *map = nullptr, *inv = nullptr, *count = nullptr, *count_host = nullptr;
+    hipEvent_t ready = nullptr;
+    long long pruned = 0, full = 0;
+  } tail;
   mb::DevArena mem;
   int loaded = 0;
+  ~mb_gen() {
+    if (tail.ready) (void)hipEventDestroy(tail.ready);
+    if (tail.count_host) (void)hipHostFree(tail.count_host);
+  }
 };
 
 namespace {
+
+bool tail_arm(mb_gen* g, const int64_t* tokens, int B, bool guided, hipStream_t s) {
+  mb_gen::Tail& t = g->tail;
+  t.armed = false; t.packed = 0;
+  if (!t.ok || !t.mode || !guided || B > g->chunk_seqs / 2) return false;
+  hipStreamCaptureStatus cap = hipStreamCaptureStatusNone;
+  if (hipStreamIsCapturing(s, &cap) != hipSuccess || cap != hipStreamCaptureStatusNone) return false;
+  if (mb::masked_row_map(s, tokens, t.map, t.inv, t.count, B, g->c.seq, g->c.splits, g->C)) return false;
+  if (hipMemcpyAsync(t.count_host, t.count, sizeof(int), hipMemcpyDeviceToHost, s) != hipSuccess || hipEventRecord(t.ready, s) != hipSuccess) return false;
+  t.armed = true; t.B = B;
+  return true;
+}
+struct TailScope {
+  mb_gen::Tail& t;
+  explicit TailScope(mb_gen::Tail& tail) : t(tail) { t.armed = false; t.packed = 0; }
+  ~TailScope() { t.armed = false; t.packed = 0; }
+};
+int tail_take(mb_gen* g) {
+  const int packed = g->tail.packed;
+  g->tail.armed = false; g->tail.packed = 0;
+  return packed;
+}
+int tail_resolve(mb_gen* g, int B) {
+  mb_gen::Tail& t = g->tail;
+  if (!t.armed || t.B != B) return 0;
+  t.armed = false;
+  if (hipEventSynchronize(t.ready) != hipSuccess) return fail(-10, "masked tail: waiting for the row map failed");
+  const int n = g->c.seq, open = *t.count_host;
+  int packed = open > 0 ? (open + n - 1) / n : 1;
+  if (packed > B) return fail(-10, "masked tail: %d open positions in %d samples of %d", open, B, n);
+  if (packed == B && t.mode != 2) packed = 0;
+  t.packed = packed;
+  ++(packed ? t.pruned : t.full);
+  return packed;
+}
 
 void alloc_f4(mb::DevArena& m, F4Buf* b, size_t rows, size_t width, size_t ntok) {
   m.zeroed(&b->v, rows * 2 * width);
@@ -174,7 +220,9 @@
 int gen_forward_pair_impl(mb_gen* g, const int64_t* tokens, const int64_t* labels, const uint8_t* drop, float* logits, int B, bool wmode, hipStream_t s) {
   using namespace mb;
   const mb_gen_cfg& c = g->c;
-  const int d = c.hidden, f = c.mlp, N = g->N, nb = 2 * B, M = nb * N, P = B * N;
+  const int d = c.hidden, f = c.mlp, N = g->N, nb = 2 * B;
+  int M = nb * N, P = B * N, Bf = B;
+  float* y = g->y_f32;
   int rc = 0;
   int wdir = 0;
   auto walk_next = [&] { wdir ^= g->walk; return wdir; };
@@ -182,7 +230,7 @@
   auto f4_for = [&](bool feeds_ffn = false) {
     Fp4Rows f;
     if (wmode) {
-      f.x4 = g->x4.v; f.x4s = g->x4.s; f.nseq = B; f.seq_rows = N;
+      f.x4 = g->x4.v; f.x4s = g->x4.s; f.nseq = Bf; f.seq_rows = N;
       if (alo_on(feeds_ffn ? 2 : 0)) { f.xl4 = g->xl4.v; f.xl4s = g->xl4.s; }
     }
     return f;
@@ -228,15 +276,21 @@
       GemmArgs ga = pgemm(EPI_RES_F32, g->att, L.wo, L.bo, nullptr, g->y_f32, d, d, 4 * l + 1, wmode ? (alo_on(1) ? 2 : 1) : 0, g->att4.v, g->att4.s, g->attl4.v, g->attl4.s);
       if (l > 0 && !c.prenorm) { ga.ln_stats = g->ln_stats; ga.ln_g = g->layers[l - 1].ln2g; ga.ln_b = g->layers[l - 1].ln2b; }
       rc |= gemm_tn(s, EPI_RES_F32, ga, 257); }
+    RowMap gather;
+    if (l + 1 == c.depth) {
+      const int packed = tail_resolve(g, B);
+      if (packed < 0) return packed;
+      if (packed) { gather = RowMap{g->tail.map, P, (float*)g->qkv}; y = gather.y_out; Bf = packed; P = packed * N; M = 2 * P; }
+    }
     { ProfScope p("layernorm", s, true);
-      rc |= layernorm_pair(s, g->y_f32, c.prenorm ? L.ln2g : L.ln1g, c.prenorm ? L.ln2b : L.ln1b, 1e-12f, g->x_h16, c.prenorm ? nullptr : g->ln_stats, P, d, f4_for(true), walk_next(), N); }
+      rc |= layernorm_pair(s, g->y_f32, c.prenorm ? L.ln2g : L.ln1g, c.prenorm ? L.ln2b : L.ln1b, 1e-12f, g->x_h16, c.prenorm ? nullptr : g->ln_stats, P, d, f4_for(true), walk_next(), N, gather); }
     { ProfScope p("gemm_ffn_up", s, true);
       GemmArgs ga = pgemm(EPI_GELU_H16, g->x_h16, L.w1, L.b1, g->h, nullptr, f, d, 4 * l + 2, xlo_mode, g->x4.v, g->x4.s, g->xl4.v, g->xl4.s);
       if (wmode) { ga.out4 = g->h4.v; ga.out4_scale = g->h4.s; }
       if (lo_h) { ga.out4l = g->hl4.v; ga.out4l_scale = g->hl4.s; }
       rc |= gemm_tn(s, EPI_GELU_H16, ga, 257); }
     { ProfScope p("gemm_ffn_down", s, true);
-      GemmArgs ga = pgemm(EPI_RES_F32, g->h, L.w2, L.b2, nullptr, g->y_f32, d, f, 4 * l + 3, wmode ? (alo_on(3) ? 2 : 1) : 0, g->h4.v, g->h4.s, g->hl4.v, g->hl4.s);
+      GemmArgs ga = pgemm(EPI_RES_F32, g->h, L.w2, L.b2, nullptr, y, d, f, 4 * l + 3, wmode ? (alo_on(3) ? 2 : 1) : 0, g->h4.v, g->h4.s, g->hl4.v, g->hl4.s);
       if (!c.prenorm) { ga.ln_stats = g->ln_stats; ga.ln_g = L.ln1g; ga.ln_b = L.ln1b; }
       rc |= gemm_tn(s, EPI_RES_F32, ga, 257); }
     { ProfScope p("layernorm", s, true);
@@ -244,7 +298,7 @@
         if (l + 1 == c.depth) layernorm_rows(s, g->y_f32, g->lnag, g->lnab, 1e-12f, nullptr, g->x_h16, nullptr, M, d, g->x_lo, Fp4Rows{}, walk_next(), N);
         else rc |= layernorm_pair(s, g->y_f32, g->layers[l + 1].ln1g, g->layers[l + 1].ln1b, 1e-12f, g->x_h16, nullptr, P, d, f4_for(), walk_next(), N);
       }
-      else if (l + 1 == c.depth) layernorm_rows(s, g->y_f32, L.ln2g, L.ln2b, 1e-12f, nullptr, g->x_h16, g->ln_stats, M, d, g->x_lo, Fp4Rows{}, walk_next(), N);
+      else if (l + 1 == c.depth) layernorm_rows(s, y, L.ln2g, L.ln2b, 1e-12f, nullptr, g->x_h16, g->ln_stats, M, d, g->x_lo, Fp4Rows{}, walk_next(), N);
       else rc |= layernorm_pair(s, g->y_f32, L.ln2g, L.ln2b, 1e-12f, g->x_h16, g->ln_stats, P, d, f4_for(), walk_next(), N); }
   }
   rc |= head_gemms(g, logits, M, s);
@@ -456,6 +510,12 @@
   m.get(&g->lab_cfg, B); m.get(&g->drop_cfg, B); m.get(&g->logits, B * P * C);
   m.get(&g->num_regen, B);
   if (g->chunk_seqs < max_seqs) m.get(&g->logits_tmp, (size_t)g->chunk_seqs * P * C);
+  g->tail.ok = g->pair_ok && g->mini_ok && c.seq == 256 && !c.prenorm && !c.embed_tables && c.depth >= 1;
+  if (g->tail.ok) {
+    m.get(&g->tail.map, B * g->N); m.get(&g->tail.inv, B * c.seq); m.get(&g->tail.count, 1);
+    if (hipHostMalloc((void**)&g->tail.count_host, sizeof(int), hipHostMallocDefault) != hipSuccess ||
+        hipEventCreateWithFlags(&g->tail.ready, hipEventDisableTiming) != hipSuccess) { delete g; return fail(-10, "mb_gen_create: the masked tail's host word / event"); }
+  }
   if (int rc = m.failed("mb_gen_create")) { delete g; return rc; }
   *out = g;
   return 0;
@@ -567,6 +627,33 @@
   return 0;
 }
 
+int mb_gen_set_tail(mb_gen* g, int mode) {
+  if (!g || mode < 0 || mode > 2) return fail(-1, "mb_gen_set_tail: mode 0 (every row), 1 (packed where that saves a sequence) or 2 (always packed)");
+  g->tail.mode = mode;
+  return 0;
+}
+
+int mb_gen_tail_counts(mb_gen* g, int* served, long long* packed_forwards, long long* full_forwards) {
+  if (!g) return fail(-1, "mb_gen_tail_counts: null argument");
+  if (served) *served = g->tail.ok;
+  if (packed_forwards) *packed_forwards = g->tail.pruned;
+  if (full_forwards) *full_forwards = g->tail.full;
+  return 0;
+}
+
+int mb_gen_forward_tail(mb_gen* g, const int64_t* tokens, const int64_t* labels, int guided, float* logits, int* inv, int* packed, int B, mb_stream stream) {
+  if (!g || !tokens || !labels || !logits || !inv || !packed) return fail(-1, "mb_gen_forward_tail: null argument");
+  if (B <= 0 || (guided ? 2 : 1) * B > g->max_seqs) return fail(-1, "mb_gen_forward_tail: B=%d outside what the engine holds (%d sequences)", B, g->max_seqs);
+  hipStream_t s = (hipStream_t)stream;
+  TailScope tail_scope(g->tail);
+  if (!tail_arm(g, tokens, B, guided != 0, s)) return fail(-3, "mb_gen_forward_tail: this handle or batch does not run the masked tail");
+  int rc = guided ? gen_forward_cfg(g, tokens, labels, logits, B, s) : gen_forward(g, tokens, labels, nullptr, logits, B, s);
+  if (rc) return rc;
+  *packed = tail_take(g);
+  HIP_TRY(hipMemcpyAsync(inv, g->tail.inv, (size_t)B * g->c.seq * sizeof(int), hipMemcpyDeviceToDevice, s));
+  return launched();
+}
+
 int mb_gen_saturation_count(mb_gen* g, unsigned* count, int reset, mb_stream stream) {
   if (!g || !count) return fail(-1, "mb_gen_saturation_count: null argument");
   return mb::read_counter("mb_gen_saturation_count", g->sat, count, reset, (hipStream_t)stream);
@@ -716,17 +803,23 @@
   mb::StepArgs a{};
   a.logits_c = g->logits; a.B = B; a.P = (int)P; a.C = C;
   a.seeds = nz.seeds; a.rand_temp = nz.rand_temp;
+  a.m = m;
+  TailScope tail_scope(g->tail);
   for (int i = s0; i < s1; ++i) {
     int rc;
-    if (id.guided && (r.scale[i] != 0.0f || (!g->f32 && g->pair_ok && c.precision >= 4))) {
+    const bool guided_fwd = id.guided && (r.scale[i] != 0.0f || (!g->f32 && g->pair_ok && c.precision >= 4));
+    if (!(i == s1 - 1 && s1 < num_steps)) tail_arm(g, cur, B, guided_fwd, s);
+    if (guided_fwd) {
       rc = gen_forward_cfg(g, cur, labels, g->logits, B, s);
-      a.logits_u = g->logits + (size_t)B * P * C;
       if (B <= g->chunk_seqs / 2) { run.cfg_labels = labels; run.cfg_B = B; }
     } else {
       rc = gen_forward(g, cur, labels, nullptr, g->logits, B, s);
       a.logits_u = nullptr;
     }
     if (rc) return rc;
+    const int packed = tail_take(g);
+    a.inv = packed ? g->tail.inv : nullptr;
+    if (guided_fwd) a.logits_u = g->logits + (size_t)(packed ? packed : B) * P * C;
     const size_t k = (size_t)(i - s0);
     a.scale = r.scale[i]; a.temperature = r.temperature[i];
     a.tokens = nxt; a.pred = out.step_tokens ? out.step_tokens + k * B * P : g->pred;
@@ -788,12 +881,14 @@
   mb::StepArgs a{};
   a.logits_c = g->logits; a.P = (int)P; a.C = C;
   a.seeds = seeds;
+  a.m = m;
+  TailScope tail_scope(g->tail);
   for (int t = 0; t < S; ++t) {
     const int Bt = plan.active[t];
     int rc;
+    tail_arm(g, cur, Bt, guided, s);
     if (guided) {
       rc = gen_forward_cfg(g, cur, labels, g->logits, Bt, s);
-      a.logits_u = g->logits + (size_t)Bt * P * C;
       if (Bt <= g->chunk_seqs / 2) { run.cfg_labels = labels; run.cfg_B = Bt; }
       else run.cfg_labels = nullptr;
     } else {
@@ -801,6 +896,9 @@
       a.logits_u = nullptr;
     }
     if (rc) return rc;
+    const int packed = tail_take(g);
+    a.inv = packed ? g->tail.inv : nullptr;
+    if (guided) a.logits_u = g->logits + (size_t)(packed ? packed : Bt) * P * C;
     a.B = Bt;
     a.req = (const mb::RequestStep*)plan.table + (size_t)t * B;
     a.tokens = nxt; a.pred = out.step_tokens ? out.step_tokens + (size_t)t * B * P : g->pred;
diff --git a/maskbit_amd/csrc/mb_kernels.h b/maskbit_amd/csrc/mb_kernels.h
--- a/maskbit_amd/csrc/mb_kernels.h
+++ b/maskbit_amd/csrc/mb_kernels.h
@@ -104,12 +104,14 @@
 
 struct Fp4Rows { uint8_t* x4 = nullptr; uint8_t* x4s = nullptr; uint8_t* xl4 = nullptr; uint8_t* xl4s = nullptr; int nseq = 0; int seq_rows = 257; };
 
+struct RowMap { const int* src = nullptr; int src_pair_rows = 0; float* y_out = nullptr; };
+
 void layernorm_rows(hipStream_t s, const float* y, const float* gamma, const float* beta, float eps,
                     float* x_f32, h16* x_h16, float* stats, int M, int d, h16* x_lo = nullptr,
-                    const Fp4Rows& f4 = Fp4Rows{}, int reverse = 0, int seq_rows = 0);
+                    const Fp4Rows& f4 = Fp4Rows{}, int reverse = 0, int seq_rows = 0, const RowMap& map = RowMap{});
 
 int layernorm_pair(hipStream_t s, const float* y, const float* gamma, const float* beta, float eps, h16* x_h16, float* stats, int P, int d,
-                   const Fp4Rows& f4 = Fp4Rows{}, int reverse = 0, int seq_rows = 0);
+                   const Fp4Rows& f4 = Fp4Rows{}, int reverse = 0, int seq_rows = 0, const RowMap& map = RowMap{});
 int pairify_rows(hipStream_t s, const float* x32, h16* x_h16, int P, int d, const Fp4Rows& f4 = Fp4Rows{}, int reverse = 0, int seq_rows = 0);
 
 struct EmbedArgs {
@@ -151,10 +153,14 @@
   int step = 0;
   float rand_temp = 0.f, conf_w = 0.f;
   const RequestStep* req = nullptr;
+  const int* inv = nullptr;
+  int m = 1;
 };
 int sample_step(hipStream_t s, const StepArgs& a, const int64_t* tokens_in, const int* num_regen = nullptr, float mask_ratio = 0.f);
 int seeded_noise_dump(hipStream_t s, const int64_t* seeds, int step, float rand_temp, float conf_w, float* exp_u, float* exp_noise, float* conf_u,
                       float* conf_noise, int B, int P, int C);
+
+int masked_row_map(hipStream_t s, const int64_t* tokens, int* map, int* inv, int* count, int B, int n, int m, int C);
 
 void fill_i64(hipStream_t s, int64_t* dst, int64_t value, size_t n);
 
diff --git a/maskbit_amd/csrc/norm_embed.hip b/maskbit_amd/csrc/norm_embed.hip
--- a/maskbit_amd/csrc/norm_embed.hip
+++ b/maskbit_amd/csrc/norm_embed.hip
@@ -81,15 +81,15 @@
   }
 }
 
-template <int NV>
+template <int NV, bool MAP = false>
 __global__ __launch_bounds__(256) void ln_rows_kernel(const float* __restrict__ y, const float* __restrict__ gamma,
                                                       const float* __restrict__ beta, float eps, float* x_f32,
-                                                      h16* x_h16, float* stats, int M, int d, h16* x_lo, Fp4Rows f4, WalkRows wk) {
+                                                      h16* x_h16, float* stats, int M, int d, h16* x_lo, Fp4Rows f4, WalkRows wk, RowMap map = RowMap{}) {
   const int lane = threadIdx.x & 63;
   const int slot = blockIdx.x * 4 + __builtin_amdgcn_readfirstlane(threadIdx.x >> 6);
   if (slot >= M) return;
   const int row = walk_row(slot, M, wk);
-  const float* yr = y + (size_t)row * d;
+  const float* yr = y + (size_t)(MAP ? map.src[row] : row) * d;
   constexpr bool VEC = NV > 0;
   float4 v[VEC ? NV : 1]; float sc[VEC ? 1 : MAXS];
   const int ns = (d + 63) / 64;
@@ -98,6 +98,16 @@
     for (int q = 0; q < NV; ++q) v[q] = *(const float4*)(yr + q * 256 + lane * 4);
   }
   else     { for (int q = 0; q < ns; ++q) { const int c = lane + q * 64; sc[q] = c < d ? yr[c] : 0.f; } }
+  if constexpr (MAP) {
+    if (map.y_out) {
+      float* yo = map.y_out + (size_t)row * d;
+      if (VEC) {
+#pragma unroll
+        for (int q = 0; q < NV; ++q) *(float4*)(yo + q * 256 + lane * 4) = v[q];
+      }
+      else     { for (int q = 0; q < ns; ++q) { const int c = lane + q * 64; if (c < d) yo[c] = sc[q]; } }
+    }
+  }
   ln_finish<NV>(v, sc, ns, d, lane, gamma, beta, eps, x_f32 ? x_f32 + (size_t)row * d : nullptr,
                  x_h16 ? x_h16 + (size_t)row * d : nullptr, stats ? stats + (size_t)row * 2 : nullptr,
                  x_lo ? x_lo + (size_t)row * d : nullptr,
@@ -138,40 +148,51 @@
   if (f4.x4 || f4.xl4) fp4_rows_out<NV>(f4, xc, lane, row, d);
 }
 
-template <int NV>
+template <int NV, bool MAP = false>
 __global__ __launch_bounds__(256) void ln_pair_kernel(const float* __restrict__ y, const float* __restrict__ gamma, const float* __restrict__ beta, float eps,
-                                                      h16* __restrict__ x_h16, float* __restrict__ stats, int P, int d, Fp4Rows f4, WalkRows wk) {
+                                                      h16* __restrict__ x_h16, float* __restrict__ stats, int P, int d, Fp4Rows f4, WalkRows wk, RowMap map = RowMap{}) {
+  const int lane = threadIdx.x & 63;
+  const int slot = blockIdx.x * 4 + __builtin_amdgcn_readfirstlane(threadIdx.x >> 6);
+  if (slot >= P) return;
+  const int row = walk_row(slot, P, wk);
+  const int src = MAP ? map.src[row] : row, srcP = MAP ? map.src_pair_rows : P;
+  float4 vc[NV], vu[NV];
+#pragma unroll
+  for (int q = 0; q < NV; ++q) { vc[q] = *(const float4*)(y + (size_t)src * d + q * 256 + lane * 4); vu[q] = *(const float4*)(y + (size_t)(src + srcP) * d + q * 256 + lane * 4); }
+  if constexpr (MAP) {
+    if (map.y_out) {
+#pragma unroll
+      for (int q = 0; q < NV; ++q) { *(float4*)(map.y_out + (size_t)row * d + q * 256 + lane * 4) = vc[q]; *(float4*)(map.y_out + (size_t)(row + P) * d + q * 256 + lane * 4) = vu[q]; }
+    }
+  }
+  const float2 sc = ln_normalize<NV>(vc, d, gamma, beta, eps, lane), su = ln_normalize<NV>(vu, d, gamma, beta, eps, lane);
+  if (stats && lane == 0) { *(float2*)(stats + 2 * (size_t)row) = sc; *(float2*)(stats + 2 * (size_t)(row + P)) = su; }
+  pair_store<NV>(vc, vu, lane, x_h16 + (size_t)row * d, x_h16 + (size_t)(row + P) * d, f4, row, d);
+}
+
+template <int NV>
+__global__ __launch_bounds__(256) void pairify_kernel(const float* __restrict__ x32, h16* __restrict__ x_h16, int P, int d, Fp4Rows f4, WalkRows wk) {
   const int lane = threadIdx.x & 63;
   const int slot = blockIdx.x * 4 + __builtin_amdgcn_readfirstlane(threadIdx.x >> 6);
   if (slot >= P) return;
   const int row = walk_row(slot, P, wk);
   float4 vc[NV], vu[NV];
 #pragma unroll
-  for (int q = 0; q < NV; ++q) { vc[q] = *(const float4*)(y + (size_t)row * d + q * 256 + lane * 4); vu[q] = *(const float4*)(y + (size_t)(row + P) * d + q * 256 + lane * 4); }
-  const float2 sc = ln_normalize<NV>(vc, d, gamma, beta, eps, lane), su = ln_normalize<NV>(vu, d, gamma, beta, eps, lane);
-  if (stats && lane == 0) { *(float2*)(stats + 2 * (size_t)row) = sc; *(float2*)(stats + 2 * (size_t)(row + P)) = su; }
-  pair_store<NV>(vc, vu, lane, x_h16 + (size_t)row * d, x_h16 + (size_t)(row + P) * d, f4, row, d);
-}
-
-template <int NV>
-__global__ __launch_bounds__(256) void pairify_kernel(const float* __restrict__ x32, h16* __restrict__ x_h16, int P, int d, Fp4Rows f4, WalkRows wk) {
-  const int lane = threadIdx.x & 63;
-  const int slot = blockIdx.x * 4 + __builtin_amdgcn_readfirstlane(threadIdx.x >> 6);
-  if (slot >= P) return;
-  const int row = walk_row(slot, P, wk);
-  float4 vc[NV], vu[NV];
-#pragma unroll
   for (int q = 0; q < NV; ++q) { vc[q] = *(const float4*)(x32 + (size_t)row * d + q * 256 + lane * 4); vu[q] = *(const float4*)(x32 + (size_t)(row + P) * d + q * 256 + lane * 4); }
   pair_store<NV>(vc, vu, lane, x_h16 + (size_t)row * d, x_h16 + (size_t)(row + P) * d, f4, row, d);
 }
 
 int layernorm_pair(hipStream_t s, const float* y, const float* gamma, const float* beta, float eps, h16* x_h16, float* stats, int P, int d,
-                   const Fp4Rows& f4, int reverse, int seq_rows) {
+                   const Fp4Rows& f4, int reverse, int seq_rows, const RowMap& map) {
   dim3 grid((P + 3) / 4), block(256);
   const WalkRows wk = walk_rows(P, seq_rows, true, reverse);
-  if (d == 1024) hipLaunchKernelGGL(ln_pair_kernel<4>, grid, block, 0, s, y, gamma, beta, eps, x_h16, stats, P, d, f4, wk);
-  else if (d == 768) hipLaunchKernelGGL(ln_pair_kernel<3>, grid, block, 0, s, y, gamma, beta, eps, x_h16, stats, P, d, f4, wk);
-  else return -1;
+  if (d != 1024 && d != 768) return -1;
+  if (map.src) {
+    if (d == 1024) hipLaunchKernelGGL((ln_pair_kernel<4, true>), grid, block, 0, s, y, gamma, beta, eps, x_h16, stats, P, d, f4, wk, map);
+    else hipLaunchKernelGGL((ln_pair_kernel<3, true>), grid, block, 0, s, y, gamma, beta, eps, x_h16, stats, P, d, f4, wk, map);
+  }
+  else if (d == 1024) hipLaunchKernelGGL(ln_pair_kernel<4>, grid, block, 0, s, y, gamma, beta, eps, x_h16, stats, P, d, f4, wk, RowMap{});
+  else hipLaunchKernelGGL(ln_pair_kernel<3>, grid, block, 0, s, y, gamma, beta, eps, x_h16, stats, P, d, f4, wk, RowMap{});
   return 0;
 }
 int pairify_rows(hipStream_t s, const float* x32, h16* x_h16, int P, int d, const Fp4Rows& f4, int reverse, int seq_rows) {
@@ -184,12 +205,17 @@
 }
 
 void layernorm_rows(hipStream_t s, const float* y, const float* gamma, const float* beta, float eps,
-                    float* x_f32, h16* x_h16, float* stats, int M, int d, h16* x_lo, const Fp4Rows& f4, int reverse, int seq_rows) {
+                    float* x_f32, h16* x_h16, float* stats, int M, int d, h16* x_lo, const Fp4Rows& f4, int reverse, int seq_rows, const RowMap& map) {
   dim3 grid((M + 3) / 4), block(256);
   const WalkRows wk = walk_rows(M, seq_rows, false, reverse);
-  if (d == 1024) hipLaunchKernelGGL(ln_rows_kernel<4>, grid, block, 0, s, y, gamma, beta, eps, x_f32, x_h16, stats, M, d, x_lo, f4, wk);
-  else if (d == 768) hipLaunchKernelGGL(ln_rows_kernel<3>, grid, block, 0, s, y, gamma, beta, eps, x_f32, x_h16, stats, M, d, x_lo, f4, wk);
-  else hipLaunchKernelGGL(ln_rows_kernel<0>, grid, block, 0, s, y, gamma, beta, eps, x_f32, x_h16, stats, M, d, x_lo, Fp4Rows{}, wk);
+  if (map.src) {
+    if (d == 1024) hipLaunchKernelGGL((ln_rows_kernel<4, true>), grid, block, 0, s, y, gamma, beta, eps, x_f32, x_h16, stats, M, d, x_lo, f4, wk, map);
+    else if (d == 768) hipLaunchKernelGGL((ln_rows_kernel<3, true>), grid, block, 0, s, y, gamma, beta, eps, x_f32, x_h16, stats, M, d, x_lo, f4, wk, map);
+    else hipLaunchKernelGGL((ln_rows_kernel<0, true>), grid, block, 0, s, y, gamma, beta, eps, x_f32, x_h16, stats, M, d, x_lo, Fp4Rows{}, wk, map);
+  }
+  else if (d == 1024) hipLaunchKernelGGL(ln_rows_kernel<4>, grid, block, 0, s, y, gamma, beta, eps, x_f32, x_h16, stats, M, d, x_lo, f4, wk, RowMap{});
+  else if (d == 768) hipLaunchKernelGGL(ln_rows_kernel<3>, grid, block, 0, s, y, gamma, beta, eps, x_f32, x_h16, stats, M, d, x_lo, f4, wk, RowMap{});
+  else hipLaunchKernelGGL(ln_rows_kernel<0>, grid, block, 0, s, y, gamma, beta, eps, x_f32, x_h16, stats, M, d, x_lo, Fp4Rows{}, wk, RowMap{});
 }
 
 constexpr int MAXBITS = 24;
diff --git a/maskbit_amd/csrc/sampling.hip b/maskbit_amd/csrc/sampling.hip
--- a/maskbit_amd/csrc/sampling.hip
+++ b/maskbit_amd/csrc/sampling.hip
@@ -45,8 +45,29 @@
   for (int it = 0; it < 4; ++it) {
     const size_t row = (size_t)blockIdx.x * 16 + wave * 4 + it;
     if (row >= nrows) return;
-    const float* lc = a.logits_c + row * C;
-    const float* lu = a.logits_u ? a.logits_u + row * C : nullptr;
+    size_t lrow = row;
+    if (a.inv) {
+      const size_t b = row / (size_t)a.P;
+      const int sl = (int)(row - b * (size_t)a.P), pos = sl / a.m;
+      const int64_t tin = tokens_in[row];
+      if (tin != mask_tok) {
+        if (lane == 0) {
+          float cn;
+          if constexpr (SEEDED) {
+            float rt = a.rand_temp, cw = a.conf_w; int st = a.step;
+            if constexpr (REQ) { const RequestStep rs = a.req[b]; st = rs.step; rt = rs.rand_temp; cw = rs.conf_w; }
+            cn = seeded_noise((uint64_t)a.seeds[b], st, sl, 0, true, rt, cw, nullptr);
+          }
+          else cn = a.conf_noise[row];
+          const float conf = INFINITY + cn;
+          a.tokens[row] = (int64_t)(((uint64_t)(uint32_t)(int)tin << 32) | (uint64_t)__float_as_uint(conf));
+        }
+        continue;
+      }
+      lrow = (size_t)a.inv[b * (size_t)(a.P / a.m) + pos] * a.m + (sl - pos * a.m);
+    }
+    const float* lc = a.logits_c + lrow * C;
+    const float* lu = a.logits_u ? a.logits_u + lrow * C : nullptr;
     const float* qn = SEEDED ? nullptr : a.exp_noise + row * C;
     uint64_t seed = 0; int slot = 0;
     float scale = a.scale, temperature = a.temperature, rand_temp = a.rand_temp, conf_w = a.conf_w;
@@ -227,6 +248,57 @@
   return 0;
 }
 
+__global__ __launch_bounds__(1024) void masked_row_map_kernel(const int64_t* __restrict__ tokens, int* __restrict__ map, int* __restrict__ inv,
+                                                               int* __restrict__ count, int B, int n, int m, int C) {
+  extern __shared__ int off_s[];
+  const int tid = threadIdx.x, lane = tid & 63, wave = tid >> 6, nw = blockDim.x >> 6;
+  const int64_t mask_tok = (int64_t)C;
+  const int N = n + 1;
+  auto open_at = [&](int b, int p) {
+    bool o = false;
+    if (p < n) for (int g = 0; g < m; ++g) o |= tokens[((size_t)b * n + p) * m + g] == mask_tok;
+    return o;
+  };
+  for (int b = wave; b < B; b += nw) {
+    int c = 0;
+    for (int p0 = 0; p0 < n; p0 += 64) c += __popcll(__ballot(open_at(b, p0 + lane)));
+    if (lane == 0) off_s[b] = c;
+  }
+  __syncthreads();
+  if (tid == 0) {
+    int acc = 0;
+    for (int b = 0; b < B; ++b) { const int c = off_s[b]; off_s[b] = acc; acc += c; }
+    off_s[B] = acc;
+    *count = acc;
+  }
+  __syncthreads();
+  const int T = off_s[B];
+  for (int b = wave; b < B; b += nw) {
+    int e0 = off_s[b];
+    for (int p0 = 0; p0 < n; p0 += 64) {
+      const int p = p0 + lane;
+      const bool o = open_at(b, p);
+      const unsigned long long bal = __ballot(o);
+      const int e = e0 + __popcll(bal & ((1ull << lane) - 1ull));
+      if (p < n) inv[(size_t)b * n + p] = o ? e : -1;
+      if (o) map[(size_t)(e / n) * N + (e % n)] = b * N + p;
+      e0 += __popcll(bal);
+    }
+  }
+  __syncthreads();
+  const int pad = T > 0 ? map[0] : 0;
+  __syncthreads();
+  for (int r = tid; r < B * N; r += blockDim.x) {
+    const int q = r / N, t = r - q * N;
+    if (t == n || q * n + t >= T) map[r] = pad;
+  }
+}
+int masked_row_map(hipStream_t s, const int64_t* tokens, int* map, int* inv, int* count, int B, int n, int m, int C) {
+  if (B < 1 || B > 8192 || n < 1 || m < 1) return -1;
+  hipLaunchKernelGGL(masked_row_map_kernel, dim3(1), dim3(1024), (size_t)(B + 1) * sizeof(int), s, tokens, map, inv, count, B, n, m, C);
+  return 0;
+}
+
 __global__ void fill_i64_kernel(int64_t* dst, int64_t v, size_t n) {
   for (size_t i = (size_t)blockIdx.x * blockDim.x + threadIdx.x; i < n; i += (size_t)gridDim.x * blockDim.x) dst[i] = v;
 }
```

Result: no change. 35.57 (median of 6 runs) (+0.4%).
